# iacopo97/Multimodal-SAM-Adapter

Hardware: AMD Instinct MI355X
Metric: images/sec encoder fwd @1024x1024 RGB+LiDAR ViT-L (higher is better)
Workload: dtype split-operand MFMA: fp16 hi + e5m2 cross terms (h8c / h8 planes, ViT / interaction / up-conv GEMMs) fp16 hi/lo pairs x3 (TwinConvNeXt: f3 planes) and bf16 hi/lo x3 (neck, head); attention blocks with the rel-pos terms fused: every contraction on one fp16 MFMA (q, k, v, P rounded to fp16) in the bloc

## Files before the change

### include/mmsa.h

```cpp
#ifndef MMSA_H
#define MMSA_H
#include <stddef.h>
#include <stdint.h>
#ifdef __cplusplus
extern "C" {
#endif

#ifdef MMSA_BUILDING_LIBRARY
typedef hipStream_t mmsa_stream_t;
#else
typedef void* mmsa_stream_t;
#endif

#include "mmsa_version.h"
int mmsa_version(void);
const char* mmsa_last_error(void);

int mmsa_debug_poison_lds(unsigned pattern, mmsa_stream_t stream);
int mmsa_event_create(void** ev);
int mmsa_event_record(void* ev, mmsa_stream_t stream);
int mmsa_event_elapsed_ms(void* start, void* stop, float* ms);
int mmsa_event_destroy(void* ev);

enum { MMSA_ACT_NONE = 0, MMSA_ACT_GELU = 1, MMSA_ACT_RELU = 2, MMSA_ACT_RELU6 = 3, MMSA_ACT_HSWISH = 4, MMSA_ACT_SIGMOID = 5 };

enum { MMSA_DT_F32 = 0, MMSA_DT_F16 = 1, MMSA_DT_F64 = 2 };

enum { MMSA_FMT_B3 = 0, MMSA_FMT_H8 = 1, MMSA_FMT_H8C = 2, MMSA_FMT_F3 = 3, MMSA_FMT_W8 = 4  };

int mmsa_ms_deform_attn_forward(const void* value, const int64_t* spatial_shapes, const int64_t* level_start_index,
                                const void* sampling_loc, const void* attn_weight, void* out, int batch,
                                int spatial_size, int num_heads, int channels, int num_levels, int num_query,
                                int num_point, int im2col_step, int dtype, mmsa_stream_t stream);

int mmsa_ms_deform_attn_backward(const void* value, const int64_t* spatial_shapes, const int64_t* level_start_index,
                                 const void* sampling_loc, const void* attn_weight, const void* grad_output,
                                 void* grad_value, void* grad_sampling_loc, void* grad_attn_weight, int batch,
                                 int spatial_size, int num_heads, int channels, int num_levels, int num_query,
                                 int num_point, int im2col_step, int dtype, mmsa_stream_t stream);

int mmsa_msda_fused(const float* value, const int64_t* spatial_shapes, const int64_t* level_start_index,
                    const float* raw, long ldraw, const float* ref_points, float* out, long ldo,
                    uint16_t* out_planes, long ldop , int out_fmt , int batch,
                    int spatial_size, int num_heads, int channels, int num_levels, int num_query, int num_point,
                    float* clamp_max , mmsa_stream_t stream);

int mmsa_msda_fused_planes(const uint16_t* value_planes, long ldvp, int lo_bytes, const int64_t* spatial_shapes, const int64_t* level_start_index,
                           const float* raw, long ldraw, const float* ref_points, float* out, long ldo,
                           uint16_t* out_planes, long ldop, int out_fmt, int batch,
                           int spatial_size, int num_heads, int channels, int num_levels, int num_query, int num_point,
                           float* clamp_max, mmsa_stream_t stream);

int mmsa_rowstats_finalize(const float* rowstats, int rows, int strips, int D, float eps, float* mean_rstd, mmsa_stream_t stream);

int mmsa_zero_bytes(void* p, size_t bytes, mmsa_stream_t stream);
int mmsa_gemm_split3(const float* A, const uint16_t* Ap, long lda, long strideA,
                     const uint16_t* Wp, long strideW,
                     const float* bias, long strideBias, const float* colscale, const float* resid, long ldr,
                     long strideR, int resid_mod, float beta, float* C, long ldc, long strideC,
                     uint16_t* Cp, long ldcp, long strideCp, int M, int N, int K,
                     int batch, int act, float alpha, int out_mode, int ps_H, int ps_W, int ps_C, int fmt, int cp_fmt,
                     int max_grid, float* rowstats_out, const float* rownorm_mean_rstd, const float* rownorm_colsum, int flavour,
                     float* clamp_max , mmsa_stream_t stream);

int mmsa_convnext_mlp_fused(const uint16_t* Ap, long lda, long strideA, const uint16_t* W1p, long strideW1, const uint16_t* W2p,
                            long strideW2, const float* b1, const float* b2, const float* gamma, float* x, long ldx, long strideX,
                            int M, int C, int batch, int max_grid, int fmt,
                            float* clamp_max , mmsa_stream_t stream);

int mmsa_split_planes(const float* src, long ld, int rows, int cols, int cols_pad, uint16_t* planes, int kind,
                      float* clamp_max , mmsa_stream_t stream);

int mmsa_attention(const float* qkv, long ldq, const float* qkv_bias, const float* rp, float* out, long ldo, int B,
                   int H, int W, int heads, int head_dim, int window_size, float scale, mmsa_stream_t stream);
int mmsa_attention_planes(const uint16_t* qkv_planes, long ldq, const uint16_t* bias_planes, const float* rp,
                          uint16_t* out_planes, long ldo, int B, int H, int W, int heads, int head_dim,
                          int window_size, float scale, int out_fmt ,
                          int v_fmt ,
                          float* max_abs_logit , mmsa_stream_t stream);

int mmsa_relpos_bias(const float* qkv, long ldq, const float* Rh, const float* Rw, float* rp, int B, int H, int W,
                     int heads, int head_dim, int window_size, mmsa_stream_t stream);
int mmsa_relpos_bias_planes(const uint16_t* qkv_planes, long ldq, const float* Rh, const float* Rw,
                            float* rp, int B, int H, int W, int heads, int head_dim, int window_size, mmsa_stream_t stream);

int mmsa_layernorm_rows(const float* x, long ldx, const float* w, const float* b, float eps, float* y, long ldy,
                        float* y2, long ldy2, uint16_t* y_planes, long ldp ,
                        int rows, int C, int map_mode, int map_H, int map_W, int group_rows, long w_gstride, long y_gcol,
                        int y_wrap, int plane_fmt , float* clamp_max ,
                        mmsa_stream_t stream);

int mmsa_colstats(const float* x, long ldx, long strideB, const float* wrow, int B, int HW, int C, double* out,
                  int out_is_zero , mmsa_stream_t stream);

int mmsa_ffrm_finalize(const double* stats, int B, int HW, int C, float mean_w, float mean_b, const float* Wc,
                       const float* gn_w, const float* gn_b, float* mean_o, float* rstd_o, float* mult_o,
                       float* scratch , mmsa_stream_t stream);
int mmsa_lnhw_apply(const float* x, long ldx, const float* mean, const float* rstd, const float* mult, const float* w,
                    const float* bias, float* y, long ldy, int B, int HW, int C, mmsa_stream_t stream);

int mmsa_dwconv_nhwc(const float* x, long ldx, long xstrideB, const float* w, const float* bias, float* y, long ldy,
                     long ystrideB, uint16_t* y_planes, long ldp, long pstrideB , int planes_fmt ,
                     int B, int H, int W, int C, int k, int act,
                     int imgs_per_group ,
                     float* rowstats ,
                     float* clamp_max , mmsa_stream_t stream);
int mmsa_gconv_nhwc(const float* x, long ldx, const float* w, const float* bias, float* y, long ldy, int B, int H,
                    int W, int G, int cin_g, int cout_g, int k, int act, mmsa_stream_t stream);
int mmsa_gfe_qkv_conv(const float* x, long ldx, const float* w, float* y, long ldy, int B, int H, int W, int G, int cin_g, int cout_g,
                      int* covered, mmsa_stream_t stream);
int mmsa_dwpair_gate(const float* x, long ldx, const float* w, float* y, long ldy, uint16_t* y_planes, long ldp, int B, int H,
                     int W, int C, mmsa_stream_t stream);
int mmsa_im2col_nchw(const float* x, int B, int Ctot, int c0, int Cin, int H, int W, int p, float* out, int Kpad,
                     mmsa_stream_t stream);

long mmsa_gram_tn_scratch_bytes(int B, int P, int c);
int mmsa_gram_tn(const float* X, long ldx, const float* Y, long ldy, long strideB, double* G , int B, int P, int c,
                 int nblk, void* scratch, long scratch_bytes, mmsa_stream_t stream);
int mmsa_chanattn_build(const double* G, const double* sq, long sq_strideB, const double* sk, long sk_strideB,
                        const float* temp, const float* Wp, uint16_t* planes , int B, int c, int cpad,
                        int heads, mmsa_stream_t stream);
int mmsa_gffm_build(const double* E, uint16_t* x_planes, uint16_t* y_planes , int B, int c,
                    int cpad, mmsa_stream_t stream);
int mmsa_gelu_gate(const float* x, long ldx, float* y, long ldy, long rows, int C, mmsa_stream_t stream);
int mmsa_pool_hw(const float* z, long ldz, float* out, long ldo, int B, int H, int W, int C, mmsa_stream_t stream);
int mmsa_ca_apply(const float* z, long ldz, const float* att, long lda, float* out, long ldo,
                  uint16_t* out_planes, long ldp , int B, int H, int W, int C, mmsa_stream_t stream);

int mmsa_tail_fuse(const float* cmap, long ldc, long cstrideB, const float* xtok, long ldx, const float* bn_scale,
                   const float* bn_shift, float* out, uint16_t* out_planes , long ldp,
                   int B, int Hc, int Wc, int Hx, int Wx, int C, mmsa_stream_t stream);

int mmsa_global_attention_planes(const uint16_t* qkv_planes, long ldq, const uint16_t* bias_planes, const uint16_t* relpos_planes,
                                 uint16_t* out_planes, long ldo, int B, int H, int W, int heads, int head_dim, float scale,
                                 int out_fmt , int v_fmt ,
                                 float* max_abs_logit , mmsa_stream_t stream);

int mmsa_window_attention_planes(const uint16_t* qkv_planes, long ldq, const uint16_t* bias_planes,
                                 const uint16_t* relpos_planes, const uint16_t* selector, uint16_t* out_planes, long ldo, int B, int H, int W,
                                 int heads, int head_dim, int window_size, float scale, int out_fmt ,
                                 int v_fmt , float* max_abs_logit , mmsa_stream_t stream);

int mmsa_nchw_to_planes(const float* src, long strideB, uint16_t* planes, long ldp, int B, int C, long HW,
                        mmsa_stream_t stream);
int mmsa_head_fuse(const float* z0, const float* z1, int H1, int W1, const float* z2, int H2, int W2, const float* z3,
                   int H3, int W3, long ld, const float* bn_scale, const float* bn_shift, uint16_t* planes, long ldp,
                   float* out32, long ldo, int B, int H, int W, int C, int act, mmsa_stream_t stream);
int mmsa_tokens_to_nchw(const float* src, long ld, float* dst, int B, long HW, int C, mmsa_stream_t stream);

int mmsa_bilinear_accum_nchw(const float* src, long src_strideB, int B, int C, int hs, int ws, float* dst, int Hd, int Wd, int y0, int x0,
                             int hc, int wc, float* count, int accumulate, mmsa_stream_t stream);
int mmsa_div_count_nchw(float* x, const float* count, int B, int C, long HW, mmsa_stream_t stream);
int mmsa_argmax_nchw(const float* x, unsigned char* out, int B, int C, long HW, mmsa_stream_t stream);
int mmsa_crop_batch_nchw(const float* src, int B, int C, int H, int W, const int* windows, int n, float* dst, int hc, int wc,
                         mmsa_stream_t stream);
int mmsa_slide_argmax(const float* logits, int n, int C, int hs, int ws, const int* windows, unsigned char* out, int B, int H, int W,
                      int hc, int wc, int* uncovered, mmsa_stream_t stream);
int mmsa_slide_argmax_resized(const float* logits, int n, int C, int hs, int ws, const int* windows, unsigned char* out, int B, int H, int W,
                              int hc, int wc, int Hd, int Wd, int Hcut, int Wcut, int* uncovered, mmsa_stream_t stream);

int mmsa_softmax_flip_accum_nchw(const float* logits, float* acc, int B, int C, int H, int W, int flip, int accumulate, int finish_div, mmsa_stream_t stream);
int mmsa_aug_argmax(const float* const* logits, const int* views, int A, int C, const int* windows, const int* windows_host, int total,
                    unsigned char* out, int B, int Ho, int Wo, int* uncovered, mmsa_stream_t stream);

int mmsa_argmax_max_nchw(const float* x, unsigned char* out, float* maxval, int B, int C, long HW, mmsa_stream_t stream);
int mmsa_slide_argmax_conf(const float* logits, int n, int C, int hs, int ws, const int* windows, unsigned char* out, float* conf, int B, int H, int W,
                           int hc, int wc, int* uncovered, mmsa_stream_t stream);
int mmsa_slide_argmax_resized_conf(const float* logits, int n, int C, int hs, int ws, const int* windows, unsigned char* out, float* conf, int B, int H,
                                   int W, int hc, int wc, int Hd, int Wd, int Hcut, int Wcut, int* uncovered, mmsa_stream_t stream);
int mmsa_aug_argmax_conf(const float* const* logits, const int* views, int A, int C, const int* windows, const int* windows_host, int total,
                         unsigned char* out, float* conf, int B, int Ho, int Wo, int* uncovered, mmsa_stream_t stream);

enum { MMSA_PRE_U8 = 0, MMSA_PRE_F32 = 1 };
int mmsa_preprocess_nhwc(const void* src0, int dtype0, const void* src1, int dtype1, int B, int Hs, int Ws, const float* mean,
                         const float* sinv, const int* div255, const int* swap, const float* pad_val, float* dst, int H, int W,
                         mmsa_stream_t stream);
int mmsa_preprocess_crops(const void* src0, int dtype0, const void* src1, int dtype1, int B, int Hs, int Ws, const float* mean,
                          const float* sinv, const int* div255, const int* swap, const float* pad_val, int H, int W, const int* windows,
                          int n, float* dst, int hc, int wc, mmsa_stream_t stream);
int mmsa_preprocess_resize_nhwc(const void* src0, int dtype0, const void* src1, int dtype1, int B, int Hs, int Ws, const float* mean,
                                const float* sinv, const int* div255, const int* swap, const float* pad_val, float* dst, int H, int W,
                                int Hr, int Wr, const int* xofs, const void* xcoef, const int* yofs, const void* ycoef, int fixed_point,
                                mmsa_stream_t stream);
int mmsa_preprocess_resize_crops(const void* src0, int dtype0, const void* src1, int dtype1, int B, int Hs, int Ws, const float* mean,
                                 const float* sinv, const int* div255, const int* swap, const float* pad_val, int H, int W, const int* windows,
                                 int n, float* dst, int hc, int wc, int Hr, int Wr, const int* xofs, const void* xcoef, const int* yofs,
                                 const void* ycoef, int fixed_point, mmsa_stream_t stream);

int mmsa_eval_confusion_u8(const unsigned char* pred, const unsigned char* label, int B, int H, int W, int Hl, int Wl, const unsigned char* lut,
                           int C, const int* ymap, const int* xmap, const int* slots, int n_slots, int64_t* counts, mmsa_stream_t stream);
int mmsa_slide_argmax_eval(const float* logits, int n, int C, int hs, int ws, const int* windows, unsigned char* out, int B, int H, int W,
                           int hc, int wc, int* uncovered, const unsigned char* label, int Hl, int Wl, const unsigned char* lut, const int* ymap,
                           const int* xmap, const int* slots, int n_slots, int64_t* counts, mmsa_stream_t stream);

int mmsa_eval_calibration(const unsigned char* pred, const float* conf, const unsigned char* label, int B, int H, int W, int Hl, int Wl,
                          const unsigned char* lut, int C, const int* ymap, const int* xmap, const int* slots, int n_slots, int bins, int64_t* cal,
                          mmsa_stream_t stream);

int mmsa_eval_selective(const unsigned char* pred, const float* conf, const unsigned char* label, int B, int H, int W, int Hl, int Wl,
                        const unsigned char* lut, int C, const int* ymap, const int* xmap, const int* slots, int n_slots, int bins, int64_t* counts,
                        mmsa_stream_t stream);
int mmsa_abstain_u8(const unsigned char* pred, const float* conf, long n, int bins, int min_bin, unsigned char* out, mmsa_stream_t stream);

int mmsa_slide_argmax_conf_t(const float* logits, int n, int C, int hs, int ws, const int* windows, unsigned char* out, float* conf, int B, int H, int W,
                             int hc, int wc, int* uncovered, float inv_temperature, mmsa_stream_t stream);
int mmsa_slide_argmax_resized_conf_t(const float* logits, int n, int C, int hs, int ws, const int* windows, unsigned char* out, float* conf, int B, int H,
                                     int W, int hc, int wc, int Hd, int Wd, int Hcut, int Wcut, int* uncovered, float inv_temperature, mmsa_stream_t stream);
int mmsa_softmax_flip_accum_nchw_t(const float* logits, float* acc, int B, int C, int H, int W, int flip, int accumulate, int finish_div,
                                   float inv_temperature, mmsa_stream_t stream);
int mmsa_temperature_sweep_nchw(const float* logits, const unsigned char* label, int B, int C, int H, int W, int Hl, int Wl, const unsigned char* lut,
                                const int* ymap, const int* xmap, const int* slots, int n_slots, const float* inv_temperatures, int J, int bins,
                                int64_t* sweep, mmsa_stream_t stream);

int mmsa_argmax_score_nchw(const float* prob, unsigned char* out, float* score, int B, int C, int H, int W, int kind, float inv_log_c, mmsa_stream_t stream);
int mmsa_slide_argmax_score(const float* logits, int n, int C, int hs, int ws, const int* windows, unsigned char* out, float* score, int B, int H, int W,
                            int hc, int wc, int* uncovered, int kind, float inv_temperature, float inv_log_c, mmsa_stream_t stream);
int mmsa_slide_argmax_resized_score(const float* logits, int n, int C, int hs, int ws, const int* windows, unsigned char* out, float* score, int B, int H,
                                    int W, int hc, int wc, int Hd, int Wd, int Hcut, int Wcut, int* uncovered, int kind, float inv_temperature,
                                    float inv_log_c, mmsa_stream_t stream);

int mmsa_slide_argmax_topk(const float* logits, int n, int C, int hs, int ws, const int* windows, unsigned char* classes, float* probs, int B, int H, int W,
                           int hc, int wc, int* uncovered, int K, float inv_temperature, mmsa_stream_t stream);
int mmsa_argmax_topk_nchw(const float* prob, const unsigned char* first, unsigned char* classes, float* probs, int B, int C, int H, int W, int K,
                          mmsa_stream_t stream);
int mmsa_eval_topk_u8(const unsigned char* classes, int K, const unsigned char* label, int B, int H, int W, int Hl, int Wl, const unsigned char* lut, int C,
                      const int* ymap, const int* xmap, const int* slots, int n_slots, int64_t* counts, mmsa_stream_t stream);

int mmsa_eval_boundary_u8(const unsigned char* pred, const unsigned char* label, int B, int H, int W, int Hl, int Wl, const unsigned char* lut, int C,
                          const int* ymap, const int* xmap, const int* slots, int n_slots, int radius, int border, int64_t* counts, mmsa_stream_t stream);

int mmsa_boundary_distance_u8(const unsigned char* src, int B, int Hs, int Ws, const unsigned char* lut, const int* ymap, const int* xmap, int H, int W,
                              int cap, int border, unsigned short* scratch, unsigned short* d2, mmsa_stream_t stream);
int mmsa_eval_boundary_d2(const unsigned char* pred, const unsigned char* label, int B, int H, int W, int Hl, int Wl, const unsigned char* lut, int C,
                          const int* ymap, const int* xmap, const int* slots, int n_slots, const unsigned short* d2_pred, const unsigned short* d2_label,
                          int t, int64_t* counts, mmsa_stream_t stream);
int mmsa_eval_boundary_displacement(const unsigned char* pred, const unsigned char* label, int B, int H, int W, int Hl, int Wl, const unsigned char* lut,
                                    int C, const int* ymap, const int* xmap, const int* slots, int n_slots, const unsigned short* d2_pred,
                                    const unsigned short* d2_label, int cap, int64_t* hist, mmsa_stream_t stream);

int mmsa_components_u8(const unsigned char* src, int B, int Hs, int Ws, const unsigned char* lut, const int* ymap, const int* xmap, int H, int W,
                       int connectivity, int* root, mmsa_stream_t stream);
int mmsa_component_area(const int* root, int B, int H, int W, int* area, mmsa_stream_t stream);
int mmsa_suppress_small_u8(const unsigned char* pred, const int* root, const int* area, int B, int H, int W, int min_area, int fill, unsigned char* out,
                           mmsa_stream_t stream);
int mmsa_eval_segments(const unsigned char* pred, const unsigned char* label, int B, int H, int W, int Hl, int Wl, const unsigned char* lut, int C,
                       const int* ymap, const int* xmap, const int* slots, int n_slots, const int* root_pred, const int* root_label, int bins, int* scratch,
                       int64_t* counts, mmsa_stream_t stream);

int mmsa_segment_pairs(const unsigned char* pred, const unsigned char* label, int Hl, int Wl, const unsigned char* lut, int C, const int* ymap,
                       const int* xmap, const int* root_pred, const int* root_label, int B, int H, int W, int64_t* keys, int* counts, long capacity,
                       int* overflow, mmsa_stream_t stream);
int mmsa_eval_panoptic(const unsigned char* pred, const unsigned char* label, int B, int H, int W, int Hl, int Wl, const unsigned char* lut, int C,
                       const int* ymap, const int* xmap, const int* slots, int n_slots, const int* root_pred, const int* root_label, const int* planes,
                       const int64_t* keys, const int* counts, long capacity, int* match, int64_t* pq_counts, mmsa_stream_t stream);

int mmsa_render_u8(const unsigned char* pred, long pred_image_stride, long pred_row_stride, int B, int h, int w, const unsigned* palette, int npal,
                   int palette_reverse, const unsigned char* src, int Hs, int Ws, int src_reverse, double opacity, double one_minus_opacity,
                   unsigned char* out, mmsa_stream_t stream);
int mmsa_render_denorm_f32(const unsigned char* pred, long pred_image_stride, long pred_row_stride, int B, int h, int w, const unsigned* palette, int npal,
                           int palette_reverse, const float* src, int Cs, int Hs, int Ws, const float* mean, const float* std, int to_rgb, int mul255,
                           double opacity, double one_minus_opacity, unsigned char* out, mmsa_stream_t stream);

int mmsa_render_labels_u8(const unsigned char* pred, long pred_image_stride, long pred_row_stride, const unsigned char* label, int B, int h, int w, int Hl, int Wl,
                          const unsigned char* lut, int C, const int* ymap, const int* xmap, int mode, int wrong_by_label, const unsigned* table, int ntab,
                          const void* src, int src_form, int Cs, int Hs, int Ws, int src_reverse, const float* mean, const float* std, int to_rgb, int mul255,
                          double opacity, double one_minus_opacity, double mark_opacity, double one_minus_mark_opacity, unsigned char* out,
                          mmsa_stream_t stream);
int mmsa_render_values_f32(const float* values, const unsigned char* pred, long pred_image_stride, long pred_row_stride, int B, int h, int w, int bins,
                           int min_bin, const unsigned* table, int ntab, const void* src, int src_form, int Cs, int Hs, int Ws, int src_reverse,
                           const float* mean, const float* std, int to_rgb, int mul255, double opacity, double one_minus_opacity, double mark_opacity,
                           double one_minus_mark_opacity, unsigned char* out, mmsa_stream_t stream);
int mmsa_render_band_u8(const unsigned char* pred, long pred_image_stride, long pred_row_stride, const unsigned char* label, int B, int H, int W, int Hl, int Wl,
                        const unsigned char* lut, int C, const int* ymap, const int* xmap, int radius, int border, int where, int mark_by_label,
                        int inside_by_label, const unsigned* table, int ntab, const void* src, int src_form, int Cs, int Hs, int Ws, int src_reverse,
                        const float* mean, const float* std, int to_rgb, int mul255, double opacity, double one_minus_opacity, double mark_opacity,
                        double one_minus_mark_opacity, unsigned char* out, mmsa_stream_t stream);

#ifdef __cplusplus
}
#endif
#endif
```

### multimodal-sam-adapter_amd/csrc/common.h

```cpp
#pragma once
#include <hip/hip_runtime.h>
#include <stdint.h>
#include <stdio.h>
#include <stdarg.h>

#define MMSA_OK 0
#define MMSA_ERR_ARG (-1)
#define MMSA_ERR_LAUNCH (-2)

#define MMSA_BUILDING_LIBRARY 1
#include "../../include/mmsa.h"
void mmsa_set_error(const char* fmt, ...);

#ifdef MMSA_DEBUG_KNOBS
#include <stdlib.h>
static inline int mmsa_knob_env(const char* name, int dflt) { const char* v = getenv(name); return v ? atoi(v) : dflt; }
#define MMSA_KNOB(name_, dflt_) mmsa_knob_env(name_, dflt_)
#else
#define MMSA_KNOB(name_, dflt_) (dflt_)
#endif

#define MMSA_CHECK_ARG(cond, ...)            \
  do {                                       \
    if (!(cond)) {                           \
      mmsa_set_error(__VA_ARGS__);           \
      return MMSA_ERR_ARG;                   \
    }                                        \
  } while (0)

#define MMSA_CHECK_LAUNCH(name)                                              \
  do {                                                                       \
    hipError_t e__ = hipGetLastError();                                      \
    if (e__ != hipSuccess) {                                                 \
      mmsa_set_error("%s: launch failed: %s", name, hipGetErrorString(e__)); \
      return MMSA_ERR_LAUNCH;                                                \
    }                                                                        \
  } while (0)

#define MMSA_CHECK_INV_TEMPERATURE(name, it) \
  MMSA_CHECK_ARG((it) > 0.f && (it) <= 3.402823466e38f, "%s: inv_temperature = %g; a finite value > 0 is expected (float32(1 / T))", name, (double)(it))

#ifndef MMSA_XCD_ORDER
#define MMSA_XCD_ORDER 1
#endif
__device__ __forceinline__ unsigned mmsa_xcd_order(unsigned lin, unsigned total) {
#if MMSA_XCD_ORDER
  const unsigned per = total >> 3;
  return lin < (per << 3) ? (lin & 7u) * per + (lin >> 3) : lin;
#else
  (void)total;
  return lin;
#endif
}
__device__ __forceinline__ unsigned mmsa_block_lin() { return blockIdx.x + gridDim.x * (blockIdx.y + gridDim.y * blockIdx.z); }
__device__ __forceinline__ unsigned mmsa_block_count() { return gridDim.x * gridDim.y * gridDim.z; }

typedef __attribute__((ext_vector_type(8))) short bf16x8;
typedef __attribute__((ext_vector_type(4))) short bf16x4;
typedef __attribute__((ext_vector_type(4))) float f32x4;

__device__ __forceinline__ unsigned short f32_to_bf16_rn(float x) {
  unsigned u = __float_as_uint(x);
  u += 0x7FFFu + ((u >> 16) & 1u);
  return (unsigned short)(u >> 16);
}
__device__ __forceinline__ float bf16_to_f32(unsigned short h) { return __uint_as_float(((unsigned)h) << 16); }

typedef __attribute__((ext_vector_type(2))) __bf16 mmsa_bf16x2;
typedef __attribute__((ext_vector_type(2))) float mmsa_f32x2;

__device__ __forceinline__ void split2(float a, float b, unsigned& hi, unsigned& lo) {
  const mmsa_f32x2 v = {a, b};
  const mmsa_bf16x2 h = __builtin_convertvector(v, mmsa_bf16x2);
  const mmsa_f32x2 r = v - __builtin_convertvector(h, mmsa_f32x2);
  const mmsa_bf16x2 l = __builtin_convertvector(r, mmsa_bf16x2);
  hi = __builtin_bit_cast(unsigned, h);
  lo = __builtin_bit_cast(unsigned, l);
}

__device__ __forceinline__ void split_bf16(float x, unsigned short& hi, unsigned short& lo) {
  unsigned h, l;
  split2(x, 0.f, h, l);
  hi = (unsigned short)(h & 0xFFFFu);
  lo = (unsigned short)(l & 0xFFFFu);
}

__device__ __forceinline__ void split4(const float4 v, uint2& hi, uint2& lo) {
  split2(v.x, v.y, hi.x, lo.x);
  split2(v.z, v.w, hi.y, lo.y);
}

__device__ __forceinline__ float wave_sum(float v) {
#pragma unroll
  for (int o = 32; o > 0; o >>= 1) v += __shfl_xor(v, o, 64);
  return v;
}
__device__ __forceinline__ float half_wave_sum(float v) {
#pragma unroll
  for (int o = 16; o > 0; o >>= 1) v += __shfl_xor(v, o, 64);
  return v;
}
__device__ __forceinline__ float wave_max(float v) {
#pragma unroll
  for (int o = 32; o > 0; o >>= 1) v = fmaxf(v, __shfl_xor(v, o, 64));
  return v;
}

__host__ __device__ __forceinline__ int ilv(int k) { return ((k >> 5) << 6) | (k & 31); }

#define MMSA_CP_BASE(f_) ((f_) & 0xff)
#define MMSA_CP_SPLIT(f_) (((f_) >> 8) * 32)
#define MMSA_CP_AT(f_, col_) ((MMSA_CP_SPLIT(f_) > 0 && (col_) >= MMSA_CP_SPLIT(f_)) ? MMSA_FMT_H8 : MMSA_CP_BASE(f_))
#define MMSA_H8_MAX 57344.0f
#define MMSA_H8_LO_SCALE 2048.0f
#define MMSA_H8_MFMA_SCALE 0x74747474
#define MMSA_H8C_LO_COMP 1.09375f
typedef __attribute__((ext_vector_type(2))) _Float16 mmsa_h2;
typedef __attribute__((ext_vector_type(8))) _Float16 f16x8;
__device__ __forceinline__ void split2_f16(float a, float b, unsigned& hi, unsigned& lo) {
  const mmsa_f32x2 v = {a, b};
  const mmsa_h2 h = __builtin_convertvector(v, mmsa_h2);
  const mmsa_f32x2 r = v - __builtin_convertvector(h, mmsa_f32x2);
  hi = __builtin_bit_cast(unsigned, h);
  lo = __builtin_bit_cast(unsigned, __builtin_convertvector(r, mmsa_h2));
}
__device__ __forceinline__ unsigned pack_f16(float a, float b) {
  const mmsa_f32x2 v = {a, b};
  return __builtin_bit_cast(unsigned, __builtin_convertvector(v, mmsa_h2));
}

#define MMSA_F3_MAX 65504.0f
__device__ __forceinline__ void f3_split2(float a, float b, unsigned& hi, unsigned& lo) {
  a = __builtin_amdgcn_fmed3f(a, -MMSA_F3_MAX, MMSA_F3_MAX);
  b = __builtin_amdgcn_fmed3f(b, -MMSA_F3_MAX, MMSA_F3_MAX);
  split2_f16(a, b, hi, lo);
}
__device__ __forceinline__ void f3_split4(const float4 v, uint2& hi, uint2& lo) {
  f3_split2(v.x, v.y, hi.x, lo.x);
  f3_split2(v.z, v.w, hi.y, lo.y);
}
__device__ __forceinline__ void split4_fmt(const float4 v, uint2& hi, uint2& lo, int fmt) {
  if (fmt == MMSA_FMT_F3) f3_split4(v, hi, lo);
  else split4(v, hi, lo);
}

template <bool UPPER, bool COMP = false>
__device__ __forceinline__ void h8_split2(float a, float b, unsigned& hi, unsigned& lo8, unsigned& qh8) {
  a = __builtin_amdgcn_fmed3f(a, -MMSA_H8_MAX, MMSA_H8_MAX);
  b = __builtin_amdgcn_fmed3f(b, -MMSA_H8_MAX, MMSA_H8_MAX);
  const mmsa_f32x2 v = {a, b};
  const mmsa_h2 h = __builtin_convertvector(v, mmsa_h2);
  const mmsa_f32x2 hf = __builtin_convertvector(h, mmsa_f32x2);
  constexpr float ls_ = COMP ? MMSA_H8_LO_SCALE * MMSA_H8C_LO_COMP : MMSA_H8_LO_SCALE;
  const mmsa_f32x2 l = (v - hf) * ls_;
  hi = __builtin_bit_cast(unsigned, h);
  lo8 = (unsigned)__builtin_amdgcn_cvt_pk_bf8_f32(l.x, l.y, (int)lo8, UPPER);
  qh8 = (unsigned)__builtin_amdgcn_cvt_pk_bf8_f32(hf.x, hf.y, (int)qh8, UPPER);
}
template <bool COMP = false>
__device__ __forceinline__ void h8_split4(const float4 v, uint2& hi, unsigned& lo8, unsigned& qh8) {
  lo8 = 0u; qh8 = 0u;
  h8_split2<false, COMP>(v.x, v.y, hi.x, lo8, qh8);
  h8_split2<true, COMP>(v.z, v.w, hi.y, lo8, qh8);
}
__host__ __device__ __forceinline__ int h8_lo_off(int c) { return ((c >> 5) << 7) + 64 + (((c & 31) >> 3) << 4) + (c & 7); }

__device__ __forceinline__ void store_planes4(unsigned short* row, int c, const float4 v, int fmt) {
  if (fmt == MMSA_FMT_H8) {
    uint2 hi; unsigned lo8, qh8;
    h8_split4(v, hi, lo8, qh8);
    *reinterpret_cast<uint2*>(row + ilv(c)) = hi;
    unsigned char* rb = reinterpret_cast<unsigned char*>(row) + h8_lo_off(c);
    *reinterpret_cast<unsigned*>(rb) = lo8;
    *reinterpret_cast<unsigned*>(rb + 8) = qh8;
  } else {
    uint2 hh, ll;
    split4_fmt(v, hh, ll, fmt);
    *reinterpret_cast<uint2*>(row + ilv(c)) = hh;
    *reinterpret_cast<uint2*>(row + ilv(c) + 32) = ll;
  }
}

template <int XOR>
__device__ __forceinline__ void store_planes8_pair(unsigned short* row, int c8, const float4 v, int fmt, bool odd, bool do_store) {
  uint2 mine_hi, mine_x;
  if (fmt == MMSA_FMT_H8) h8_split4(v, mine_hi, mine_x.x, mine_x.y);
  else split4_fmt(v, mine_hi, mine_x, fmt);
  const uint2 snd = odd ? mine_hi : mine_x;
  uint2 rcv;
  rcv.x = __shfl_xor(snd.x, XOR, 64);
  rcv.y = __shfl_xor(snd.y, XOR, 64);
  uint4 pk;
  if (!odd) pk = make_uint4(mine_hi.x, mine_hi.y, rcv.x, rcv.y);
  else if (fmt == MMSA_FMT_H8) pk = make_uint4(rcv.x, mine_x.x, rcv.y, mine_x.y);
  else pk = make_uint4(rcv.x, rcv.y, mine_x.x, mine_x.y);
  const int off = odd ? (fmt == MMSA_FMT_H8 ? h8_lo_off(c8) >> 1 : ilv(c8) + 32) : ilv(c8);
  if (do_store) *reinterpret_cast<uint4*>(row + off) = pk;
}

__device__ __forceinline__ void store_planes1(unsigned short* row, int c, float x, int fmt) {
  if (fmt == MMSA_FMT_H8) {
    unsigned hi, lo8 = 0u, qh8 = 0u;
    h8_split2<false>(x, 0.f, hi, lo8, qh8);
    row[ilv(c)] = (unsigned short)(hi & 0xFFFFu);
    unsigned char* rb = reinterpret_cast<unsigned char*>(row) + h8_lo_off(c & ~3) + (c & 3);
    rb[0] = (unsigned char)(lo8 & 0xFFu);
    rb[8] = (unsigned char)(qh8 & 0xFFu);
  } else {
    unsigned short hh, ll;
    if (fmt == MMSA_FMT_F3) {
      unsigned h2, l2;
      f3_split2(x, 0.f, h2, l2);
      hh = (unsigned short)(h2 & 0xFFFFu);
      ll = (unsigned short)(l2 & 0xFFFFu);
    } else {
      split_bf16(x, hh, ll);
    }
    row[ilv(c)] = hh;
    row[ilv(c) + 32] = ll;
  }
}

struct H8cRow {
  unsigned short* hi;
  unsigned char* lo;
};
__device__ __forceinline__ H8cRow h8c_row(unsigned short* base, long ld_pair, long row, int kpad) {
  unsigned short* pb = base + (row >> 1) * ld_pair;
  H8cRow r;
  r.hi = pb + (row & 1) * kpad;
  r.lo = reinterpret_cast<unsigned char*>(pb + 2 * kpad) + (row & 1) * 64;
  return r;
}
__host__ __device__ __forceinline__ int h8c_lo_off(int k) { return ((k >> 6) << 7) + (((k & 31) >> 3) << 4) + (((k >> 5) & 1) << 3) + (k & 7); }
__device__ __forceinline__ void h8c_store4(const H8cRow r, int c, const float4 v) {
  uint2 hi; unsigned lo8, qh8;
  h8_split4<true>(v, hi, lo8, qh8);
  *reinterpret_cast<uint2*>(r.hi + c) = hi;
  *reinterpret_cast<unsigned*>(r.lo + h8c_lo_off(c)) = lo8;
}
template <int XOR>
__device__ __forceinline__ void h8c_store8_pair(const H8cRow r, int c8, const float4 v, bool odd, bool do_store) {
  uint2 hi; unsigned lo8, qh8;
  h8_split4<true>(v, hi, lo8, qh8);
  const uint2 snd = odd ? hi : make_uint2(lo8, 0u);
  uint2 rcv;
  rcv.x = __shfl_xor(snd.x, XOR, 64);
  rcv.y = __shfl_xor(snd.y, XOR, 64);
  if (!do_store) return;
  if (!odd) *reinterpret_cast<uint4*>(r.hi + c8) = make_uint4(hi.x, hi.y, rcv.x, rcv.y);
  else *reinterpret_cast<uint2*>(r.lo + h8c_lo_off(c8)) = make_uint2(rcv.x, lo8);
}
__device__ __forceinline__ void h8c_store1(const H8cRow r, int c, float x) {
  unsigned hi, lo8 = 0u, qh8 = 0u;
  h8_split2<false, true>(x, 0.f, hi, lo8, qh8);
  r.hi[c] = (unsigned short)(hi & 0xFFFFu);
  r.lo[h8c_lo_off(c)] = (unsigned char)(lo8 & 0xFFu);
}
template <int XOR>
__device__ __forceinline__ void store_planes8_pair_any(unsigned short* base, long ld, long row, int kpad, int c8, const float4 v, int fmt, bool odd, bool do_store) {
  if (fmt == MMSA_FMT_H8C) h8c_store8_pair<XOR>(h8c_row(base, ld, row, kpad), c8, v, odd, do_store);
  else store_planes8_pair<XOR>(base + row * ld, c8, v, fmt, odd, do_store);
}
__device__ __forceinline__ void store_planes4_any(unsigned short* base, long ld, long row, int kpad, int c, const float4 v, int fmt) {
  if (fmt == MMSA_FMT_H8C) h8c_store4(h8c_row(base, ld, row, kpad), c, v);
  else store_planes4(base + row * ld, c, v, fmt);
}
#define MMSA_PAD64(x_) (((x_) + 63) & ~63)

#define MMSA_W8_EMIN (-15)
#define MMSA_W8_EMAX 7

__device__ __forceinline__ float mmsa_clamp_limit(int fmt) {
  return (fmt == MMSA_FMT_H8 || fmt == MMSA_FMT_H8C) ? MMSA_H8_MAX : fmt == MMSA_FMT_F3 ? MMSA_F3_MAX : 3.0e38f;
}
#ifndef MMSA_CW_LEG
#define MMSA_CW_LEG 1
#endif
#ifndef MMSA_CW_REGS
#define MMSA_CW_REGS 1
#endif
#ifndef MMSA_CLAMP_WATCH
#define MMSA_CLAMP_WATCH 1
#endif
__device__ __forceinline__ void clamp_see(float& m, const float4 v) {
  if (MMSA_CLAMP_WATCH) m = fmaxf(fmaxf(m, fmaxf(fabsf(v.x), fabsf(v.y))), fmaxf(fabsf(v.z), fabsf(v.w)));
}
__device__ __forceinline__ void clamp_see1(float& m, float x) { if (MMSA_CLAMP_WATCH) m = fmaxf(m, fabsf(x)); }
__device__ __forceinline__ void clamp_report(float* word, float m, float limit) {
  if (MMSA_CLAMP_WATCH && word != nullptr && m > limit) atomicMax(reinterpret_cast<int*>(word), __float_as_int(m));
}

enum { ACT_NONE = 0, ACT_GELU = 1, ACT_RELU = 2, ACT_RELU6 = 3, ACT_HSWISH = 4, ACT_SIGMOID = 5 };

#ifndef MMSA_GELU_DEG
#define MMSA_GELU_DEG 7
#endif
#if MMSA_GELU_DEG == 6
#define MMSA_GELU_COEFFS {-1.151147127e+00f, -4.589156806e-01f, -5.323817953e-02f, 7.977456786e-03f, -7.398718735e-04f, 2.992386726e-05f}
#elif MMSA_GELU_DEG == 7
#define MMSA_GELU_COEFFS {-1.151126981e+00f, -4.590439200e-01f, -5.294858292e-02f, 7.670805324e-03f, -5.757985055e-04f, -1.279479329e-05f, 4.278379038e-06f}
#else
#define MMSA_GELU_COEFFS {-1.151111007e+00f, -4.591621459e-01f, -5.262760073e-02f, 7.245406508e-03f, -2.720646735e-04f, -1.314778056e-04f, 2.805791701e-05f, -1.902148711e-06f}
#endif
__device__ __forceinline__ float gelu1(float x) {
  constexpr float c[MMSA_GELU_DEG] = MMSA_GELU_COEFFS;
  const float a = fminf(fabsf(x), 6.0f);
  float p = fmaf(c[MMSA_GELU_DEG - 1], a, c[MMSA_GELU_DEG - 2]);
#pragma unroll
  for (int k = MMSA_GELU_DEG - 3; k >= 0; --k) p = fmaf(p, a, c[k]);
  p *= a;
  const float r = 1.0f - __builtin_amdgcn_exp2f(p);
  const float h = x * 0.5f;
  return fmaf(fabsf(h), r, h);
}
typedef __attribute__((ext_vector_type(2))) float mmsa_f2;
__device__ __forceinline__ mmsa_f2 gelu2(mmsa_f2 x) {
  mmsa_f2 a;
  a.x = fminf(fabsf(x.x), 6.0f);
  a.y = fminf(fabsf(x.y), 6.0f);
  constexpr float c[MMSA_GELU_DEG] = MMSA_GELU_COEFFS;
  mmsa_f2 p = a * c[MMSA_GELU_DEG - 1] + c[MMSA_GELU_DEG - 2];
#pragma unroll
  for (int k = MMSA_GELU_DEG - 3; k >= 0; --k) p = p * a + c[k];
  p = p * a;
  mmsa_f2 e;
  e.x = __builtin_amdgcn_exp2f(p.x);
  e.y = __builtin_amdgcn_exp2f(p.y);
  const mmsa_f2 r = 1.0f - e;
  const mmsa_f2 h = x * 0.5f;
  mmsa_f2 o;
  o.x = fmaf(fabsf(h.x), r.x, h.x);
  o.y = fmaf(fabsf(h.y), r.y, h.y);
  return o;
}
__device__ __forceinline__ float4 gelu4(float4 v) {
  const mmsa_f2 a = gelu2((mmsa_f2){v.x, v.y}), b = gelu2((mmsa_f2){v.z, v.w});
  return make_float4(a.x, a.y, b.x, b.y);
}

__device__ __forceinline__ float apply_act(float x, int act) {
  switch (act) {
    case ACT_GELU: return gelu1(x);
    case ACT_RELU: return fmaxf(x, 0.0f);
    case ACT_RELU6: return fminf(fmaxf(x, 0.0f), 6.0f);
    case ACT_HSWISH: return x * (fminf(fmaxf(x + 3.0f, 0.0f), 6.0f) / 6.0f);
    case ACT_SIGMOID: return 1.0f / (1.0f + expf(-x));
    default: return x;
  }
}

static inline int cdiv(long a, long b) { return (int)((a + b - 1) / b); }

#define MMSA_MAX_DEVICES 16
struct MmsaPerDevice { int cus[MMSA_MAX_DEVICES]; };
template <class F>
static inline int mmsa_per_device(MmsaPerDevice& st, F&& setup) {
  int dev = 0;
  if (hipGetDevice(&dev) != hipSuccess || dev < 0) dev = 0;
  if (dev < MMSA_MAX_DEVICES && st.cus[dev] > 0) return st.cus[dev];
  setup();
  int n = 0;
  if (hipDeviceGetAttribute(&n, hipDeviceAttributeMultiprocessorCount, dev) != hipSuccess || n <= 0) n = 256;
  if (dev < MMSA_MAX_DEVICES) st.cus[dev] = n;
  return n;
}
```

### multimodal-sam-adapter_amd/csrc/head.hip

```cpp
#include "common.h"

template <bool VEC>
__global__ __launch_bounds__(256) void nchw_to_planes_kernel(const float* __restrict__ src, long strideB, int C, long HW,
                                                             uint16_t* __restrict__ planes, long ldp) {
  __shared__ float tile[32][257];
  const int b = blockIdx.z;
  const long pix0 = (long)blockIdx.x * 256;
  const int c0 = blockIdx.y * 32;
  const int lane = threadIdx.x & 63, wv = threadIdx.x >> 6;
  const float* sb = src + (long)b * strideB;
  if (VEC) {
    float4 v[8];
#pragma unroll
    for (int j = 0; j < 8; ++j) {
      const int c = c0 + wv * 8 + j;
      const long pix = pix0 + 4 * lane;
      v[j] = (c < C && pix < HW) ? *reinterpret_cast<const float4*>(sb + (long)c * HW + pix) : make_float4(0.f, 0.f, 0.f, 0.f);
    }
#pragma unroll
    for (int j = 0; j < 8; ++j) {
      float* t = &tile[wv * 8 + j][4 * lane];
      t[0] = v[j].x; t[1] = v[j].y; t[2] = v[j].z; t[3] = v[j].w;
    }
  } else {
#pragma unroll
    for (int j = 0; j < 8; ++j) {
      const int cl = wv * 8 + j;
      const int c = c0 + cl;
#pragma unroll
      for (int k = 0; k < 4; ++k) {
        const long pix = pix0 + lane + 64 * k;
        tile[cl][lane + 64 * k] = (c < C && pix < HW) ? sb[(long)c * HW + pix] : 0.f;
      }
    }
  }
  __syncthreads();
  const int q = threadIdx.x & 3;
  const int pl = threadIdx.x >> 2;
#pragma unroll
  for (int k = 0; k < 4; ++k) {
    const int p = pl + 64 * k;
    const long pix = pix0 + p;
    if (pix >= HW) continue;
    float v[8];
#pragma unroll
    for (int j = 0; j < 8; ++j) v[j] = tile[8 * q + j][p];
    uint4 hi, lo;
    split2(v[0], v[1], hi.x, lo.x);
    split2(v[2], v[3], hi.y, lo.y);
    split2(v[4], v[5], hi.z, lo.z);
    split2(v[6], v[7], hi.w, lo.w);
    uint16_t* row = planes + ((long)b * HW + pix) * ldp + (long)blockIdx.y * 64 + 8 * q;
    *reinterpret_cast<uint4*>(row) = hi;
    *reinterpret_cast<uint4*>(row + 32) = lo;
  }
}

extern "C" int mmsa_nchw_to_planes(const float* src, long strideB, uint16_t* planes, long ldp, int B, int C, long HW,
                                   hipStream_t stream) {
  MMSA_CHECK_ARG(src && planes, "nchw_to_planes: null pointer");
  MMSA_CHECK_ARG(B > 0 && C > 0 && HW > 0, "nchw_to_planes: bad shape");
  const int cpad = (C + 31) / 32 * 32;
  MMSA_CHECK_ARG(ldp >= 2L * cpad && ldp % 64 == 0, "nchw_to_planes: planes row stride %ld < 2*%d or not a multiple of 64", ldp, cpad);
  MMSA_CHECK_ARG((reinterpret_cast<uintptr_t>(planes) & 127) == 0, "nchw_to_planes: planes must be 128-byte aligned");
  MMSA_CHECK_ARG(strideB >= (long)C * HW, "nchw_to_planes: image stride %ld < C*HW", strideB);
  dim3 grid(cdiv(HW, 256), cpad / 32, B);
  if ((HW & 3) == 0 && (strideB & 3) == 0 && (reinterpret_cast<uintptr_t>(src) & 15) == 0)
    hipLaunchKernelGGL(nchw_to_planes_kernel<true>, grid, dim3(256), 0, stream, src, strideB, C, HW, planes, ldp);
  else
    hipLaunchKernelGGL(nchw_to_planes_kernel<false>, grid, dim3(256), 0, stream, src, strideB, C, HW, planes, ldp);
  MMSA_CHECK_LAUNCH("nchw_to_planes");
  return MMSA_OK;
}

struct HeadLevels {
  const float* z[3];
  int H[3], W[3];
  float rh[3], rw[3];
};

__global__ __launch_bounds__(256) void head_fuse_kernel(const float* __restrict__ z0, long ld, HeadLevels lv, int nlv,
                                                        const float* __restrict__ bn_scale, const float* __restrict__ bn_shift,
                                                        uint16_t* __restrict__ planes, long ldp, float* __restrict__ out32, long ldo,
                                                        int H, int W, int C, long npix_total, int act) {
  const long pixg = (long)blockIdx.x * 4 + (threadIdx.x >> 6);
  if (pixg >= npix_total) return;
  const int lane = threadIdx.x & 63;
  const unsigned hw = (unsigned)H * (unsigned)W;
  const unsigned pg = (unsigned)pixg;
  const int b = (int)(pg / hw);
  const int rem = (int)(pg - (unsigned)b * hw);
  const int h = rem / W, w = rem - h * W;
  long o00[3], o01[3], o10[3], o11[3];
  float lh[3], lw[3];
#pragma unroll
  for (int i = 0; i < 3; ++i) {
    if (i < nlv) {
      float sh = ((float)h + 0.5f) * lv.rh[i] - 0.5f;
      float sw = ((float)w + 0.5f) * lv.rw[i] - 0.5f;
      sh = sh < 0.f ? 0.f : sh;
      sw = sw < 0.f ? 0.f : sw;
      const int h0 = min((int)sh, lv.H[i] - 1), w0 = min((int)sw, lv.W[i] - 1);
      const int h1 = h0 + (h0 < lv.H[i] - 1 ? 1 : 0), w1 = w0 + (w0 < lv.W[i] - 1 ? 1 : 0);
      lh[i] = sh - (float)h0;
      lw[i] = sw - (float)w0;
      const long base = (long)b * lv.H[i] * lv.W[i];
      o00[i] = (base + (long)h0 * lv.W[i] + w0) * ld;
      o01[i] = (base + (long)h0 * lv.W[i] + w1) * ld;
      o10[i] = (base + (long)h1 * lv.W[i] + w0) * ld;
      o11[i] = (base + (long)h1 * lv.W[i] + w1) * ld;
    } else {
      o00[i] = o01[i] = o10[i] = o11[i] = 0; lh[i] = lw[i] = 0.f;
    }
  }
  for (int c = lane * 8; c < C; c += 512) {
    float v[8];
    float4 t[3][2][4];
    const float4 a = *reinterpret_cast<const float4*>(z0 + pixg * ld + c);
    const float4 d = *reinterpret_cast<const float4*>(z0 + pixg * ld + c + 4);
#pragma unroll
    for (int i = 0; i < 3; ++i) {
      const int il = i < nlv ? i : 0;
      const float* zi = (nlv > 0 ? lv.z[il] : z0 + pixg * ld) + c;
#pragma unroll
      for (int hh = 0; hh < 2; ++hh) {
        t[i][hh][0] = *reinterpret_cast<const float4*>(zi + o00[il] + 4 * hh);
        t[i][hh][1] = *reinterpret_cast<const float4*>(zi + o01[il] + 4 * hh);
        t[i][hh][2] = *reinterpret_cast<const float4*>(zi + o10[il] + 4 * hh);
        t[i][hh][3] = *reinterpret_cast<const float4*>(zi + o11[il] + 4 * hh);
      }
    }
    const float4 s0 = *reinterpret_cast<const float4*>(bn_scale + c), s1 = *reinterpret_cast<const float4*>(bn_scale + c + 4);
    const float4 f0 = *reinterpret_cast<const float4*>(bn_shift + c), f1 = *reinterpret_cast<const float4*>(bn_shift + c + 4);
    __builtin_amdgcn_sched_barrier(0);
    v[0] = a.x; v[1] = a.y; v[2] = a.z; v[3] = a.w; v[4] = d.x; v[5] = d.y; v[6] = d.z; v[7] = d.w;
#pragma unroll
    for (int i = 0; i < 3; ++i) {
      if (i < nlv) {
        const float w00 = (1.f - lh[i]) * (1.f - lw[i]), w01 = (1.f - lh[i]) * lw[i], w10 = lh[i] * (1.f - lw[i]), w11 = lh[i] * lw[i];
#pragma unroll
        for (int hh = 0; hh < 2; ++hh) {
          const float4 t00 = t[i][hh][0], t01 = t[i][hh][1], t10 = t[i][hh][2], t11 = t[i][hh][3];
          v[4 * hh + 0] += w00 * t00.x + w01 * t01.x + w10 * t10.x + w11 * t11.x;
          v[4 * hh + 1] += w00 * t00.y + w01 * t01.y + w10 * t10.y + w11 * t11.y;
          v[4 * hh + 2] += w00 * t00.z + w01 * t01.z + w10 * t10.z + w11 * t11.z;
          v[4 * hh + 3] += w00 * t00.w + w01 * t01.w + w10 * t10.w + w11 * t11.w;
        }
      }
    }
    const float bs[8] = {s0.x, s0.y, s0.z, s0.w, s1.x, s1.y, s1.z, s1.w}, bf[8] = {f0.x, f0.y, f0.z, f0.w, f1.x, f1.y, f1.z, f1.w};
#pragma unroll
    for (int j = 0; j < 8; ++j) v[j] = apply_act(v[j] * bs[j] + bf[j], act);
    if (out32) {
      *reinterpret_cast<float4*>(out32 + pixg * ldo + c) = make_float4(v[0], v[1], v[2], v[3]);
      *reinterpret_cast<float4*>(out32 + pixg * ldo + c + 4) = make_float4(v[4], v[5], v[6], v[7]);
    }
    if (planes) {
      uint4 hi, lo;
      split2(v[0], v[1], hi.x, lo.x);
      split2(v[2], v[3], hi.y, lo.y);
      split2(v[4], v[5], hi.z, lo.z);
      split2(v[6], v[7], hi.w, lo.w);
      uint16_t* row = planes + pixg * ldp + ilv(c);
      *reinterpret_cast<uint4*>(row) = hi;
      *reinterpret_cast<uint4*>(row + 32) = lo;
    }
  }
}

extern "C" int mmsa_head_fuse(const float* z0, const float* z1, int H1, int W1, const float* z2, int H2, int W2, const float* z3,
                              int H3, int W3, long ld, const float* bn_scale, const float* bn_shift, uint16_t* planes, long ldp,
                              float* out32, long ldo, int B, int H, int W, int C, int act, hipStream_t stream) {
  MMSA_CHECK_ARG(z0 && bn_scale && bn_shift && (planes || out32), "head_fuse: null pointer");
  MMSA_CHECK_ARG(((((uintptr_t)bn_scale) | ((uintptr_t)bn_shift) | ((uintptr_t)z0)) & 15) == 0, "head_fuse: z0 / bn_scale / bn_shift must be 16-byte aligned");
  MMSA_CHECK_ARG(B > 0 && H > 0 && W > 0 && C > 0 && C % 8 == 0, "head_fuse: bad shape (C=%d must be a multiple of 8)", C);
  MMSA_CHECK_ARG(ld >= C && ld % 4 == 0, "head_fuse: row stride %ld", ld);
  MMSA_CHECK_ARG(!planes || (ldp >= 2L * ((C + 31) / 32 * 32) && ldp % 64 == 0 && (reinterpret_cast<uintptr_t>(planes) & 127) == 0),
                 "head_fuse: planes stride/alignment");
  MMSA_CHECK_ARG(!out32 || (ldo >= C && ldo % 4 == 0), "head_fuse: fp32 out stride %ld", ldo);
  HeadLevels lv;
  int n = 0;
  const float* zs[3] = {z1, z2, z3};
  const int hs[3] = {H1, H2, H3}, wsz[3] = {W1, W2, W3};
  for (int i = 0; i < 3; ++i) {
    lv.z[i] = nullptr; lv.H[i] = lv.W[i] = 1; lv.rh[i] = lv.rw[i] = 1.f;
  }
  for (int i = 0; i < 3; ++i) {
    if (!zs[i]) continue;
    MMSA_CHECK_ARG(hs[i] > 0 && wsz[i] > 0, "head_fuse: level %d has bad size", i + 1);
    lv.z[n] = zs[i]; lv.H[n] = hs[i]; lv.W[n] = wsz[i];
    lv.rh[n] = (float)hs[i] / (float)H;
    lv.rw[n] = (float)wsz[i] / (float)W;
    ++n;
  }
  const long npix = (long)B * H * W;
  MMSA_CHECK_ARG(npix < (1L << 31), "head_fuse: too many pixels for the 32-bit index arithmetic");
  hipLaunchKernelGGL(head_fuse_kernel, dim3(cdiv(npix, 4)), dim3(256), 0, stream, z0, ld, lv, n, bn_scale, bn_shift, planes, ldp,
                     out32, ldo, H, W, C, npix, act);
  MMSA_CHECK_LAUNCH("head_fuse");
  return MMSA_OK;
}

__global__ __launch_bounds__(256) void tokens_to_nchw_kernel(const float* __restrict__ src, long ld, float* __restrict__ dst, long HW, int C) {
  __shared__ float tile[32][33];
  const int b = blockIdx.z;
  const long pix0 = (long)blockIdx.x * 32;
  const int c0 = blockIdx.y * 32;
  const int tx = threadIdx.x & 31, ty = threadIdx.x >> 5;
#pragma unroll
  for (int k = 0; k < 4; ++k) {
    const int pl = ty + 8 * k;
    const long pix = pix0 + pl;
    const int c = c0 + tx;
    tile[pl][tx] = (pix < HW && c < C) ? src[((long)b * HW + pix) * ld + c] : 0.f;
  }
  __syncthreads();
#pragma unroll
  for (int k = 0; k < 4; ++k) {
    const int c = c0 + ty + 8 * k;
    const long pix = pix0 + tx;
    if (c < C && pix < HW) dst[((long)b * C + c) * HW + pix] = tile[tx][ty + 8 * k];
  }
}

extern "C" int mmsa_tokens_to_nchw(const float* src, long ld, float* dst, int B, long HW, int C, hipStream_t stream) {
  MMSA_CHECK_ARG(src && dst, "tokens_to_nchw: null pointer");
  MMSA_CHECK_ARG(B > 0 && HW > 0 && C > 0 && ld >= C, "tokens_to_nchw: bad shape");
  dim3 grid(cdiv(HW, 32), cdiv(C, 32), B);
  hipLaunchKernelGGL(tokens_to_nchw_kernel, grid, dim3(256), 0, stream, src, ld, dst, HW, C);
  MMSA_CHECK_LAUNCH("tokens_to_nchw");
  return MMSA_OK;
}
```

### multimodal-sam-adapter_amd/csrc/neck.hip

```cpp
#include "common.h"
#include <stdlib.h>

#define GR_ROWS 256
#define GR_BLK 96
#define GR_T 6
__device__ __forceinline__ bool gram_block_needed(int bi, int bj, int c, int nblk) {
  if (nblk <= 1) return true;
  const int ch = c / nblk;
  const int hi0 = (GR_BLK * bi) / ch, hi1 = min(c - 1, GR_BLK * bi + GR_BLK - 1) / ch;
  const int hj0 = (GR_BLK * bj) / ch, hj1 = min(c - 1, GR_BLK * bj + GR_BLK - 1) / ch;
  return !(hi1 < hj0 || hj1 < hi0);
}
__global__ __launch_bounds__(256) void gram_part_kernel(const float* __restrict__ X, long ldx, const float* __restrict__ Y, long ldy,
                                                        long strideB, float4* __restrict__ part, int P, int c, int nblk, int nslice) {
  const int nb = (c + GR_BLK - 1) / GR_BLK;
  const unsigned wg_ = mmsa_xcd_order(mmsa_block_lin(), mmsa_block_count());
  const int bx_ = (int)(wg_ % gridDim.x);
  const int bi = bx_ / nb, bj = bx_ % nb;
  if (!gram_block_needed(bi, bj, c, nblk)) return;
  const int lane = threadIdx.x & 63, wave = threadIdx.x >> 6;
  const int l15 = lane & 15, kk = lane >> 4;
  const int b = (int)(wg_ / (gridDim.x * gridDim.y));
  const int slice = (int)((wg_ / gridDim.x) % gridDim.y);
  const int u0 = 3 * (wave >> 1), v0 = 3 * (wave & 1);
// ... 11 lines not shown
#pragma unroll
  for (int u = 0; u < 3; ++u)
#pragma unroll
    for (int v = 0; v < 3; ++v) acc[u][v] = (f32x4){0.f, 0.f, 0.f, 0.f};
  const int pbeg = slice * GR_ROWS;
  const int pend = min(P, pbeg + GR_ROWS);
#define GR_LOADS(av_, bv_, pb_)                                                                   \
  _Pragma("unroll") for (int t = 0; t < 8; ++t) {                                                 \
    const int p = (pb_) + 4 * t + kk;                                                             \
    const long pr = p < pend ? p : pbeg;             \
    const float* xr = Xb + pr * ldx;                                                              \
    const float* yr = Yb + pr * ldy;                                                              \
    _Pragma("unroll") for (int u = 0; u < 3; ++u) { av_[t][u] = xr[ci[u]]; bv_[t][u] = yr[cj[u]]; } \
  }
#define GR_MFMAS(av_, bv_, pb_)                                                                   \
  _Pragma("unroll") for (int t = 0; t < 8; ++t) {                                                 \
    const float mp = ((pb_) + 4 * t + kk) < pend ? 1.f : 0.f;                                     \
      \
    _Pragma("unroll") for (int u = 0; u < 3; ++u) { av_[t][u] *= mp * mi[u]; bv_[t][u] *= mp * mj[u]; } \
    _Pragma("unroll") for (int u = 0; u < 3; ++u)                                                 \
      _Pragma("unroll") for (int v = 0; v < 3; ++v) acc[u][v] = __builtin_amdgcn_mfma_f32_16x16x4f32(av_[t][u], bv_[t][v], acc[u][v], 0, 0, 0); \
  }
  float a0[8][3], b0[8][3], a1[8][3], b1[8][3];
  GR_LOADS(a0, b0, pbeg)
#pragma unroll 1
  for (int pb = pbeg; pb < pend; pb += 64) {
    __builtin_amdgcn_sched_barrier(0);
    GR_LOADS(a1, b1, pb + 32)
    __builtin_amdgcn_sched_barrier(0);
    GR_MFMAS(a0, b0, pb)
    __builtin_amdgcn_sched_barrier(0);
    GR_LOADS(a0, b0, pb + 64)
    __builtin_amdgcn_sched_barrier(0);
    GR_MFMAS(a1, b1, pb + 32)
  }
#undef GR_LOADS
#undef GR_MFMAS
  float4* dst = part + ((((long)b * nb * nb + bx_) * nslice + slice) * (GR_T * GR_T)) * 64 + lane;
#pragma unroll
  for (int u = 0; u < 3; ++u)
#pragma unroll
    for (int v = 0; v < 3; ++v) dst[((u0 + u) * GR_T + v0 + v) * 64] = make_float4(acc[u][v][0], acc[u][v][1], acc[u][v][2], acc[u][v][3]);
}
__global__ __launch_bounds__(1024) void gram_sum_kernel(const float4* __restrict__ part, double* __restrict__ G, int c, int nblk, int nslice) {
  __shared__ double red[16][64][4];
  const int nb = (c + GR_BLK - 1) / GR_BLK;
  const int bi = blockIdx.y / nb, bj = blockIdx.y % nb;
  if (!gram_block_needed(bi, bj, c, nblk)) return;
  const int lane = threadIdx.x & 63, q = threadIdx.x >> 6;
  const int tile = blockIdx.x, b = blockIdx.z;
  const float4* src = part + (((long)b * nb * nb + blockIdx.y) * nslice * (GR_T * GR_T) + tile) * 64 + lane;
  double s0 = 0, s1 = 0, s2 = 0, s3 = 0;
#pragma unroll 4
  for (int sl = q; sl < nslice; sl += 16) {
    const float4 v = src[(long)sl * (GR_T * GR_T) * 64];
    s0 += (double)v.x; s1 += (double)v.y; s2 += (double)v.z; s3 += (double)v.w;
  }
  red[q][lane][0] = s0; red[q][lane][1] = s1; red[q][lane][2] = s2; red[q][lane][3] = s3;
  __syncthreads();
  if (threadIdx.x < 256) {
    const int ln = threadIdx.x >> 2, r = threadIdx.x & 3;
    double t = 0;
#pragma unroll
    for (int k = 0; k < 16; ++k) t += red[k][ln][r];
    const int u = tile / GR_T, v = tile % GR_T;
    const int i = GR_BLK * bi + 16 * u + 4 * (ln >> 4) + r;
    const int j = GR_BLK * bj + 16 * v + (ln & 15);
    if (i < c && j < c) G[((long)b * c + i) * c + j] = t;
  }
}

extern "C" long mmsa_gram_tn_scratch_bytes(int B, int P, int c) {
  if (B <= 0 || P <= 0 || c <= 0) return 0;
  const long nb = cdiv(c, GR_BLK);
  return (long)B * nb * nb * cdiv(P, GR_ROWS) * (GR_T * GR_T) * 64 * (long)sizeof(float4);
}

extern "C" int mmsa_gram_tn(const float* X, long ldx, const float* Y, long ldy, long strideB, double* G,
                            int B, int P, int c, int nblk, void* scratch, long scratch_bytes, hipStream_t stream) {
  MMSA_CHECK_ARG(X && Y && G && scratch && B > 0 && P > 0 && c > 0 && nblk > 0 && c % nblk == 0, "gram_tn: bad args");
  MMSA_CHECK_ARG(scratch_bytes >= mmsa_gram_tn_scratch_bytes(B, P, c) && (((uintptr_t)scratch) & 15) == 0,
                 "gram_tn: scratch of %ld bytes, %ld needed (mmsa_gram_tn_scratch_bytes), 16-byte aligned", scratch_bytes, mmsa_gram_tn_scratch_bytes(B, P, c));
  const int nb = cdiv(c, GR_BLK), nslice = cdiv(P, GR_ROWS);
  hipLaunchKernelGGL(gram_part_kernel, dim3(nb * nb, nslice, B), dim3(256), 0, stream, X, ldx, Y, ldy, strideB,
                     reinterpret_cast<float4*>(scratch), P, c, nblk, nslice);
  MMSA_CHECK_LAUNCH("gram_tn");
  hipLaunchKernelGGL(gram_sum_kernel, dim3(GR_T * GR_T, nb * nb, B), dim3(1024), 0, stream, reinterpret_cast<const float4*>(scratch), G, c, nblk, nslice);
  MMSA_CHECK_LAUNCH("gram_tn (slice sum)");
  return MMSA_OK;
}

__global__ __launch_bounds__(256) void chanattn_build_kernel(const double* __restrict__ G, const double* __restrict__ sq,
                                                             long sq_strideB, const double* __restrict__ sk, long sk_strideB,
                                                             const float* __restrict__ temp, const float* __restrict__ Wp,
                                                             unsigned short* __restrict__ planes,
                                                             int c, int cpad, int heads) {
  extern __shared__ float attn[];
  const int h = blockIdx.x, b = blockIdx.y;
  const int ch = c / heads;
  const int st = ch + 1;
  const double* Gb = G + (long)b * c * c;
  const float t = temp[h];
  float* nq = attn + ch * st;
  float* nk = nq + ch;
  for (int i = threadIdx.x; i < ch; i += 256) {
    nq[i] = fmaxf((float)sqrt(sq[(long)b * sq_strideB + h * ch + i]), 1e-12f);
    nk[i] = fmaxf((float)sqrt(sk[(long)b * sk_strideB + h * ch + i]), 1e-12f);
  }
  __syncthreads();
  for (int idx0 = threadIdx.x; idx0 < ch * ch; idx0 += 256 * 4) {
    double gv[4];
    int ii[4], jj[4];
#pragma unroll
    for (int u = 0; u < 4; ++u) {
      const int idx = min(idx0 + 256 * u, ch * ch - 1);
      ii[u] = idx / ch; jj[u] = idx - ii[u] * ch;
      gv[u] = Gb[(long)(h * ch + ii[u]) * c + h * ch + jj[u]];
    }
#pragma unroll
    for (int u = 0; u < 4; ++u)
      if (idx0 + 256 * u < ch * ch) attn[ii[u] * st + jj[u]] = (float)gv[u] / (nq[ii[u]] * nk[jj[u]]) * t;
  }
  __syncthreads();
  for (int i = threadIdx.x; i < ch; i += 256) {
    float mx = -INFINITY;
#pragma unroll 8
    for (int j = 0; j < ch; ++j) mx = fmaxf(mx, attn[i * st + j]);
    float s = 0.f;
#pragma unroll 4
    for (int j = 0; j < ch; ++j) {
      const float e = expf(attn[i * st + j] - mx);
      attn[i * st + j] = e;
      s += e;
    }
    const float inv = 1.0f / s;
#pragma unroll 8
    for (int j = 0; j < ch; ++j) attn[i * st + j] *= inv;
  }
  __syncthreads();
  const int o_per = (c + gridDim.z - 1) / gridDim.z;
  const int o_beg = blockIdx.z * o_per, o_end = min(c, o_beg + o_per);
  float* wl = nk + ch;
  {
    const int nw = (o_end - o_beg) * ch;
    for (int idx0 = threadIdx.x; idx0 < nw; idx0 += 256 * 4) {
      float wv[4];
#pragma unroll
      for (int u = 0; u < 4; ++u) {
        const int idx = min(idx0 + 256 * u, nw - 1);
        const int o = idx / ch, i = idx - o * ch;
        wv[u] = Wp[(long)(o_beg + o) * c + h * ch + i];
      }
#pragma unroll
      for (int u = 0; u < 4; ++u)
        if (idx0 + 256 * u < nw) wl[idx0 + 256 * u] = wv[u];
    }
  }
  __syncthreads();
  for (int idx = o_beg * ch + threadIdx.x; idx < o_end * ch; idx += 256) {
    const int o = idx / ch, j = idx - o * ch;
    const float* wrow = wl + (o - o_beg) * ch;
    float acc = 0.f;
#pragma unroll 8
    for (int i = 0; i < ch; ++i) acc += wrow[i] * attn[i * st + j];
    unsigned short hh, ll;
    split_bf16(acc, hh, ll);
    unsigned short* q_ = planes + ((long)b * c + o) * 2 * cpad + ilv(h * ch + j);
    q_[0] = hh;
    q_[32] = ll;
  }
}

extern "C" int mmsa_chanattn_build(const double* G, const double* sq, long sq_strideB, const double* sk, long sk_strideB,
                                   const float* temp, const float* Wp, unsigned short* planes,
                                   int B, int c, int cpad, int heads, hipStream_t stream) {
  MMSA_CHECK_ARG(G && sq && sk && temp && Wp && planes, "chanattn_build: null pointer");
  MMSA_CHECK_ARG(c % heads == 0 && cpad >= c, "chanattn_build: bad channel split");
  const int ch = c / heads;
  const int nz = c >= 192 ? 16 : 4;
  const size_t smem = ((size_t)ch * (ch + 1) + 2 * (size_t)ch + (size_t)cdiv(c, nz) * ch) * sizeof(float);
  MMSA_CHECK_ARG(smem <= 64 * 1024, "chanattn_build: head block too large");
  hipLaunchKernelGGL(chanattn_build_kernel, dim3(heads, B, nz), dim3(256), smem, stream, G, sq, sq_strideB, sk, sk_strideB, temp, Wp, planes, c, cpad, heads);
  MMSA_CHECK_LAUNCH("chanattn_build");
  return MMSA_OK;
}

__global__ __launch_bounds__(256) void gffm_build_kernel(const double* __restrict__ E, unsigned short* __restrict__ xp,
                                                         unsigned short* __restrict__ yp, int c, int cpad) {
  __shared__ float red[4];
  const int i = blockIdx.x, b = blockIdx.y, tr = blockIdx.z;
  const double* Eb = E + (long)b * c * c;
  const int lane = threadIdx.x & 63, wave = threadIdx.x >> 6;
  float mx = -INFINITY;
  for (int j = threadIdx.x; j < c; j += 256) mx = fmaxf(mx, (float)(tr ? Eb[(long)j * c + i] : Eb[(long)i * c + j]));
  mx = wave_max(mx);
  if (lane == 0) red[wave] = mx;
  __syncthreads();
  mx = fmaxf(fmaxf(red[0], red[1]), fmaxf(red[2], red[3]));
  __syncthreads();
  float s = 0.f;
  for (int j = threadIdx.x; j < c; j += 256) s += expf((float)((tr ? Eb[(long)j * c + i] : Eb[(long)i * c + j]) - (double)mx));
  s = wave_sum(s);
  if (lane == 0) red[wave] = s;
  __syncthreads();
  const float inv = 1.0f / (red[0] + red[1] + red[2] + red[3]);
  unsigned short* pl = tr ? yp : xp;
  for (int j = threadIdx.x; j < c; j += 256) {
    const float p = expf((float)((tr ? Eb[(long)j * c + i] : Eb[(long)i * c + j]) - (double)mx)) * inv;
    unsigned short hh, ll;
    split_bf16(p, hh, ll);
    unsigned short* q_ = pl + ((long)b * c + i) * 2 * cpad + ilv(j);
    q_[0] = hh;
    q_[32] = ll;
  }
}

extern "C" int mmsa_gffm_build(const double* E, unsigned short* xp, unsigned short* yp, int B, int c, int cpad,
                               hipStream_t stream) {
  MMSA_CHECK_ARG(E && xp && yp && cpad >= c, "gffm_build: bad args");
  hipLaunchKernelGGL(gffm_build_kernel, dim3(c, B, 2), dim3(256), 0, stream, E, xp, yp, c, cpad);
  MMSA_CHECK_LAUNCH("gffm_build");
  return MMSA_OK;
}

__global__ __launch_bounds__(256) void gelu_gate_kernel(const float* __restrict__ x, long ldx, float* __restrict__ y, long ldy,
                                                        int C, long total4) {
  const unsigned c4n = C >> 2;
  for (unsigned i = blockIdx.x * blockDim.x + threadIdx.x; i < (unsigned)total4; i += gridDim.x * blockDim.x) {
    const unsigned rowu = i / c4n;
    const int c = (int)(i - rowu * c4n) * 4;
    const long row = rowu;
    const float4 a = *reinterpret_cast<const float4*>(x + row * ldx + c);
    const float4 g = *reinterpret_cast<const float4*>(x + row * ldx + C + c);
    float4 o;
    o.x = apply_act(a.x, ACT_GELU) * g.x;
    o.y = apply_act(a.y, ACT_GELU) * g.y;
    o.z = apply_act(a.z, ACT_GELU) * g.z;
    o.w = apply_act(a.w, ACT_GELU) * g.w;
    *reinterpret_cast<float4*>(y + row * ldy + c) = o;
  }
}

extern "C" int mmsa_gelu_gate(const float* x, long ldx, float* y, long ldy, long rows, int C, hipStream_t stream) {
  MMSA_CHECK_ARG(x && y && rows > 0 && C > 0 && (C & 3) == 0 && (ldx & 3) == 0 && (ldy & 3) == 0, "gelu_gate: bad args");
  const long total4 = rows * (C >> 2);
  MMSA_CHECK_ARG(total4 < (1L << 31), "gelu_gate: too many elements for the 32-bit index arithmetic");
  int blocks = cdiv(total4, 256);
  if (blocks > 8192) blocks = 8192;
  hipLaunchKernelGGL(gelu_gate_kernel, dim3(blocks), dim3(256), 0, stream, x, ldx, y, ldy, C, total4);
  MMSA_CHECK_LAUNCH("gelu_gate");
  return MMSA_OK;
}

template <bool VEC>
__global__ __launch_bounds__(256) void pool_hw_kernel(const float* __restrict__ z, long ldz, float* __restrict__ out, long ldo,
                                                      int H, int W, int C) {
  const int r = blockIdx.x, b = blockIdx.y;
  const float* zb = z + (long)b * H * W * ldz;
  const bool row = r < H;
  const int n = row ? W : H;
  const long step = row ? ldz : (long)W * ldz;
  const float* base = zb + (row ? (long)r * W * ldz : (long)(r - H) * ldz);
  constexpr int V = VEC ? 4 : 1;
  for (int c = threadIdx.x * V; c < C; c += 256 * V) {
    float s[4] = {0.f, 0.f, 0.f, 0.f};
    int i = 0;
    for (; i + 8 <= n; i += 8) {
      float v[8][4];
#pragma unroll
      for (int k = 0; k < 8; ++k) {
        if constexpr (VEC) {
          const float4 t = *reinterpret_cast<const float4*>(base + (long)(i + k) * step + c);
          v[k][0] = t.x; v[k][1] = t.y; v[k][2] = t.z; v[k][3] = t.w;
        } else {
          v[k][0] = base[(long)(i + k) * step + c];
        }
      }
#pragma unroll
      for (int k = 0; k < 8; ++k)
#pragma unroll
        for (int q = 0; q < V; ++q) s[q] += v[k][q];
    }
    for (; i < n; ++i)
#pragma unroll
      for (int q = 0; q < V; ++q) s[q] += base[(long)i * step + c + q];
    float* o = out + ((long)b * (H + W) + r) * ldo + c;
#pragma unroll
    for (int q = 0; q < V; ++q) o[q] = s[q] / (float)n;
  }
}

extern "C" int mmsa_pool_hw(const float* z, long ldz, float* out, long ldo, int B, int H, int W, int C, hipStream_t stream) {
  MMSA_CHECK_ARG(z && out && B > 0 && H > 0 && W > 0 && C > 0, "pool_hw: bad args");
  if ((C & 3) == 0 && (ldz & 3) == 0 && (ldo & 3) == 0 && ((((uintptr_t)z) | ((uintptr_t)out)) & 15) == 0)
    hipLaunchKernelGGL(pool_hw_kernel<true>, dim3(H + W, B), dim3(256), 0, stream, z, ldz, out, ldo, H, W, C);
  else
    hipLaunchKernelGGL(pool_hw_kernel<false>, dim3(H + W, B), dim3(256), 0, stream, z, ldz, out, ldo, H, W, C);
  MMSA_CHECK_LAUNCH("pool_hw");
  return MMSA_OK;
}

__global__ __launch_bounds__(256) void ca_apply_kernel(const float* __restrict__ z, long ldz, const float* __restrict__ att, long lda,
                                                       float* __restrict__ out, long ldo, unsigned short* __restrict__ outp, long ldp,
                                                       int H, int W, int C, long total4) {
  const unsigned c4n = C >> 2;
  for (unsigned i = blockIdx.x * blockDim.x + threadIdx.x; i < (unsigned)total4; i += gridDim.x * blockDim.x) {
    const unsigned rowu = i / c4n;
    const int c = (int)(i - rowu * c4n) * 4;
    const long row = rowu;
    const unsigned t = rowu / (unsigned)W;
    const int w = (int)(rowu - t * (unsigned)W);
    const int b = (int)(t / (unsigned)H);
    const int h = (int)(t - (unsigned)b * (unsigned)H);
    const float4 v = *reinterpret_cast<const float4*>(z + row * ldz + c);
    const float4 ah = *reinterpret_cast<const float4*>(att + ((long)b * (H + W) + h) * lda + c);
    const float4 aw = *reinterpret_cast<const float4*>(att + ((long)b * (H + W) + H + w) * lda + c);
    float4 o;
    o.x = v.x + v.x * aw.x * ah.x;
    o.y = v.y + v.y * aw.y * ah.y;
    o.z = v.z + v.z * aw.z * ah.z;
    o.w = v.w + v.w * aw.w * ah.w;
    if (out) *reinterpret_cast<float4*>(out + row * ldo + c) = o;
    if (outp) {
      uint2 h2, l2;
      split4(o, h2, l2);
      unsigned short* q_ = outp + row * ldp + ilv(c);
      *reinterpret_cast<uint2*>(q_) = h2;
      *reinterpret_cast<uint2*>(q_ + 32) = l2;
    }
  }
}

extern "C" int mmsa_ca_apply(const float* z, long ldz, const float* att, long lda, float* out, long ldo,
                             unsigned short* out_planes, long ldp, int B, int H, int W, int C, hipStream_t stream) {
  MMSA_CHECK_ARG(z && att && (out || out_planes) && (C & 3) == 0 && (ldz & 3) == 0 && (lda & 3) == 0 && (ldo & 3) == 0, "ca_apply: bad args");
  MMSA_CHECK_ARG(!out_planes || ((((uintptr_t)out_planes) & 127) == 0 && (ldp & 63) == 0 && ldp >= 2L * ((C + 31) / 32 * 32)), "ca_apply: bad output planes");
  const long total4 = (long)B * H * W * (C >> 2);
  MMSA_CHECK_ARG(total4 < (1L << 31), "ca_apply: too many elements for the 32-bit index arithmetic");
  int blocks = cdiv(total4, 256);
  if (blocks > 8192) blocks = 8192;
  hipLaunchKernelGGL(ca_apply_kernel, dim3(blocks), dim3(256), 0, stream, z, ldz, att, lda, out, ldo, out_planes, ldp, H, W, C, total4);
  MMSA_CHECK_LAUNCH("ca_apply");
  return MMSA_OK;
}
```

### multimodal-sam-adapter_amd/csrc/tail.hip

```cpp
#include "common.h"

__global__ __launch_bounds__(256) void tail_fuse_kernel(const float* __restrict__ cmap, long ldc, long cstrideB, const float* __restrict__ xtok, long ldx,
                                                        const float* __restrict__ bn_scale, const float* __restrict__ bn_shift,
                                                        float* __restrict__ out, unsigned short* __restrict__ outp, long ldp,
                                                        int Hc, int Wc, int Hx, int Wx, int C, float rh, float rw) {
  __shared__ float tile[32][33];
  const int b = blockIdx.z;
  const int pix0 = blockIdx.x * 32;
  const int c0 = blockIdx.y * 32;
  const int tx = threadIdx.x & 31, ty = threadIdx.x >> 5;
  const int npix = Hc * Wc;
#pragma unroll
  for (int k = 0; k < 4; ++k) {
    const int pl = ty + 8 * k;
    const int pix = pix0 + pl;
    const int c = c0 + tx;
    float v = 0.f;
    if (pix < npix && c < C) {
      const int h = pix / Wc, w = pix - h * Wc;
      v = cmap[(long)b * cstrideB + (long)pix * ldc + c];
      float sh = ((float)h + 0.5f) * rh - 0.5f;
      float sw = ((float)w + 0.5f) * rw - 0.5f;
      sh = sh < 0.f ? 0.f : sh;
      sw = sw < 0.f ? 0.f : sw;
      const int h0 = (int)sh, w0 = (int)sw;
      const int h1 = h0 + (h0 < Hx - 1 ? 1 : 0), w1 = w0 + (w0 < Wx - 1 ? 1 : 0);
      const float lh = sh - (float)h0, lw = sw - (float)w0;
      if (xtok) {
        const float* xb = xtok + (long)b * Hx * Wx * ldx + c;
        const float v00 = xb[((long)h0 * Wx + w0) * ldx], v01 = xb[((long)h0 * Wx + w1) * ldx];
        const float v10 = xb[((long)h1 * Wx + w0) * ldx], v11 = xb[((long)h1 * Wx + w1) * ldx];
        const float r = (1.f - lh) * ((1.f - lw) * v00 + lw * v01) + lh * ((1.f - lw) * v10 + lw * v11);
        v = v + r;
      }
      v = v * bn_scale[c] + bn_shift[c];
      if (outp) {
        unsigned short hh, ll;
        split_bf16(v, hh, ll);
        unsigned short* q_ = outp + ((long)b * npix + pix) * ldp + ilv(c);
        q_[0] = hh;
        q_[32] = ll;
      }
    }
    tile[pl][tx] = v;
  }
  __syncthreads();
#pragma unroll
  for (int k = 0; k < 4; ++k) {
    const int cl = ty + 8 * k;
    const int c = c0 + cl;
    const int pix = pix0 + tx;
    if (c < C && pix < npix) out[((long)b * C + c) * npix + pix] = tile[tx][cl];
  }
}

__global__ __launch_bounds__(256) void tail_fuse64_kernel(const float* __restrict__ cmap, long ldc, long cstrideB, const float* __restrict__ xtok, long ldx,
                                                          const float* __restrict__ bn_scale, const float* __restrict__ bn_shift,
                                                          float* __restrict__ out, unsigned short* __restrict__ outp, long ldp,
                                                          int Hc, int Wc, int Hx, int Wx, int C, float rh, float rw) {
  __shared__ float tile[64][65];
  const int b = blockIdx.z;
  const int pix0 = blockIdx.x * 64, c0 = blockIdx.y * 64;
  const int t = threadIdx.x;
  const int cg = t & 15, pr = t >> 4;
  const int npix = Hc * Wc;
  const int c = c0 + 4 * cg;
  const bool c_ok = c < C;
  float4 sc = make_float4(0.f, 0.f, 0.f, 0.f), sf = sc;
  if (c_ok) { sc = *reinterpret_cast<const float4*>(bn_scale + c); sf = *reinterpret_cast<const float4*>(bn_shift + c); }
  const float* xb = xtok + (long)b * Hx * Wx * ldx + c;
#pragma unroll
  for (int k = 0; k < 4; ++k) {
    const int pl = pr + 16 * k;
    const int pix = pix0 + pl;
    float4 v = make_float4(0.f, 0.f, 0.f, 0.f);
    const bool ok = pix < npix && c_ok;
    if (ok) {
      const int h = pix / Wc, w = pix - h * Wc;
      v = *reinterpret_cast<const float4*>(cmap + (long)b * cstrideB + (long)pix * ldc + c);
      float sh = ((float)h + 0.5f) * rh - 0.5f;
      float sw = ((float)w + 0.5f) * rw - 0.5f;
      sh = sh < 0.f ? 0.f : sh;
      sw = sw < 0.f ? 0.f : sw;
      const int h0 = (int)sh, w0 = (int)sw;
      const int h1 = h0 + (h0 < Hx - 1 ? 1 : 0), w1 = w0 + (w0 < Wx - 1 ? 1 : 0);
      const float lh = sh - (float)h0, lw = sw - (float)w0;
      if (xtok) {
        const float4 v00 = *reinterpret_cast<const float4*>(xb + ((long)h0 * Wx + w0) * ldx), v01 = *reinterpret_cast<const float4*>(xb + ((long)h0 * Wx + w1) * ldx);
        const float4 v10 = *reinterpret_cast<const float4*>(xb + ((long)h1 * Wx + w0) * ldx), v11 = *reinterpret_cast<const float4*>(xb + ((long)h1 * Wx + w1) * ldx);
#define TF_ONE(f_) { const float r_ = (1.f - lh) * ((1.f - lw) * v00.f_ + lw * v01.f_) + lh * ((1.f - lw) * v10.f_ + lw * v11.f_); v.f_ = (v.f_ + r_) * sc.f_ + sf.f_; }
        TF_ONE(x) TF_ONE(y) TF_ONE(z) TF_ONE(w)
#undef TF_ONE
      } else {
        v.x = v.x * sc.x + sf.x; v.y = v.y * sc.y + sf.y; v.z = v.z * sc.z + sf.z; v.w = v.w * sc.w + sf.w;
      }
    }
    if (outp) {
      unsigned short* row = outp + ((long)b * npix + min(pix, npix - 1)) * ldp;
      store_planes8_pair<1>(row, c & ~7, v, MMSA_FMT_B3, (cg & 1) != 0, ok);
    }
    tile[pl][4 * cg + 0] = v.x; tile[pl][4 * cg + 1] = v.y; tile[pl][4 * cg + 2] = v.z; tile[pl][4 * cg + 3] = v.w;
  }
  __syncthreads();
  const int pg = t & 15, cr = t >> 4;
  const bool vec = (npix & 3) == 0;
#pragma unroll
  for (int k = 0; k < 4; ++k) {
    const int cl = cr + 16 * k;
    const int cc = c0 + cl;
    const int pix = pix0 + 4 * pg;
    if (cc >= C || pix >= npix) continue;
    const float4 o = make_float4(tile[4 * pg][cl], tile[4 * pg + 1][cl], tile[4 * pg + 2][cl], tile[4 * pg + 3][cl]);
    float* dst = out + ((long)b * C + cc) * npix + pix;
    if (vec) *reinterpret_cast<float4*>(dst) = o;
    else {
      dst[0] = o.x;
      if (pix + 1 < npix) dst[1] = o.y;
      if (pix + 2 < npix) dst[2] = o.z;
      if (pix + 3 < npix) dst[3] = o.w;
    }
  }
}

extern "C" int mmsa_tail_fuse(const float* cmap, long ldc, long cstrideB, const float* xtok, long ldx, const float* bn_scale,
                              const float* bn_shift, float* out, unsigned short* out_planes, long ldp, int B, int Hc, int Wc,
                              int Hx, int Wx, int C, hipStream_t stream) {
  MMSA_CHECK_ARG(cmap && bn_scale && bn_shift && out, "tail_fuse: null pointer");
  MMSA_CHECK_ARG(B > 0 && Hc > 0 && Wc > 0 && Hx > 0 && Wx > 0 && C > 0, "tail_fuse: bad shape");
  MMSA_CHECK_ARG(!out_planes || ((C & 31) == 0 && ldp >= 2L * C), "tail_fuse: planes output needs C % 32 == 0 and ldp >= 2C");
  const float rh = (float)Hx / (float)Hc, rw = (float)Wx / (float)Wc;
  const bool old_tiles = MMSA_KNOB("MMSA_TAIL32", 0) != 0;
  const bool wide = !old_tiles && (C & 3) == 0 && (ldc & 3) == 0 && (!xtok || (ldx & 3) == 0) && (cstrideB & 3) == 0 &&
                    ((((uintptr_t)cmap) | ((uintptr_t)xtok) | ((uintptr_t)bn_scale) | ((uintptr_t)bn_shift) | ((uintptr_t)out)) & 15) == 0 &&
                    (!out_planes || ((C & 7) == 0 && (ldp & 7) == 0 && (((uintptr_t)out_planes) & 15) == 0));
  if (wide) {
    dim3 grid64(cdiv((long)Hc * Wc, 64), cdiv(C, 64), B);
    hipLaunchKernelGGL(tail_fuse64_kernel, grid64, dim3(256), 0, stream, cmap, ldc, cstrideB, xtok, ldx, bn_scale, bn_shift, out, out_planes, ldp, Hc, Wc, Hx, Wx, C, rh, rw);
    MMSA_CHECK_LAUNCH("tail_fuse");
    return MMSA_OK;
  }
  dim3 grid(cdiv((long)Hc * Wc, 32), cdiv(C, 32), B);
  hipLaunchKernelGGL(tail_fuse_kernel, grid, dim3(256), 0, stream, cmap, ldc, cstrideB, xtok, ldx, bn_scale, bn_shift, out, out_planes, ldp, Hc, Wc, Hx, Wx, C, rh, rw);
  MMSA_CHECK_LAUNCH("tail_fuse");
  return MMSA_OK;
}
```

### multimodal-sam-adapter_amd/mmsa/backbone.py

```python
import contextlib
import functools
import math
import os

import torch
import torch.nn as nn

from . import ops, pack
from .pack import PackPlan, _linear_resize_rows, fold_gfe_qkv
from .params import CONVNEXT_ARCH, build_tree

_VIT_DEFAULTS = dict(img_size=1024, patch_size=16, in_chans=3, embed_dim=1024, depth=24, mlp_ratio=4.0,
                     qkv_bias=True, use_abs_pos=True, use_rel_pos=True, rel_pos_zero_init=True, window_size=14,
                     global_attn_indexes=[5, 11, 17, 23], pretrained_size=1024, fix=False)


class OperandRangeError(RuntimeError):
    """A forward converted a value beyond the range of an fp16-based operand format (the clamp watch word, include/mmsa.h) and nothing is left to
    re-route: `range_fallback` is off, or the value is a q / k / v (or a qkv bias / rel-pos table entry) beyond +-65504 inside the attention kernels,
    which read fp16-based planes in every mode.  The outputs of that forward are invalid."""


class Workspace:

    def __init__(self, device):
        self.device = device
        self.bufs = {}
        self.zeroed = set()

    def get(self, name, rows, cols, dtype=torch.float32, zero=False):
        n = rows * cols
        b = self.bufs.get(name)
        if b is None or b.numel() < n or b.dtype != dtype:
            b = torch.zeros(n, dtype=dtype, device=self.device) if zero else torch.empty(n, dtype=dtype, device=self.device)
            self.bufs[name] = b
        if zero:
            self.zeroed.add(name)
        return b[:n].view(rows, cols)

    def poison(self):
        for name, b in self.bufs.items():
            if name in self.zeroed:
                continue
            if b.dtype in (torch.float32, torch.float64):
                b.fill_(float("nan"))
            elif b.dtype == torch.int16:
                b.fill_(0x7fc0)

    def planes(self, name, rows, cols, zero=False, fmt=ops.FMT_B3):
        tr, tc, cp = ops.planes_shape(rows, cols, fmt)
        return ops.Planes(self.get(name + ".pl", tr, tc, torch.int16, zero or cp != cols), rows, cols, cp, fmt)

    def nbytes(self):
        return sum(b.numel() * b.element_size() for b in self.bufs.values())


class _Tagged:

    def __init__(self, ws, tag):
        self.ws, self.tag = ws, tag

    def get(self, name, *a, **k):
        return self.ws.get(self.tag + name, *a, **k)

    def planes(self, name, *a, **k):
        return self.ws.planes(self.tag + name, *a, **k)

    @property
    def device(self):
        return self.ws.device

    def poison(self):
        return self.ws.poison()

    def nbytes(self):
        return self.ws.nbytes()


class SAMAdapterbimodalMixModNewInTwinConvNEW(nn.Module):
    def __init__(self, pretrain_size=1024, num_heads=12, conv_inplane=64, n_points=4,
                 modalities_name=['rgb', 'depth', 'lidar', 'event'], modalities_ch=[3, 3, 3, 1],
                 deform_num_heads=6, init_values=0., gamma_init_values=0., interaction_indexes=None, with_cffn=True,
                 cffn_ratio=0.25, deform_ratio=1.0, add_vit_feature=True, pretrained=None,
                 use_extra_extractor=True, with_cp=True, drop_path_rate=0.4, drop_rate=0., drop_multimodal_path=0.2,
                 arch='base', checkpoint='check', *args, **kwargs):
        super().__init__()
        vit = dict(_VIT_DEFAULTS)
        for k in list(kwargs):
            if k in vit:
                vit[k] = kwargs.pop(k)
        if 'rgb' not in modalities_name or len(modalities_name) != 2:
            raise NotImplementedError("mmsa: the MI355X path implements the bimodal (rgb + one auxiliary modality) encoder; "
                                      f"got modalities_name={modalities_name}")
        if list(modalities_ch) != [3, 3]:
            raise NotImplementedError("mmsa: TwinConvNeXt takes two 3-channel streams (TC:296-316)")
        if not vit["use_abs_pos"]:
            raise NotImplementedError("mmsa: use_abs_pos=False is not a working configuration of the reference either (its forward interpolates "
                                      "self.pos_embed unconditionally, BK:276, which is None then: IE:113-114)")
        if interaction_indexes is None:
            raise ValueError("interaction_indexes is required")
        D = vit["embed_dim"]
        self.cfg = dict(embed_dim=D, depth=vit["depth"], num_heads=num_heads, mlp_ratio=vit["mlp_ratio"],
                        patch_size=vit["patch_size"], pretrained_size=vit["pretrained_size"], img_size=vit["img_size"],
                        window_size=vit["window_size"], global_attn_indexes=list(vit["global_attn_indexes"]),
                        conv_inplane=conv_inplane, n_points=n_points, deform_num_heads=deform_num_heads,
                        init_values=init_values, interaction_indexes=[list(i) for i in interaction_indexes],
                        cffn_ratio=cffn_ratio, deform_ratio=deform_ratio, arch=arch,
                        use_extra_extractor=bool(use_extra_extractor), with_cffn=bool(with_cffn), add_vit_feature=bool(add_vit_feature),
                        use_rel_pos=bool(vit["use_rel_pos"]), qkv_bias=bool(vit["qkv_bias"]))
        a = CONVNEXT_ARCH[arch] if isinstance(arch, str) else arch
        self.depths, self.channels = list(a["depths"]), list(a["channels"])
        if [2 * c for c in self.channels] != [conv_inplane * m for m in (4, 8, 16, 32)]:
            raise ValueError("conv_inplane*{4,8,16,32} must equal twice the ConvNeXt stage widths (AM:894-907)")
        for c in self.channels:
            if c % 32 != 0:
                raise ValueError("ConvNeXt stage widths must be multiples of 32 (groups=32 convs, GroupNorm(32))")
        hd = D // num_heads
        if D % num_heads or ops.pad32(hd) not in (32, 64, 96):
            raise NotImplementedError(f"mmsa: attention head_dim {hd} not supported by the HIP kernels (up to 96; widths that are "
                                      "not multiples of 32 run zero-padded per head, e.g. ViT-H's 80 as 96)")
        self.img_size = vit["img_size"]
        self.embed_dim = D
        self.interaction_indexes = self.cfg["interaction_indexes"]
        self.modalities_name, self.modalities_ch = modalities_name, modalities_ch
        self.in_ch_im = 3
        build_tree(self, self.cfg)
        self._packed = None
        self._ws = None
        self._taps = None
        self.register_load_state_dict_post_hook(lambda m, _: m.invalidate())
        self.init_weights(pretrained)
        if isinstance(checkpoint, str) and checkpoint not in ("", "check"):
            local = checkpoint if os.path.isfile(checkpoint) else os.environ.get("MMSA_CONVNEXT_CKPT", "")
            if os.path.isfile(local):
                self.load_convnext_checkpoint(local)
            else:
                import warnings
                warnings.warn(f"mmsa: ConvNeXt checkpoint '{checkpoint}' is not a local file and MMSA_CONVNEXT_CKPT names no mirror: "
                              "TwinConvNeXt keeps its random initialisation (the reference downloads and loads it, TC:382-443)")
        self.eval()

    def init_weights(self, pretrained=None):
        if isinstance(pretrained, str):
            from .checkpoint import load_pretrained
            self._pretrained_report = load_pretrained(self, pretrained)

    def load_convnext_checkpoint(self, path):
        ck = torch.load(path, map_location="cpu")
        sd = ck.get("state_dict", ck.get("model", ck)) if isinstance(ck, dict) else ck
        sd = {(k[9:] if k.startswith("backbone.") else k): v for k, v in sd.items()}
        if list(sd.keys())[0].startswith("module."):
            sd = {k[7:]: v for k, v in sd.items()}
        own = self.state_dict()
        loaded, new = [], {}
        for k, v in sd.items():
            dot = k.find(".")
            for sfx in ("_x", "_y"):
                nk = (k[:dot] + sfx + k[dot:]) if dot != -1 else k + sfx
                full = "spm.twin_conv." + nk
                if full in own:
                    new[full] = v
                    loaded.append(full)
        self.load_state_dict(new, strict=False)
        return loaded

    def invalidate(self):
        self._packed = None
        self._wide_range = False
        self._carry_modes = None
        self._inter_pairs = set()

    def train(self, mode=True):
        if mode:
            raise NotImplementedError("mmsa: the MI355X backbone implements the inference forward path only")
        return super().train(False)

    H8_DEFAULT = ("vit", "inter", "up", "attnv")
    attention_precision = "auto"

    range_fallback = True

    inter_follow_blocks = True

    fp8_weights = False

    fuse_gfe_qkv = True

    def _inter_pair_set(self):
        return set(getattr(self, "_inter_pairs", ()) or ())

    def _interaction_of_block(self, bi):
        for i, idx in enumerate(self.interaction_indexes):
            if idx[0] <= bi <= idx[-1]:
                return i
        return None

    def _wide(self):
        return bool(getattr(self, "_wide_range", False))

    def _h8_sites(self):
        return PackPlan.of(self).h8_sites

    @contextlib.contextmanager
    def chain(self, index):
        base = self._ws
        if base is None:
            raise RuntimeError("mmsa: run one forward() before opening a chain (workspace not created yet)")
        self._ws = _Tagged(base, f"chain{index}_")
        try:
            yield self
        finally:
            self._ws = base

    @torch.no_grad()
    def effective_state_dict(self):
        sd = self.state_dict()
        out = type(sd)((k, v.detach().clone()) for k, v in sd.items())
        plan = PackPlan.of(self)
        if not plan.fp8_weights:
            return out
        fold = plan.fold_ln
        dev = torch.device("cuda", torch.cuda.current_device()) if torch.cuda.is_available() else torch.device("cpu")
        for i in range(self.cfg["depth"]):
            b = f"blocks.{i}."
            for key, ln in (("attn.qkv.weight", "norm1.weight"), ("attn.proj.weight", None), ("mlp.lin1.weight", "norm2.weight"), ("mlp.lin2.weight", None)):
                w = sd[b + key].detach().to(dev, torch.float32)
                lnw = sd[b + ln].detach().to(dev, torch.float32) if (fold and ln) else None
                out[b + key] = pack.fp8_effective(w, lnw)[1].to(sd[b + key].device, sd[b + key].dtype)
        return out

    def _fold_ln_wanted(self):
        return PackPlan.of(self).fold_ln

    def _pack(self, dev):
        return pack.pack(self, dev)

    _hd_true = property(lambda self: self.cfg["embed_dim"] // self.cfg["num_heads"])
    _hd_pad = property(lambda self: ops.pad32(self._hd_true))

    @torch.no_grad()
    def _geometry(self, H, W, dev):
        pk = self._packed
        key = (H, W)
        if key in pk["geom"]:
            return pk["geom"][key]
        cfg = self.cfg
        p = cfg["patch_size"]
        Hp, Wp = H // p, W // p
        g = {}
        g["pos"] = _bicubic_resize(pk["pos_src"][0], Hp, Wp).reshape(Hp * Wp, -1).contiguous()
        ss1 = torch.tensor([(H // 8, W // 8), (H // 16, W // 16), (H // 32, W // 32)], dtype=torch.int64)
        ss2 = torch.tensor([(H // 16, W // 16)], dtype=torch.int64)
        g["ss1"], g["ss2"] = ss1.to(dev), ss2.to(dev)
        g["lsi1"] = torch.cat((ss1.new_zeros(1), ss1.prod(1).cumsum(0)[:-1])).to(dev)
        g["lsi2"] = ss2.new_zeros(1).to(dev)
        g["ref1"] = _ref_points([(H // 16, W // 16)]).to(dev)
        g["ref2"] = _ref_points([(H // 8, W // 8), (H // 16, W // 16), (H // 32, W // 32)]).to(dev)
        g["rel"] = []
        ws = cfg["window_size"]
        hd_ = self._hd_pad
        g["relg"] = []
        for blk in pk["blocks"]:
            relg = None
            if blk["ws"]:
                g["rel"].append((_rel_table(ws, blk["rph"]), _rel_table(ws, blk["rpw"])) if blk.get("relp") is None else None)
            elif hd_ == 64 and Wp == 64 and Hp <= 64 and Hp % 4 == 0:
                th = blk["rph"] if blk["rph"].shape[0] == 2 * Hp - 1 else _linear_resize_rows(blk["rph"], 2 * Hp - 1)
                tw = blk["rpw"] if blk["rpw"].shape[0] == 2 * Wp - 1 else _linear_resize_rows(blk["rpw"], 2 * Wp - 1)
                relg = (ops.global_relpos_planes(th, tw, fmt=ops.FMT_F3),
                        ops.global_relpos_planes(th, tw, fmt=ops.FMT_H8) if blk["qkv_bp16"] is not None else None)
                g["rel"].append(None)
            else:
                g["rel"].append((_rel_table(Hp, blk["rph"]), _rel_table(Wp, blk["rpw"])))
            g["relg"].append(relg)
        pk["geom"][key] = g
        return g

    @torch.no_grad()
    def _prepare(self, x):
        if not x.is_cuda:
            raise RuntimeError("mmsa: input must be a GPU tensor; the MI355X backbone has no CPU path")
        if x.dim() != 4 or x.shape[1] != 6:
            raise RuntimeError(f"mmsa: expected [B, 6, H, W] (rgb + auxiliary modality), got {tuple(x.shape)}")
        B, _, H, W = x.shape
        if H != self.img_size or W != self.img_size:
            raise RuntimeError(f"mmsa: H=W=img_size={self.img_size} is required (GFFM LayerNorm length, AM:240-241); got {H}x{W}")
        if H % 32 != 0:
            raise RuntimeError("mmsa: img_size must be a multiple of 32")
        dev = x.device
        x = x.contiguous().float()
        if self._packed is None or self._packed.get("dev") != dev or pack.packed_settings(self._packed) != PackPlan.of(self).settings():
            self._packed = self._pack(dev)
            self._packed["dev"] = dev
        if self._ws is None or self._ws.device != dev:
            self._ws = Workspace(dev)
        return x, B, H, W

    def _cbufs(self, B, H, W, tag=""):
        D = self.cfg["embed_dim"]
        Nc = (H // 8) * (W // 8) + (H // 16) * (W // 16) + (H // 32) * (W // 32)
        return self._ws.get("c1" + tag, B * (H // 4) * (W // 4), D), self._ws.get("c" + tag, B * Nc, D), Nc

    def forward(self, x):
        if not x.is_cuda:
            raise RuntimeError("mmsa: input must be a GPU tensor; the MI355X backbone has no CPU path")
        with torch.cuda.device(x.device):
            guard = self.attention_guard == "sync" and not torch.cuda.is_current_stream_capturing()
            depth = self.cfg["depth"]
            for _ in range(depth + 2):
                x, B, H, W = self._prepare(x)
                with ops.clamp_watch(self._packed["attn_guard"][depth:]):
                    c1, cbuf, Nc = self._cbufs(B, H, W)
                    c1_ready = self._spm(x, B, H, W, c1, cbuf, Nc)
                    outs = self._vit(x, B, H, W, c1, cbuf, c1_ready)
                if not guard or not self.check_attention_guard():
                    break
            return outs, None

    @torch.no_grad()
    def forward_taps(self, x):
        self._taps = {}
        try:
            outs, _ = self.forward(x)
            torch.cuda.synchronize(x.device)
            taps = self._taps
        finally:
            self._taps = None
        B, _, H, W = x.shape
        D = self.cfg["embed_dim"]
        res = {}
        for k, v in taps.items():
            if k.startswith(("twin", "fuse")):
                i = int(k[-1])
                h, w = H // (4 << i), W // (4 << i)
                res[k] = v.reshape(B, h, w, -1).permute(0, 3, 1, 2).contiguous()
            else:
                res[k] = v.reshape(B, -1, D)
        for i, f in enumerate(outs):
            res[f"f{i + 1}"] = f
        return outs, res

    def forward_pipelined(self, x_next):
        cur = getattr(self, "_pl_cur", None)
        dev_ = x_next.device if x_next is not None else (cur["x"].device if cur is not None else None)
        if dev_ is None:
            return None
        with torch.cuda.device(dev_):
            return self._forward_pipelined(x_next, cur)

    def _forward_pipelined(self, x_next, cur):
        main = torch.cuda.current_stream()
        nxt = None
        if x_next is not None:
            x_next, B, H, W = self._prepare(x_next)
            q = 1 - cur["set"] if cur is not None else 0
            c1, cbuf, Nc = self._cbufs(B, H, W, f"_p{q}")
            if getattr(self, "_pipe_stream", None) is None or self._pipe_stream.device != x_next.device:
                self._pipe_stream = torch.cuda.Stream(device=x_next.device)
            sa = self._pipe_stream
            ops.zero_(self._ws.get("pl_tick", 1, 1))
            sa.wait_stream(main)
            with torch.cuda.stream(sa):
                joins = self._spm(x_next, B, H, W, c1, cbuf, Nc, join=False)
            nxt = dict(x=x_next, set=q, dims=(B, H, W), c1=c1, c=cbuf)
        outs = None
        if cur is not None:
            B, H, W = cur["dims"]
            outs = self._vit(cur["x"], B, H, W, cur["c1"], cur["c"], None)
        if nxt is not None:
            for e in joins:
                main.wait_event(e)
            main.wait_stream(self._pipe_stream)
        self._pl_cur = nxt
        return (outs, None) if outs is not None else None

    def _vit(self, x, B, H, W, c1, cbuf, c1_ready):
        pk, ws, cfg = self._packed, self._ws, self.cfg
        dev = x.device
        geo = self._geometry(H, W, dev)
        D = cfg["embed_dim"]
        p = cfg["patch_size"]
        Hp, Wp = H // p, W // p
        T = Hp * Wp
        n2, n3, n4 = (H // 8) * (W // 8), T, (H // 32) * (W // 32)
        Nc = n2 + n3 + n4

        a = ws.get("pe_a", B * T, pk["pe_w"].kpad)
        ops.im2col_nchw(x, 0, 3, p, a)
        xs = [ws.get(f"x{i}", B * T, D) for i in range(len(self.interaction_indexes) + 1)]
        ops.gemm(a, pk["pe_w"], xs[0], bias=pk["pe_b"], resid=geo["pos"], resid_mod=T)
        taps = self._taps
        if taps is not None:
            taps["x_in"], taps["c_in"] = xs[0].clone(), cbuf[:B * Nc].clone()

        self._cfold = None
        n_inter = len(self.interaction_indexes)
        for i, idx in enumerate(self.interaction_indexes):
            it = pk["inter"][i]
            self._injector(it["inj"], xs[i], xs[i + 1], cbuf, geo, B, T, Nc)
            for bi in range(idx[0], idx[-1] + 1):
                self._block(pk["blocks"][bi], geo["rel"][bi], xs[i + 1], B, Hp, Wp, geo["relg"][bi],
                            next_fmt=pk["blocks"][bi + 1]["qkv"].afmt if bi < idx[-1] else None)
            for j, ex in enumerate(it["ext"]):
                self._extractor(ex, cbuf, xs[i + 1], geo, B, T, Nc, H, W, last=(i == n_inter - 1 and j == len(it["ext"]) - 1))
            if taps is not None:
                taps[f"x{i}"], taps[f"c{i}"] = xs[i + 1].clone(), cbuf[:B * Nc].clone()
        self._cfold = None

        if c1_ready is not None:
            torch.cuda.current_stream().wait_event(c1_ready)
        if taps is not None:
            taps["c1_map"] = c1.clone()
        outs = []
        c2p = ws.planes("up_a", B * n2, D, fmt=pk["up"].fmt)
        for bi in range(B):
            ops.split_planes(cbuf[bi * Nc:bi * Nc + n2], kpad=D, out=c2p.rows(bi * n2, (bi + 1) * n2))
        ops.gemm(c2p, pk["up"], c1, bias=pk["up_b"], resid=c1, batch=B, m=n2, stride_a=c2p.batch_stride(n2),
                 stride_r=(H // 4) * (W // 4) * D, stride_c=(H // 4) * (W // 4) * D, pixel_shuffle=(H // 8, W // 8, D))
        emit = bool(getattr(self, "emit_planes", False)) and D % 32 == 0
        ctag = getattr(self._ws, "tag", "")
        if not hasattr(self, "_planes_gens"):
            self._planes_gens = {}
        pgen = self._planes_gens.setdefault(ctag, [0])
        pgen[0] += 1
        outs = []
        for k, (src, cs, (hh, wwd)) in enumerate(((c1, (H // 4) * (W // 4) * D, (H // 4, W // 4)), (cbuf, Nc * D, (H // 8, W // 8)),
                                                  (cbuf[n2:], Nc * D, (Hp, Wp)), (cbuf[n2 + n3:], Nc * D, (H // 32, W // 32)))):
            f = torch.empty(B, D, hh, wwd, device=dev)
            fpl = ws.planes(f"f{k + 1}_out", B * hh * wwd, D) if emit else None
            ops.tail_fuse(src, cs, xs[k + 1] if self.cfg["add_vit_feature"] else None, *pk["bn"][k], f, B, hh, wwd, Hp, Wp, out_planes=fpl)
            if emit:
                f._mmsa_planes = fpl.stamp(pgen)
            outs.append(f)
        f1, f2, f3, f4 = outs
        return [f1, f2, f3, f4]

    def _stream_planes(self, rows, fmt):
        D = self.cfg["embed_dim"]
        return (self._ws.planes("blk_xp", rows, D, fmt=fmt), self._ws.get("blk_rs", rows, 2 * (D // 64)))

    def _block(self, bp, rel, x, B, Hp, Wp, relg=None, next_fmt=None):
        ws, cfg = self._ws, self.cfg
        D, heads = cfg["embed_dim"], cfg["num_heads"]
        hd = self._hd_pad
        scale = self._hd_true ** -0.5
        Da = heads * hd
        T = Hp * Wp
        folded_w = self._packed["fold_ln"]
        fold = folded_w and B * T >= 128
        fused = bp.get("relp") is not None or relg is not None
        f16 = bp["qkv_bp16"] is not None and self._attn_mode(bp) == "f16"
        vf = bp["qkv"].afmt
        gw = self._packed["attn_guard"][bp["index"]:bp["index"] + 1]
        if fold:
            xp, rs = self._stream_planes(B * T, vf)
            mr = ws.get("blk_mr", B * T, 2)
            ops.rowstats_finalize(rs, B * T, D, 1e-6, mr)
            n = None
        else:
            n = ws.planes("blk_n", B * T, D, fmt=vf)
            if folded_w:
                ops.layernorm(x, self._packed["ln_one"], self._packed["ln_zero"], 1e-6, out_planes=n)
            else:
                ops.layernorm(x, bp["n1w"], bp["n1b"], 1e-6, out_planes=n)
        all16 = fused and f16
        qkv = ws.planes("blk_qkv", B * T, 3 * Da, fmt=ops.FMT_H8 if all16 else ops.FMT_F3)
        if all16:
            bias_p = bp["qkv_bp16"]
        elif f16 and not fused:
            bias_p = bp["qkv_bp"]
            qkv.split = bias_p.split
        else:
            bias_p = bp["qkv_bp_b3"]
        if fold:
            ops.gemm(xp, bp["qkv"], bias=bp["qkv_bf"], out_planes=qkv, row_norm=(mr, bp["qkv_cs"]))
        else:
            ops.gemm(n, bp["qkv"], bias=bp["qkv_bf"] if folded_w else bp["qkv_b"], out_planes=qkv)
        wsz = bp["ws"]
        ao = ws.planes("blk_ao", B * T, Da, fmt=bp["proj"].afmt)
        if bp.get("relp") is not None:
            ops.window_attention(qkv, bias_p, bp["relp16"] if all16 else bp["relp"], ao, B, Hp, Wp, heads, hd, wsz, scale, max_logit=gw)
        elif relg is not None:
            ops.global_attention(qkv, bias_p, relg[1] if all16 else relg[0], ao, B, Hp, Wp, heads, hd, scale, max_logit=gw)
        else:
            kk = 2 * wsz if wsz else Hp + Wp
            rp = ws.get("blk_rp", B * heads * T, kk)
            ops.relpos_bias(qkv, rel[0], rel[1], rp, B, Hp, Wp, heads, hd, wsz)
            ops.attention(qkv, bias_p, rp, ao, B, Hp, Wp, heads, hd, wsz, scale, max_logit=gw)
        vf = bp["lin1"].afmt
        h = ws.planes("blk_h", B * T, bp["lin1"].n, fmt=vf)
        if fold:
            xp, rs = self._stream_planes(B * T, vf)
            ops.gemm(ao, bp["proj"], x, bias=bp["proj_b"], resid=x, out_planes=xp, rowstats_out=rs)
            ops.rowstats_finalize(rs, B * T, D, 1e-6, mr)
            ops.gemm(xp, bp["lin1"], bias=bp["lin1_bf"], act="gelu", out_planes=h, row_norm=(mr, bp["lin1_cs"]))
            if next_fmt is not None:
                xp, rs = self._stream_planes(B * T, next_fmt)
                ops.gemm(h, bp["lin2"], x, bias=bp["lin2_b"], resid=x, out_planes=xp, rowstats_out=rs)
            else:
                ops.gemm(h, bp["lin2"], x, bias=bp["lin2_b"], resid=x)
            return
        ops.gemm(ao, bp["proj"], x, bias=bp["proj_b"], resid=x)
        n = ws.planes("blk_n", B * T, D, fmt=vf)
        if folded_w:
            ops.layernorm(x, self._packed["ln_one"], self._packed["ln_zero"], 1e-6, out_planes=n)
        else:
            ops.layernorm(x, bp["n2w"], bp["n2b"], 1e-6, out_planes=n)
        ops.gemm(n, bp["lin1"], bias=bp["lin1_bf"] if folded_w else bp["lin1_b"], act="gelu", out_planes=h)
        ops.gemm(h, bp["lin2"], x, bias=bp["lin2_b"], resid=x)

    ATTN_F16_MAX_LOGIT = 8.0

    attention_guard = "sync"

    def _attn_policy(self):
        return getattr(self, "attention_precision", "auto")

    def _attn_mode(self, bp):
        pol = self._attn_policy()
        if pol in ("f16", "b3"):
            return pol
        return bp.get("amode") or "f16"

    def attention_guard_words(self):
        return self._packed["attn_guard"] if self._packed is not None else None

    @torch.no_grad()
    def check_attention_guard(self, reroute=True, vals=None):
        pk = self._packed
        if pk is None:
            return []
        if vals is None:
            vals = pk["attn_guard"].tolist()
        depth = self.cfg["depth"]
        clamped = max(float(vals[depth]) if len(vals) > depth else 0.0, float(pk.get("weights_clamped", 0.0)))
        if clamped > 0.0:
            if self.range_fallback and not self._wide():
                if reroute:
                    self._carry_modes = [(bp.get("amode"), bp.get("max_logit", 0.0)) for bp in pk["blocks"]]
                    self._wide_range = True
                    self._packed = None
                return list(range(depth))
            if len(vals) > depth and vals[depth] > 0.0:
                pk["attn_guard"][depth:].zero_()
            raise OperandRangeError(f"mmsa: a value of magnitude {clamped:.6g} or more (the GEMM's register epilogue reports the format's limit, not the value) was clamped on its way "
                                    "into fp16-based operand planes (h8 / h8c hold |x| <= 57344, f3 |x| <= 65504): the outputs since the last check are not the reference's.  "
                                    + ("The model is in its wide-range state already: what clamped is an operand of the attention kernels (q / k / v, a qkv bias or a rel-pos table "
                                       "entry beyond +-65504)." if self._wide() else "`range_fallback = True` (the default) re-routes instead of refusing."))
        auto = self._attn_policy() == "auto"
        moved = []
        dev, plan = pk["attn_guard"].device, PackPlan.of(self)
        sd_dev = functools.lru_cache(None)(lambda: pack.float_state_dict(self, dev))
        for bp, v in zip(pk["blocks"], vals):
            bp["max_logit"] = max(float(v), bp.get("max_logit", 0.0))
            if not auto or bp["qkv_bp16"] is None:
                continue
            if bp.get("amode") != "b3" and bp["max_logit"] > self.ATTN_F16_MAX_LOGIT:
                moved.append(bp["index"])
                if reroute:
                    bp["amode"] = "b3"
                    pack.repack_block_on_pairs(pk, bp, sd_dev, plan, dev)
            elif bp.get("amode") is None:
                bp["amode"] = "f16"
        if moved and reroute and auto and self.inter_follow_blocks and "inter" in self._h8_sites():
            want = self._inter_pair_set() | {i for i in (self._interaction_of_block(b) for b in moved) if i is not None}
            if want != self._inter_pair_set():
                self._inter_pairs = want
                self._carry_modes = [(bp.get("amode"), bp.get("max_logit", 0.0)) for bp in pk["blocks"]]
                self._packed = None
        return moved

    def attention_modes(self):
        return [(self._attn_mode(bp), bp.get("max_logit", 0.0)) for bp in self._packed["blocks"]] if self._packed else []

    def calibrate_attention(self, x):
        keep = self.attention_guard
        before = [bp.get("amode") for bp in self._packed["blocks"]] if self._packed else None
        self.attention_guard = "sync"
        try:
            self(x)
        finally:
            self.attention_guard = keep
        after = [bp.get("amode") for bp in self._packed["blocks"]]
        return [i for i, m in enumerate(after) if m == "b3" and (before is None or before[i] != "b3")]

    def _msda(self, ap, qn, fn, resid, out, ss, lsi, ref, B, Lq, S, L, colscale=None, stream_out=None, q_rn=None, f_rn=None):
        ws, cfg = self._ws, self.cfg
        M, Pn = cfg["deform_num_heads"], cfg["n_points"]
        dv = ap["val"].n
        vmode = getattr(self, "msda_value", "f32")
        if vmode in ("f16", "f16lo") and not self._wide() and (dv // M) % 8 == 0 and dv % 32 == 0:
            val = ws.planes("msda_valp", B * S, dv, fmt=ops.FMT_H8)
            ops.gemm(fn, ap["val"], bias=ap["val_b"], row_norm=f_rn, out_planes=val)
        else:
            val = ws.get("msda_val", B * S, dv)
            ops.gemm(fn, ap["val"], val, bias=ap["val_b"], row_norm=f_rn)
        raw = ws.get("msda_raw", B * Lq, ap["oa"].n)
        ops.gemm(qn, ap["oa"], raw, bias=ap["oa_b"], row_norm=q_rn)
        samp = ws.planes("msda_s", B * Lq, dv, fmt=ap["out"].fmt)
        ops.msda_fused(val, ss, lsi, raw, ref, None, B, S, M, dv // M, L, Lq, Pn, out_planes=samp, lo_bytes=vmode == "f16lo")
        if stream_out is not None:
            ops.gemm(samp, ap["out"], out, bias=ap["out_b"], resid=resid, colscale=colscale, out_planes=stream_out[0], rowstats_out=stream_out[1])
        else:
            ops.gemm(samp, ap["out"], out, bias=ap["out_b"], resid=resid, colscale=colscale)

    def _c_fold_on(self, rows):
        return bool(self._packed.get("fold_adapter_ln")) and rows % 256 == 0

    def _c_buffers(self, rows, fmt):
        D = self.cfg["embed_dim"]
        return self._ws.planes("inj_fn", rows, D, fmt=fmt), self._ws.get("c_rs", rows, 2 * (D // 64)), self._ws.get("c_mr", rows, 2)

    def _c_produced(self, rows, fmt):
        cp, crs, cmr = self._c_buffers(rows, fmt)
        ops.rowstats_finalize(crs, rows, self.cfg["embed_dim"], 1e-6, cmr)
        self._cfold = dict(planes=cp, mr=cmr)

    def _injector(self, ip, x_in, x_out, c, geo, B, T, Nc):
        ws, D = self._ws, self.cfg["embed_dim"]
        qn = ws.planes("inj_qn", B * T, D, fmt=ip["attn"]["oa"].fmt)
        ops.layernorm(x_in, ip["qnw"], ip["qnb"], 1e-6, out_planes=qn)
        st = self._cfold
        f_rn = None
        if st is not None and "val_cs" in ip["attn"]:
            fn, f_rn = st["planes"], (st["mr"], ip["attn"]["val_cs"])
        else:
            fn = ws.planes("inj_fn", B * Nc, D, fmt=ip["attn"]["val"].fmt)
            if ip["fold_c"]:
                pk = self._packed
                ops.layernorm(c, pk["ln_one"], pk["ln_zero"], 1e-6, out_planes=fn)
            else:
                ops.layernorm(c, ip["fnw"], ip["fnb"], 1e-6, out_planes=fn)
        self._msda(ip["attn"], qn, fn, x_in, x_out, geo["ss1"], geo["lsi1"], geo["ref1"], B, T, Nc, 3, colscale=ip["gamma"],
                   stream_out=(self._stream_planes(B * T, self._packed["blocks"][ip["first_block"]]["qkv"].afmt)
                               if self._packed["fold_ln"] and B * T >= 128 else None), f_rn=f_rn)

    def _extractor(self, ep, c, x, geo, B, T, Nc, H, W, last=False):
        ws, D = self._ws, self.cfg["embed_dim"]
        pk = self._packed
        rows = B * Nc
        fold = self._c_fold_on(rows) and ep["fold_c"]
        cfmt = ep["attn"]["oa"].fmt
        st = self._cfold
        q_rn = None
        if fold and st is not None and "oa_cs" in ep["attn"]:
            qn, q_rn = st["planes"], (st["mr"], ep["attn"]["oa_cs"])
        else:
            qn = ws.planes("inj_fn", rows, D, fmt=cfmt)
            if not (ep["fold_c"] and ep["first"]):
                if ep["fold_c"]:
                    ops.layernorm(c, pk["ln_one"], pk["ln_zero"], 1e-6, out_planes=qn)
                else:
                    ops.layernorm(c, ep["qnw"], ep["qnb"], 1e-6, out_planes=qn)
        fn = ws.planes("inj_qn", B * T, D, fmt=ep["attn"]["val"].fmt)
        ops.layernorm(x, ep["fnw"], ep["fnb"], 1e-6, out_planes=fn)
        produce = fold and (ep["cffn"] or not last)
        if produce:
            cp, crs, _ = self._c_buffers(rows, cfmt)
            self._cfold = None
            self._msda(ep["attn"], qn, fn, c, c, geo["ss2"], geo["lsi2"], geo["ref2"], B, Nc, T, 1, stream_out=(cp, crs), q_rn=q_rn)
            self._c_produced(rows, cfmt)
        else:
            self._cfold = None
            self._msda(ep["attn"], qn, fn, c, c, geo["ss2"], geo["lsi2"], geo["ref2"], B, Nc, T, 1, q_rn=q_rn)
        if not ep["cffn"]:
            return
        hid = ep["fc1"].n
        hp = ep["fc2"].kpad
        h1 = ws.get("ffn_h1", rows, hid)
        h2f = ws.planes(f"ffn_h2_{hp}", rows, hp, zero=True, fmt=ep["fc2"].fmt)
        st = self._cfold
        if st is not None and "fc1_cs" in ep:
            ops.gemm(st["planes"], ep["fc1"], h1, bias=ep["fc1_b"], row_norm=(st["mr"], ep["fc1_cs"]))
        else:
            qn = ws.planes("inj_fn", rows, D, fmt=ep["fc1"].fmt)
            if ep["fold_c"]:
                ops.layernorm(c, pk["ln_one"], pk["ln_zero"], 1e-6, out_planes=qn)
            else:
                ops.layernorm(c, ep["ffw"], ep["ffb"], 1e-6, out_planes=qn)
            ops.gemm(qn, ep["fc1"], h1, bias=ep["fc1_b"])
        off = 0
        for (hh, wwd) in ((H // 8, W // 8), (H // 16, W // 16), (H // 32, W // 32)):
            ops.dwconv(h1[off:], ep["dw"], ep["dw_b"], None, B, hh, wwd, 3, act="gelu",
                       xstride_b=Nc * hid, out_planes=h2f.rows(off), pstride_b=Nc * 2 * hp)
            off += hh * wwd
        self._cfold = None
        if fold and not last:
            cp, crs, _ = self._c_buffers(rows, cfmt)
            ops.gemm(h2f, ep["fc2"], c, bias=ep["fc2_b"], resid=c, out_planes=cp, rowstats_out=crs)
            self._c_produced(rows, cfmt)
        else:
            ops.gemm(h2f, ep["fc2"], c, bias=ep["fc2_b"], resid=c)

    def _spm(self, x, B, H, W, c1_out, cbuf, Nc, join=True):
        pk, ws = self._packed, self._ws
        D = self.cfg["embed_dim"]
        chans = self.channels
        sizes = [(H // 4, W // 4), (H // 8, W // 8), (H // 16, W // 16), (H // 32, W // 32)]
        tcat = [ws.get(f"tcat{i}", B * sizes[i][0] * sizes[i][1], 2 * chans[i]) for i in range(4)]
        tcat_p = [ws.planes(f"tcat{i}", B * sizes[i][0] * sizes[i][1], 2 * chans[i]) if chans[i] % 32 == 0 else None for i in range(4)]
        main = torch.cuda.current_stream()
        multi = getattr(self, "multistream", True)
        if multi:
            if not hasattr(self, "_sides"):
                self._sides = {}
            skey = (getattr(self._ws, "tag", ""), x.device)
            if skey not in self._sides:
                self._sides[skey] = [torch.cuda.Stream(device=x.device) for _ in range(4)]
            s_neck = self._sides[skey]
        else:
            s_neck = [main] * 4
        ev_x = []
        self._twin_batched(x, B, sizes, tcat, ev_x, tcat_p)
        if self._taps is not None:
            for i in range(4):
                self._taps[f"twin{i}"] = tcat[i].clone()
        offs = [0, 0, sizes[1][0] * sizes[1][1], sizes[1][0] * sizes[1][1] + sizes[2][0] * sizes[2][1]]
        joins = []
        for i in range(4):
            sn = s_neck[i]
            sn.wait_event(ev_x[i])
            with torch.cuda.stream(sn):
                if i == 0:
                    self._neck_level(0, pk["neck"][0], tcat[0], B, sizes[0][0], sizes[0][1], chans[0], c1_out, 0, tcat_p[0])
                else:
                    self._neck_level(i, pk["neck"][i], tcat[i], B, sizes[i][0], sizes[i][1], chans[i], cbuf[offs[i]:], Nc * D, tcat_p[i])
                e = torch.cuda.Event()
                e.record(sn)
                joins.append(e)
        if not join:
            return joins
        for e in joins[1:]:
            main.wait_event(e)
        return joins[0]

    def _twin_batched(self, x, B, sizes, tcat, stage_events, tcat_p=None):
        pk, ws = self._packed, self._ws
        chans = self.channels
        st = pk["twin2"]
        t = "cnb_"
        h0, w0 = sizes[0]
        P0 = B * h0 * w0
        kp = st["stem"].kpad
        a = ws.get(t + "stem_a", 2 * P0, kp)
        for si in range(2):
            ops.im2col_nchw(x, 3 * si, 3, 4, a[si * P0:(si + 1) * P0])
        t0 = ws.get(t + "tmp", 2 * P0, chans[0])
        ops.gemm(a, st["stem"], t0, bias=st["stem_b"], batch=2, m=P0, stride_a=P0 * kp, stride_w=st["stem"].n * 2 * kp,
                 stride_bias=chans[0], stride_c=P0 * chans[0])
        cur = ws.get(t + "cur0", 2 * P0, chans[0])
        ops.layernorm(t0, st["stem_nw"], st["stem_nb"], 1e-6, cur, group_rows=P0, w_gstride=chans[0])
        for i in range(4):
            hh, wwd = sizes[i]
            P = B * hh * wwd
            c = chans[i]
            if i >= 1:
                ds = st["ds"][i - 1]
                cp = chans[i - 1]
                Pp = B * sizes[i - 1][0] * sizes[i - 1][1]
                pa = ws.planes(t + "patch", 2 * P, 4 * cp, fmt=ds["w"].fmt)
                ops.layernorm(cur, ds["nw"], ds["nb"], 1e-6, out_planes=pa, patchify=(sizes[i - 1][0], sizes[i - 1][1]),
                              group_rows=Pp, w_gstride=cp)
                cur = ws.get(t + f"cur{i}", 2 * P, c)
                ops.gemm(pa, ds["w"], cur, bias=ds["b"], batch=2, m=P, stride_a=P * 2 * pa.kpad, stride_w=ds["w"].n * 2 * ds["w"].kpad,
                         stride_bias=c, stride_c=P * c)
            d = ws.get(t + "tmp", 2 * P, c)
            wf = st["stages"][i][0]["pw1"].fmt
            n = ws.planes(t + "n", 2 * P, c, fmt=wf)
            hbuf = ws.planes(t + "h", 2 * P, 4 * c, fmt=st["stages"][i][0]["pw2"].fmt)
            fuse_mlp = ops.convnext_mlp_fused_supported(c) and bool(getattr(self, "fuse_convnext_mlp", True))
            fold = "pw1f" in st["stages"][i][0] and not fuse_mlp and hh % 8 == 0 and wwd % 8 == 0 and P >= 128
            if fold:
                rs = ws.get(t + "rs", 2 * P, 2 * (c // 64))
                mr = ws.get(t + "mr", 2 * P, 2)
            for blk in st["stages"][i]:
                if fold:
                    ops.dwconv(cur, blk["dw"], blk["dw_b"], None, 2 * B, hh, wwd, 7, imgs_per_group=B, out_planes=n, rowstats_out=rs)
                    ops.rowstats_finalize(rs, 2 * P, c, 1e-6, mr)
                    ops.gemm(n, blk["pw1f"], bias=blk["pw1_bf"], act="gelu", out_planes=hbuf, row_norm=(mr, blk["pw1_cs"]), batch=2, m=P,
                             stride_a=P * 2 * n.kpad, stride_w=blk["pw1f"].n * 2 * blk["pw1f"].kpad, stride_bias=4 * c, stride_cp=P * 2 * hbuf.kpad)
                    ops.gemm(hbuf, blk["pw2"], cur, bias=blk["pw2_b"], colscale=blk["gamma"], resid=cur, batch=2, m=P,
                             stride_a=P * 2 * hbuf.kpad, stride_w=blk["pw2"].n * 2 * blk["pw2"].kpad, stride_bias=c,
                             stride_r=P * c, stride_c=P * c)
                    continue
                ops.dwconv(cur, blk["dw"], blk["dw_b"], d, 2 * B, hh, wwd, 7, imgs_per_group=B)
                ops.layernorm(d, blk["nw"], blk["nb"], 1e-6, out_planes=n, group_rows=P, w_gstride=c)
                if fuse_mlp:
                    ops.convnext_mlp_fused(n, blk["pw1"], blk["pw2"], blk["pw1_b"], blk["pw2_b"], blk["gamma"], cur, P, batch=2,
                                           stride_a=P * 2 * n.kpad, stride_w1=blk["pw1"].n * 2 * blk["pw1"].kpad,
                                           stride_w2=blk["pw2"].n * 2 * blk["pw2"].kpad, stride_x=P * c)
                    continue
                ops.gemm(n, blk["pw1"], bias=blk["pw1_b"], act="gelu", out_planes=hbuf, batch=2, m=P, stride_a=P * 2 * n.kpad,
                         stride_w=blk["pw1"].n * 2 * blk["pw1"].kpad, stride_bias=4 * c, stride_cp=hbuf.batch_stride(P))
                ops.gemm(hbuf, blk["pw2"], cur, bias=blk["pw2_b"], colscale=blk["gamma"], resid=cur, batch=2, m=P,
                         stride_a=hbuf.batch_stride(P), stride_w=blk["pw2"].batch_stride(blk["pw2"].n), stride_bias=c,
                         stride_r=P * c, stride_c=P * c)
            nw, nb = st["out_norm"][i]
            ops.layernorm(cur, nw, nb, 1e-6, tcat[i], group_rows=P, w_gstride=c, y_gcol=c, y_wrap=True,
                          out_planes=tcat_p[i] if tcat_p is not None else None)
            ev = torch.cuda.Event()
            ev.record(torch.cuda.current_stream())
            stage_events.append(ev)

    def _neck_level(self, level, lv, t, B, h, w, c, out, out_stride_b, tp=None):
        ws = _Tagged(self._ws, f"nk{level}_")
        C = 2 * c
        HW = h * w
        P = B * HW
        gcat = ws.get("nk_g", P, C)
        lcat = ws.get("nk_l", P, C)
        pl_ok = tp is not None and c % 32 == 0
        gcat_p = ws.planes("nk_gp", P, C) if pl_ok else None
        lcat_p = ws.planes("nk_lp", P, C) if pl_ok else None
        n_st, n_g, n_st2 = B * 3 * 3 * c, B * c * c, B * 3 * C
        acc_blk = ws.get("nk_acc", 1, 2 * (n_st + n_g) + n_g + n_st2, dtype=torch.float64)
        ops.zero_(acc_blk[0, :2 * n_st + n_st2])
        gram_scr = ws.get("nk_gscr", 1, (ops.gram_tn_scratch_bytes(B, HW, c) + 3) // 4)
        acc_off = [0, 2 * n_st + n_st2]

        def acc_buf(rows, cols, gram=False):
            o = acc_off[int(gram)]
            acc_off[int(gram)] = o + rows * cols
            return acc_blk[0, o:o + rows * cols].view(rows, cols)
        for m in range(2):
            X = t[:, m * c:(m + 1) * c]
            gp = lv["gfe"][m]
            y = ws.get("nk_y", P, c)
            s = ws.get("nk_s", P, c)
            ops.layernorm(X, gp["nw"], gp["nb"], 1e-5, y, out2=s)
            q2 = ws.get("nk_q2", P, 3 * c)
            if not ("q12" in gp and getattr(self, "fuse_gfe_qkv", True) and ops.gfe_qkv(y, gp["q12"], q2, B, h, w, 32, c // 32, 3 * c // 32)):
                q1 = ws.get("nk_q1", P, 3 * c)
                ops.gconv(y, gp["q1"], None, q1, B, h, w, 32, c // 32, 3 * c // 32, 1)
                ops.gconv(q1, gp["q2"], None, q2, B, h, w, 32, 3 * c // 32, 3 * c // 32, 3)
            st = acc_buf(B * 3, 3 * c)
            ops.colstats(q2, HW * 3 * c, B, HW, st, out_is_zero=True)
            g = acc_buf(B * c, c, gram=True)
            ops.gram_tn(q2[:, :c], q2[:, c:2 * c], HW * 3 * c, g, B, HW, nblk=8, scratch=gram_scr)
            cp = ops.pad32(c)
            pl = ops.Planes(ws.get(f"nk_pp{c}", B * c, 2 * cp, dtype=torch.int16, zero=True), c, c, cp)
            base = st.data_ptr()
            ops.chanattn_build(g, base + 8 * (3 * c), 9 * c, base + 8 * (3 * c + c), 9 * c, gp["temp"], gp["proj"], pl, B, c, 8)
            ops.gemm(q2[:, 2 * c:], pl, gcat[:, m * c:(m + 1) * c], alpha=gp["scale2"], resid=s, batch=B, m=HW,
                     stride_a=HW * 3 * c, stride_w=c * 2 * cp, stride_r=HW * c, stride_c=HW * C,
                     out_planes=gcat_p.cols(m * c, (m + 1) * c) if pl_ok else None, stride_cp=HW * 2 * C)
            lp = lv["loc"][m]
            h1 = ws.get("nk_q1", P, 2 * c)
            h2 = ws.get("nk_q2", P, 2 * c)
            if pl_ok:
                ops.gemm(tp.cols(m * c, (m + 1) * c), lp["w1"], h1, act="relu6")
                h2p = ws.planes("nk_h2p", P, 2 * c)
                ops.dwconv(h1, lp["dw"], None, None, B, h, w, 3, act="relu6", out_planes=h2p)
                ops.gemm(h2p, lp["w3"], alpha=lp["scale"], resid=X, out_planes=lcat_p.cols(m * c, (m + 1) * c))
            else:
                ops.gemm(X, lp["w1"], h1, act="relu6")
                ops.dwconv(h1, lp["dw"], None, h2, B, h, w, 3, act="relu6")
                ops.gemm(h2, lp["w3"], lcat[:, m * c:(m + 1) * c], alpha=lp["scale"], resid=X)
        e = acc_buf(B * c, c, gram=True)
        ops.gram_tn(gcat[:, :c], gcat[:, c:], HW * C, e, B, HW, nblk=1, scratch=gram_scr)
        cp = ops.pad32(c)
        px = ops.Planes(ws.get(f"nk_pp{c}", B * c, 2 * cp, dtype=torch.int16, zero=True), c, c, cp)
        py = ops.Planes(ws.get(f"nk_pp2{c}", B * c, 2 * cp, dtype=torch.int16, zero=True), c, c, cp)
        ops.gffm_build(e, px, py, B, c)
        fbuf = ws.get("nk_f", P, C)
        ops.gemm(gcat_p.cols(c, C) if pl_ok else gcat[:, c:], px, fbuf[:, :c], alpha=lv["gx"], resid=gcat[:, :c], batch=B, m=HW,
                 stride_a=HW * C * (2 if pl_ok else 1), stride_w=c * 2 * cp, stride_r=HW * C, stride_c=HW * C)
        ops.gemm(gcat_p.cols(0, c) if pl_ok else gcat[:, :c], py, fbuf[:, c:], alpha=lv["gy"], resid=gcat[:, c:], batch=B, m=HW,
                 stride_a=HW * C * (2 if pl_ok else 1), stride_w=c * 2 * cp, stride_r=HW * C, stride_c=HW * C)
        st = acc_buf(B * 3, C)
        ops.colstats(fbuf, HW * C, B, HW, st, wrow=lv["lnw"], out_is_zero=True)
        mean = ws.get("nk_mean", B, C)
        rstd = ws.get("nk_rstd", B, C)
        mult = ws.get("nk_mult", B, C)
        ops.ffrm_finalize(st, B, HW, C, lv["lnw_mean"], lv["lnb_mean"], lv["ffrm_w"], lv["gn_w"], lv["gn_b"], mean, rstd, mult,
                          ws.get("nk_ffrm", 2 * B, C))
        fn = ws.get("nk_g", P, C)
        ops.lnhw_apply(fbuf, mean, rstd, mult, lv["lnw"], lv["lnb"], fn, B, HW)
        hm = ws.get("nk_hm", P, 2 * C)
        ops.gemm(lcat_p if pl_ok else lcat, lv["mlp_in"], hm)
        hg = ws.planes("nk_hg", P, C)
        ops.dwpair_gate(hm, lv["mlp_dw"], None, B, h, w, C, out_planes=hg)
        z = ws.get("nk_f", P, C)
        ops.gemm(hg, lv["mlp_out"], z, alpha=lv["s2"], resid=fn, beta=lv["s1"])
        pooled = ws.get("nk_pool", B * (h + w), C)
        ops.pool_hw(z, pooled, B, h, w)
        y1 = ws.get(f"nk_y1_{lv['mip_pad']}", B * (h + w), lv["mip_pad"], zero=True)
        ops.gemm(pooled, lv["ca1"], y1, bias=lv["ca1_b"], act="hswish")
        att = ws.get("nk_att", B * (h + w), C)
        ops.gemm(y1, lv["cah"], att, bias=lv["cah_b"], act="sigmoid", batch=B, m=h,
                 stride_a=(h + w) * lv["mip_pad"], stride_c=(h + w) * C)
        ops.gemm(y1[h:], lv["caw"], att[h:], bias=lv["caw_b"], act="sigmoid", batch=B, m=w,
                 stride_a=(h + w) * lv["mip_pad"], stride_c=(h + w) * C)
        if pl_ok:
            zo = ws.planes("nk_zop", P, C)
            ops.ca_apply(z, att, None, B, h, w, out_planes=zo)
            sa = HW * 2 * C
        else:
            zo = ws.get("nk_g", P, C)
            ops.ca_apply(z, att, zo, B, h, w)
            sa = HW * C
        if self._taps is not None:
            self._taps[f"fuse{level}"] = ops.planes_to_float(zo, cols=C) if pl_ok else zo[:, :C].clone()
        if out_stride_b == 0:
            ops.gemm(zo, lv["fc"], out, bias=lv["fc_b"])
        else:
            ops.gemm(zo, lv["fc"], out, bias=lv["fc_b"], batch=B, m=HW, stride_a=sa, stride_c=out_stride_b)


class SAMAdapterbimodalMixModNewInTwinConvNEWwithcp(SAMAdapterbimodalMixModNewInTwinConvNEW):
    """Second registered name (backbones/__init__.py:3-9): identical inference math, extra training-only kwargs."""


def _ref_points(shapes):
    refs = []
    for (h, w) in shapes:
        ys = torch.linspace(0.5, h - 0.5, h, dtype=torch.float32) / h
        xs = torch.linspace(0.5, w - 0.5, w, dtype=torch.float32) / w
        gy, gx = torch.meshgrid(ys, xs, indexing="ij")
        refs.append(torch.stack((gx.reshape(-1), gy.reshape(-1)), -1))
    return torch.cat(refs, 0).contiguous()


def rel_pos_index(q_size, k_size):
    q = torch.arange(q_size)[:, None] * max(k_size / q_size, 1.0)
    k = torch.arange(k_size)[None, :] * max(q_size / k_size, 1.0)
    return ((q - k) + (k_size - 1) * max(q_size / k_size, 1.0)).long()


def _rel_table(size, rel_pos):
    L = 2 * size - 1
    tab = rel_pos if rel_pos.shape[0] == L else _linear_resize_rows(rel_pos, L)
    return tab[rel_pos_index(size, size).to(tab.device)].contiguous()


def _cubic_w(t, A=-0.75):
    def c1(x):
        return ((A + 2) * x - (A + 3)) * x * x + 1

    def c2(x):
        return ((A * x - 5 * A) * x + 8 * A) * x - 4 * A
    return torch.stack([c2(t + 1), c1(t), c1(1 - t), c2(2 - t)], -1)


def _bicubic_matrix(n_in, n_out, device):
    scale = n_in / n_out
    x = (torch.arange(n_out, dtype=torch.float32, device=device) + 0.5) * scale - 0.5
    ix = x.floor()
    w = _cubic_w(x - ix)
    m = torch.zeros(n_out, n_in, dtype=torch.float32, device=device)
    for k in range(4):
        idx = (ix.long() - 1 + k).clamp(0, n_in - 1)
        m.scatter_add_(1, idx[:, None], w[:, k:k + 1])
    return m


def _bicubic_resize(src_hwc, H, W):
    h, w, _ = src_hwc.shape
    if (h, w) == (H, W):
        return src_hwc.contiguous()
    my = _bicubic_matrix(h, H, src_hwc.device)
    mx = _bicubic_matrix(w, W, src_hwc.device)
    return torch.einsum("Hh,hwc,Ww->HWc", my, src_hwc, mx).contiguous()
```

### multimodal-sam-adapter_amd/mmsa/lib.py

```python
import ctypes
import os
from ctypes import c_char_p, c_double, c_float, c_int, c_long, c_void_p, POINTER

_HERE = os.path.dirname(os.path.abspath(__file__))
LIB_PATH = os.environ.get("MMSA_LIB") or os.path.join(_HERE, "libmmsa_hip.so")

if not os.path.exists(LIB_PATH):
    raise RuntimeError(
        f"{LIB_PATH} not found: the MI355X HIP library is required (no CPU/PyTorch fallback exists). "
        "Build it with: python multimodal-sam-adapter_amd/build.py")

import torch

_lib = ctypes.CDLL(LIB_PATH)

P = c_void_p
I = c_int
L = c_long
F = c_float

_PAINT_TAIL = [P, I, P, I, I, I, I, I, P, P, I, I, c_double, c_double, c_double, c_double, P, P]
SIGNATURES = {
    "mmsa_version": [],
    "mmsa_last_error": [],
    "mmsa_debug_poison_lds": [ctypes.c_uint, P],
    "mmsa_event_create": [POINTER(c_void_p)],
    "mmsa_event_record": [P, P],
    "mmsa_event_elapsed_ms": [P, P, POINTER(c_float)],
    "mmsa_event_destroy": [P],
    "mmsa_ms_deform_attn_forward": [P, P, P, P, P, P, I, I, I, I, I, I, I, I, I, P],
    "mmsa_ms_deform_attn_backward": [P, P, P, P, P, P, P, P, P, I, I, I, I, I, I, I, I, I, P],
    "mmsa_msda_fused": [P, P, P, P, L, P, P, L, P, L, I, I, I, I, I, I, I, I, P, P],
    "mmsa_msda_fused_planes": [P, L, I, P, P, P, L, P, P, L, P, L, I, I, I, I, I, I, I, I, P, P],
    "mmsa_gemm_split3": [P, P, L, L, P, L, P, L, P, P, L, L, I, F, P, L, L, P, L, L, I, I, I, I, I, F, I, I, I, I, I, I, I, P, P, P, I, P, P],
    "mmsa_convnext_mlp_fused": [P, L, L, P, L, P, L, P, P, P, P, L, L, I, I, I, I, I, P, P],
    "mmsa_rowstats_finalize": [P, I, I, I, F, P, P],
    "mmsa_zero_bytes": [P, ctypes.c_size_t, P],
    "mmsa_split_planes": [P, L, I, I, I, P, I, P, P],
    "mmsa_attention": [P, L, P, P, P, L, I, I, I, I, I, I, F, P],
    "mmsa_attention_planes": [P, L, P, P, P, L, I, I, I, I, I, I, F, I, I, P, P],
    "mmsa_relpos_bias": [P, L, P, P, P, I, I, I, I, I, I, P],
    "mmsa_relpos_bias_planes": [P, L, P, P, P, I, I, I, I, I, I, P],
    "mmsa_layernorm_rows": [P, L, P, P, F, P, L, P, L, P, L, I, I, I, I, I, I, L, L, I, I, P, P],
    "mmsa_colstats": [P, L, L, P, I, I, I, P, I, P],
    "mmsa_ffrm_finalize": [P, I, I, I, F, F, P, P, P, P, P, P, P, P],
    "mmsa_lnhw_apply": [P, L, P, P, P, P, P, P, L, I, I, I, P],
    "mmsa_dwconv_nhwc": [P, L, L, P, P, P, L, L, P, L, L, I, I, I, I, I, I, I, I, P, P, P],
    "mmsa_dwpair_gate": [P, L, P, P, L, P, L, I, I, I, I, P],
    "mmsa_gconv_nhwc": [P, L, P, P, P, L, I, I, I, I, I, I, I, I, P],
    "mmsa_gfe_qkv_conv": [P, L, P, P, L, I, I, I, I, I, I, POINTER(c_int), P],
    "mmsa_im2col_nchw": [P, I, I, I, I, I, I, I, P, I, P],
    "mmsa_gram_tn": [P, L, P, L, L, P, I, I, I, I, P, L, P],
    "mmsa_gram_tn_scratch_bytes": [I, I, I],
    "mmsa_chanattn_build": [P, P, L, P, L, P, P, P, I, I, I, I, P],
    "mmsa_gffm_build": [P, P, P, I, I, I, P],
    "mmsa_gelu_gate": [P, L, P, L, L, I, P],
    "mmsa_pool_hw": [P, L, P, L, I, I, I, I, P],
    "mmsa_ca_apply": [P, L, P, L, P, L, P, L, I, I, I, I, P],
    "mmsa_tail_fuse": [P, L, L, P, L, P, P, P, P, L, I, I, I, I, I, I, P],
    "mmsa_global_attention_planes": [P, L, P, P, P, L, I, I, I, I, I, F, I, I, P, P],
    "mmsa_window_attention_planes": [P, L, P, P, P, P, L, I, I, I, I, I, I, F, I, I, P, P],
    "mmsa_nchw_to_planes": [P, L, P, L, I, I, L, P],
    "mmsa_head_fuse": [P, P, I, I, P, I, I, P, I, I, L, P, P, P, L, P, L, I, I, I, I, I, P],
    "mmsa_tokens_to_nchw": [P, L, P, I, L, I, P],
    "mmsa_bilinear_accum_nchw": [P, L, I, I, I, I, P, I, I, I, I, I, I, P, I, P],
    "mmsa_div_count_nchw": [P, P, I, I, L, P],
    "mmsa_argmax_nchw": [P, P, I, I, L, P],
    "mmsa_crop_batch_nchw": [P, I, I, I, I, P, I, P, I, I, P],
    "mmsa_slide_argmax": [P, I, I, I, I, P, P, I, I, I, I, I, P, P],
    "mmsa_slide_argmax_resized": [P, I, I, I, I, P, P, I, I, I, I, I, I, I, I, I, P, P],
    "mmsa_softmax_flip_accum_nchw": [P, P, I, I, I, I, I, I, I, P],
    "mmsa_aug_argmax": [P, P, I, I, P, P, I, P, I, I, I, P, P],
    "mmsa_argmax_max_nchw": [P, P, P, I, I, L, P],
    "mmsa_slide_argmax_conf": [P, I, I, I, I, P, P, P, I, I, I, I, I, P, P],
    "mmsa_slide_argmax_resized_conf": [P, I, I, I, I, P, P, P, I, I, I, I, I, I, I, I, I, P, P],
    "mmsa_aug_argmax_conf": [P, P, I, I, P, P, I, P, P, I, I, I, P, P],
    "mmsa_preprocess_nhwc": [P, I, P, I, I, I, I, P, P, P, P, P, P, I, I, P],
    "mmsa_preprocess_crops": [P, I, P, I, I, I, I, P, P, P, P, P, I, I, P, I, P, I, I, P],
    "mmsa_preprocess_resize_nhwc": [P, I, P, I, I, I, I, P, P, P, P, P, P, I, I, I, I, P, P, P, P, I, P],
    "mmsa_preprocess_resize_crops": [P, I, P, I, I, I, I, P, P, P, P, P, I, I, P, I, P, I, I, I, I, P, P, P, P, I, P],
    "mmsa_eval_confusion_u8": [P, P, I, I, I, I, I, P, I, P, P, P, I, P, P],
    "mmsa_eval_calibration": [P, P, P, I, I, I, I, I, P, I, P, P, P, I, I, P, P],
    "mmsa_eval_selective": [P, P, P, I, I, I, I, I, P, I, P, P, P, I, I, P, P],
    "mmsa_abstain_u8": [P, P, L, I, I, P, P],
    "mmsa_slide_argmax_conf_t": [P, I, I, I, I, P, P, P, I, I, I, I, I, P, F, P],
    "mmsa_slide_argmax_resized_conf_t": [P, I, I, I, I, P, P, P, I, I, I, I, I, I, I, I, I, P, F, P],
    "mmsa_softmax_flip_accum_nchw_t": [P, P, I, I, I, I, I, I, I, F, P],
    "mmsa_temperature_sweep_nchw": [P, P, I, I, I, I, I, I, P, P, P, P, I, P, I, I, P, P],
    "mmsa_argmax_score_nchw": [P, P, P, I, I, I, I, I, F, P],
    "mmsa_slide_argmax_score": [P, I, I, I, I, P, P, P, I, I, I, I, I, P, I, F, F, P],
    "mmsa_slide_argmax_resized_score": [P, I, I, I, I, P, P, P, I, I, I, I, I, I, I, I, I, P, I, F, F, P],
    "mmsa_slide_argmax_topk": [P, I, I, I, I, P, P, P, I, I, I, I, I, P, I, F, P],
    "mmsa_argmax_topk_nchw": [P, P, P, P, I, I, I, I, I, P],
    "mmsa_eval_topk_u8": [P, I, P, I, I, I, I, I, P, I, P, P, P, I, P, P],
    "mmsa_eval_boundary_u8": [P, P, I, I, I, I, I, P, I, P, P, P, I, I, I, P, P],
    "mmsa_boundary_distance_u8": [P, I, I, I, P, P, P, I, I, I, I, P, P, P],
    "mmsa_eval_boundary_d2": [P, P, I, I, I, I, I, P, I, P, P, P, I, P, P, I, P, P],
    "mmsa_eval_boundary_displacement": [P, P, I, I, I, I, I, P, I, P, P, P, I, P, P, I, P, P],
    "mmsa_components_u8": [P, I, I, I, P, P, P, I, I, I, P, P],
    "mmsa_component_area": [P, I, I, I, P, P],
    "mmsa_suppress_small_u8": [P, P, P, I, I, I, I, I, P, P],
    "mmsa_eval_segments": [P, P, I, I, I, I, I, P, I, P, P, P, I, P, P, I, P, P, P],
    "mmsa_segment_pairs": [P, P, I, I, P, I, P, P, P, P, I, I, I, P, P, L, P, P],
    "mmsa_eval_panoptic": [P, P, I, I, I, I, I, P, I, P, P, P, I, P, P, P, P, P, L, P, P, P],
    "mmsa_slide_argmax_eval": [P, I, I, I, I, P, P, I, I, I, I, I, P, P, I, I, P, P, P, P, I, P, P],
    "mmsa_render_u8": [P, L, L, I, I, I, P, I, I, P, I, I, I, c_double, c_double, P, P],
    "mmsa_render_denorm_f32": [P, L, L, I, I, I, P, I, I, P, I, I, I, P, P, I, I, c_double, c_double, P, P],
    "mmsa_render_labels_u8": [P, L, L, P, I, I, I, I, I, P, I, P, P, I, I] + _PAINT_TAIL,
    "mmsa_render_values_f32": [P, P, L, L, I, I, I, I, I] + _PAINT_TAIL,
    "mmsa_render_band_u8": [P, L, L, P, I, I, I, I, I, P, I, P, P, I, I, I, I, I] + _PAINT_TAIL,
}
_RESTYPES = {"mmsa_last_error": c_char_p, "mmsa_gram_tn_scratch_bytes": c_long}

for _name, _args in SIGNATURES.items():
    _fn = getattr(_lib, _name)
    _fn.argtypes = _args
    _fn.restype = _RESTYPES.get(_name, c_int)


ABI_VERSION = 114
if _lib.mmsa_version() != ABI_VERSION:
    raise RuntimeError(f"{LIB_PATH}: ABI version {_lib.mmsa_version()} but mmsa/lib.py binds version {ABI_VERSION} (include/mmsa.h MMSA_ABI_VERSION): "
                       "rebuild with python multimodal-sam-adapter_amd/build.py")


def last_error() -> str:
    return _lib.mmsa_last_error().decode()


POISON_LDS = os.environ.get("MMSA_DEBUG_POISON_LDS") == "1"


def call(name, *args):
    if POISON_LDS and not name.startswith(("mmsa_event", "mmsa_debug")) and args:
        _lib.mmsa_debug_poison_lds(0x7FC07FC0, args[-1])
    rc = getattr(_lib, name)(*args)
    if rc != 0:
        raise RuntimeError(f"{name} failed (rc={rc}): {last_error()}")


def version() -> int:
    return _lib.mmsa_version()


raw = _lib
```

### multimodal-sam-adapter_amd/mmsa/ops.py

```python
import ctypes

import os

import torch

from . import lib

ACT = {"none": 0, "gelu": 1, "relu": 2, "relu6": 3, "hswish": 4, "sigmoid": 5}

GEMM_PROFILE = None
CLAMP_WATCH = None
GEMM_MAX_GRID = 0
GEMM_FLAVOUR = 0
GEMM_SHAPES = None


def _event():
    ev = ctypes.c_void_p()
    lib.call("mmsa_event_create", ctypes.byref(ev))
    return ev


def collect_gemm_profile(prof):
    flops, ms = 0.0, 0.0
# ... 347 lines not shown
    if out_planes is not None:
        pp, _, _, ldp = out_planes.mat("y planes")
    mh, mw = patchify or (0, 0)
    lib.call("mmsa_layernorm_rows", px, ldx, _chk(w), _chk(b), eps, py, ldy, p2, ld2, pp, ldp, rows, c,
             1 if patchify else 0, mh, mw, group_rows, w_gstride, y_gcol, 1 if y_wrap else 0,
             out_planes.fmt if out_planes is not None else FMT_B3, _clamp_ptr(), _stream())
    return out if out is not None else out_planes


MSDA_DTYPES = {torch.float32: 0, torch.float16: 1, torch.float64: 2}


def _msda_args(value, spatial_shapes, level_start_index, sampling_loc, attn_weight, extra=()):
    dt = value.dtype
    if dt not in MSDA_DTYPES:
        raise RuntimeError(f"ms_deform_attn: dtype {dt} not supported (float32, float16, float64)")
    for t, n in ((value, "value"), (sampling_loc, "sampling_loc"), (attn_weight, "attn_weight")) + tuple(extra):
        if not t.is_contiguous():
            raise RuntimeError(f"{n} tensor has to be contiguous")
        if t.dtype != dt:
            raise RuntimeError(f"{n} must have the dtype of value ({dt}), got {t.dtype}")
    if not (spatial_shapes.is_contiguous() and level_start_index.is_contiguous()):
        raise RuntimeError("spatial_shapes / level_start_index tensor has to be contiguous")
    return dt


def msda_forward(value, spatial_shapes, level_start_index, sampling_loc, attn_weight, im2col_step=64):
    dt = _msda_args(value, spatial_shapes, level_start_index, sampling_loc, attn_weight)
    n, s, m, d = value.shape
    _, lq, _, l, p, _ = sampling_loc.shape
    out = torch.empty(n, lq, m * d, dtype=dt, device=value.device)
    lib.call("mmsa_ms_deform_attn_forward", _chk(value, dt), _chk(spatial_shapes, torch.int64), _chk(level_start_index, torch.int64),
             _chk(sampling_loc, dt), _chk(attn_weight, dt), out.data_ptr(), n, s, m, d, l, lq, p, im2col_step, MSDA_DTYPES[dt], _stream())
    return out


def msda_backward(value, spatial_shapes, level_start_index, sampling_loc, attn_weight, grad_output, im2col_step=64):
    dt = _msda_args(value, spatial_shapes, level_start_index, sampling_loc, attn_weight, extra=((grad_output, "grad_output"),))
    n, s, m, d = value.shape
    _, lq, _, l, p, _ = sampling_loc.shape
    if tuple(grad_output.shape) != (n, lq, m * d):
        raise RuntimeError(f"grad_output must be [{n}, {lq}, {m * d}], got {tuple(grad_output.shape)}")
    gv, gl, ga = torch.empty_like(value), torch.empty_like(sampling_loc), torch.empty_like(attn_weight)
    lib.call("mmsa_ms_deform_attn_backward", _chk(value, dt), _chk(spatial_shapes, torch.int64), _chk(level_start_index, torch.int64),
             _chk(sampling_loc, dt), _chk(attn_weight, dt), _chk(grad_output, dt), gv.data_ptr(), gl.data_ptr(), ga.data_ptr(),
             n, s, m, d, l, lq, p, im2col_step, MSDA_DTYPES[dt], _stream())
    return [gv, gl, ga]


def msda_fused(value2d, spatial_shapes, level_start_index, raw, ref_points, out, batch, spatial, heads, d, levels, lq, points,
               out_planes=None, lo_bytes=False):
    pr, _, _, ldraw = _mat(raw, "raw")
    if isinstance(value2d, Planes):
        if value2d.fmt != FMT_H8 or value2d.weight or value2d.split:
            raise RuntimeError("mmsa.msda_fused: value planes must be H8 activation planes")
        pvp, _, _, ldvp = value2d.mat("value planes")
        po, ldo = None, 0
        if out is not None:
            po, _, _, ldo = _mat(out, "out")
        pp, ldp = None, 0
        if out_planes is not None:
            pp, _, _, ldp = out_planes.mat("out planes")
        lib.call("mmsa_msda_fused_planes", pvp, ldvp, 1 if lo_bytes else 0, _chk(spatial_shapes, torch.int64), _chk(level_start_index, torch.int64), pr, ldraw,
                 _chk(ref_points), po, ldo, pp, ldp, out_planes.fmt if out_planes is not None else FMT_B3,
                 batch, spatial, heads, d, levels, lq, points, _clamp_ptr(), _stream())
        return out if out is not None else out_planes
    pv, vrows, vcols, ldv = _mat(value2d, "value")
    if vrows != batch * spatial or vcols != heads * d or (vrows > 1 and ldv != heads * d):
        raise RuntimeError(f"mmsa.msda_fused: value must be a dense [batch * spatial, heads * d] = [{batch * spatial}, {heads * d}] matrix, "
                           f"got shape {tuple(value2d.shape)} with row stride {ldv}")
    po, ldo = None, 0
    if out is not None:
        po, _, _, ldo = _mat(out, "out")
    pp, ldp = None, 0
    if out_planes is not None:
        pp, _, _, ldp = out_planes.mat("out planes")
    lib.call("mmsa_msda_fused", pv, _chk(spatial_shapes, torch.int64), _chk(level_start_index, torch.int64), pr, ldraw,
             _chk(ref_points), po, ldo, pp, ldp, out_planes.fmt if out_planes is not None else FMT_B3,
             batch, spatial, heads, d, levels, lq, points, _clamp_ptr(), _stream())
    return out if out is not None else out_planes


def relpos_bias(qkv, rh, rw, rp, b, h, w, heads, hd, ws):
    if isinstance(qkv, Planes):
        pq, _, _, ldq = qkv.mat("qkv")
        lib.call("mmsa_relpos_bias_planes", pq, ldq, _chk(rh), _chk(rw), _chk(rp), b, h, w, heads, hd, ws, _stream())
    else:
        pq, _, _, ldq = _mat(qkv, "qkv")
        lib.call("mmsa_relpos_bias", pq, ldq, _chk(rh), _chk(rw), _chk(rp), b, h, w, heads, hd, ws, _stream())
    return rp


def _v_fmt(qkv, qkv_bias, d, fused=False, rel=None):
    if qkv.fmt == FMT_H8 or qkv_bias.fmt == FMT_H8 or (rel is not None and rel.fmt == FMT_H8):
        if not (fused and qkv.fmt == FMT_H8 and qkv_bias.fmt == FMT_H8 and rel is not None and rel.fmt == FMT_H8
                and not (qkv.weight or qkv_bias.weight or rel.weight)):
            raise RuntimeError("mmsa attention: h8 planes need the fused rel-pos entry with qkv, bias AND rel-pos planes in the h8 (activation) format")
        return 2
    if qkv.split != qkv_bias.split or qkv.split not in (0, 2 * d) or (fused and qkv.split):
        raise RuntimeError(f"mmsa attention: qkv planes (split {qkv.split}) and bias planes (split {qkv_bias.split}) must both be f3 (fp16 hi/lo) "
                           f"planes, either plain or -- for the entry with a rel-pos prepass -- with the v columns from {2 * d} on as h8 planes")
    if qkv.fmt != FMT_F3 or qkv_bias.fmt != FMT_F3 or (rel is not None and rel.fmt != FMT_F3):
        raise RuntimeError("mmsa attention: the hi/lo operand form of the attention kernels reads f3 planes (fp16 hi/lo pairs: ops.FMT_F3) since round 4 -- "
                           "qkv, bias and rel-pos planes; bf16 hi/lo planes have the same layout and would be misread")
    return 1 if qkv.split else 0


def split_planes_qkv(x2d, d):
    if (2 * d) % 32 or d % 32:
        raise RuntimeError("mmsa.split_planes_qkv: embed dim must be a multiple of 32")
    qk = split_planes(x2d[:, :2 * d].contiguous(), fmt=FMT_F3)
    v = split_planes(x2d[:, 2 * d:].contiguous(), fmt=FMT_H8)
    return Planes(torch.cat([qk.p, v.p], 1).contiguous(), x2d.shape[0], 3 * d, 3 * d, FMT_F3, split=2 * d)


def _guard(g):
    if g is None:
        return None
    if g.dtype != torch.float32 or g.numel() != 1 or not g.is_cuda:
        raise RuntimeError("mmsa attention: max_logit must be a 1-element fp32 device tensor")
    return g.data_ptr()


def attention(qkv, qkv_bias, rp, out, b, h, w, heads, hd, ws, scale, max_logit=None):
    if isinstance(qkv, Planes):
        pq, _, _, ldq = qkv.mat("qkv")
        po, _, _, ldo = out.mat("out")
        lib.call("mmsa_attention_planes", pq, ldq, _chk(qkv_bias.p, torch.int16), _chk(rp),
                 po, ldo, b, h, w, heads, hd, ws, scale, out.fmt, _v_fmt(qkv, qkv_bias, heads * hd), _guard(max_logit), _stream())
    else:
        pq, _, _, ldq = _mat(qkv, "qkv")
        po, _, _, ldo = _mat(out, "out")
        lib.call("mmsa_attention", pq, ldq, _chk(qkv_bias), _chk(rp), po, ldo, b, h, w, heads, hd, ws, scale, _stream())
    return out


def window_relpos_planes(rel_pos_h, rel_pos_w, ws, fmt=FMT_B3):
    L = 2 * ws - 1
    if rel_pos_h.shape[0] != L or rel_pos_w.shape[0] != L or L > 27:
        raise RuntimeError(f"mmsa.window_relpos_planes: tables must have {L} <= 27 rows")
    m = torch.zeros(64, rel_pos_h.shape[1], dtype=torch.float32, device=rel_pos_h.device)
    m[:L] = rel_pos_h
    m[32:32 + L] = rel_pos_w
    return split_planes(m, fmt=fmt)


def global_relpos_planes(rel_pos_h, rel_pos_w, fmt=FMT_B3):
    if rel_pos_h.shape[0] > 127 or rel_pos_w.shape[0] > 127:
        raise RuntimeError("mmsa.global_relpos_planes: tables must have at most 127 rows")
    m = torch.zeros(256, rel_pos_h.shape[1], dtype=torch.float32, device=rel_pos_h.device)
    m[:rel_pos_h.shape[0]] = rel_pos_h
    m[128:128 + rel_pos_w.shape[0]] = rel_pos_w
    return split_planes(m, fmt=fmt)


def global_attention(qkv, qkv_bias, relg, out, b, h, w, heads, hd, scale, max_logit=None):
    pq, _, _, ldq = qkv.mat("qkv")
    po, _, _, ldo = out.mat("out")
    lib.call("mmsa_global_attention_planes", pq, ldq, _chk(qkv_bias.p, torch.int16), _chk(relg.p, torch.int16), po, ldo,
             b, h, w, heads, hd, scale, out.fmt, _v_fmt(qkv, qkv_bias, heads * hd, fused=True, rel=relg), _guard(max_logit), _stream())
    return out


_SELECTORS = {}


def window_selector(ws, device, f16=False):
    key = (ws, str(device), f16)
    if key not in _SELECTORS:
        sel = torch.zeros(208, 32, dtype=torch.int16)
        j = torch.arange(min(ws * ws, 208))
        one = 0x3C00
        sel[j, j // ws] = one
        sel[j, 14 + j % ws] = one
        _SELECTORS[key] = sel.to(device)
    return _SELECTORS[key]


def window_attention(qkv, qkv_bias, relp, out, b, h, w, heads, hd, ws, scale, max_logit=None):
    if not 1 <= ws <= 14:
        raise RuntimeError(f"mmsa.window_attention: window_size {ws} not supported (1..14)")
    pq, _, _, ldq = qkv.mat("qkv")
    po, _, _, ldo = out.mat("out")
    vf = _v_fmt(qkv, qkv_bias, heads * hd, fused=True, rel=relp)
    lib.call("mmsa_window_attention_planes", pq, ldq, _chk(qkv_bias.p, torch.int16), _chk(relp.p, torch.int16),
             _chk(window_selector(ws, qkv.p.device, f16=vf == 2), torch.int16), po, ldo, b, h, w, heads, hd, ws, scale, out.fmt,
             vf, _guard(max_logit), _stream())
    return out


def colstats(x, stride_b, b, hw, out, wrow=None, out_is_zero=False):
    px, _, c, ldx = _mat(x, "x")
    lib.call("mmsa_colstats", px, ldx, stride_b, _chk(wrow), b, hw, c, _chk(out, torch.float64), int(out_is_zero), _stream())
    return out


def ffrm_finalize(stats, b, hw, c, mean_w, mean_b, wc, gn_w, gn_b, mean_o, rstd_o, mult_o, scratch):
    lib.call("mmsa_ffrm_finalize", _chk(stats, torch.float64), b, hw, c, mean_w, mean_b, _chk(wc), _chk(gn_w), _chk(gn_b),
             _chk(mean_o), _chk(rstd_o), _chk(mult_o), _chk(scratch), _stream())


def lnhw_apply(x, mean, rstd, mult, w, bias, out, b, hw):
    px, _, c, ldx = _mat(x, "x")
    po, _, _, ldo = _mat(out, "y")
    lib.call("mmsa_lnhw_apply", px, ldx, _chk(mean), _chk(rstd), _chk(mult), _chk(w), _chk(bias), po, ldo, b, hw, c, _stream())
    return out


def dwconv(x, w, bias, out, b, h, wd, k, act="none", xstride_b=None, ystride_b=None, out_planes=None, pstride_b=None,
           imgs_per_group=0, rowstats_out=None):
    px, _, c, ldx = _mat(x, "x")
    po, ldo = None, 0
    if out is not None:
        po, _, _, ldo = _mat(out, "y")
    pp, ldp = None, 0
    if out_planes is not None:
        pp, _, _, ldp = out_planes.mat("y planes")
    xs = h * wd * ldx if xstride_b is None else xstride_b
    ys = h * wd * ldo if ystride_b is None else ystride_b
    ps = h * wd * ldp if pstride_b is None else pstride_b
    lib.call("mmsa_dwconv_nhwc", px, ldx, xs, _chk(w), _chk(bias), po, ldo, ys, pp, ldp, ps, out_planes.fmt if out_planes is not None else FMT_B3,
             b, h, wd, c, k, ACT[act], imgs_per_group, _chk(rowstats_out), _clamp_ptr(), _stream())
    return out if out is not None else out_planes


def gconv(x, w, bias, out, b, h, wd, groups, cin_g, cout_g, k, act="none"):
    px, _, _, ldx = _mat(x, "x")
    po, _, _, ldo = _mat(out, "y")
    lib.call("mmsa_gconv_nhwc", px, ldx, _chk(w), _chk(bias), po, ldo, b, h, wd, groups, cin_g, cout_g, k, ACT[act], _stream())


def gfe_qkv(x, w12, out, b, h, wd, groups, cin_g, cout_g):
    px, _, _, ldx = _mat(x, "x")
    po, _, _, ldo = _mat(out, "y")
    covered = ctypes.c_int(0)
    lib.call("mmsa_gfe_qkv_conv", px, ldx, _chk(w12), po, ldo, b, h, wd, groups, cin_g, cout_g, ctypes.byref(covered), _stream())
    return bool(covered.value)
    return out


def dwpair_gate(x, w_tap, out, b, h, wd, c, out_planes=None):
    px, _, _, ldx = _mat(x, "x")
    po, ldo = (None, 0)
    if out is not None:
        po, _, _, ldo = _mat(out, "y")
    pp, ldp = (None, 0)
    if out_planes is not None:
        pp, _, _, ldp = out_planes.mat("y planes")
    lib.call("mmsa_dwpair_gate", px, ldx, _chk(w_tap), po, ldo, pp, ldp, b, h, wd, c, _stream())
    return out if out is not None else out_planes


def im2col_nchw(x, c0, cin, p, out):
    b, ctot, h, w = x.shape
    if not x.is_contiguous():
        raise RuntimeError("mmsa.im2col_nchw: input image must be contiguous NCHW")
    po, _, kpad, ld = _mat(out, "out")
    if ld != kpad:
        raise RuntimeError("mmsa.im2col_nchw: output must be dense")
    lib.call("mmsa_im2col_nchw", _chk(x), b, ctot, c0, cin, h, w, p, po, kpad, _stream())
    return out


def gram_tn_scratch_bytes(b, p, c):
    return int(lib.raw.mmsa_gram_tn_scratch_bytes(b, p, c))


def gram_tn(x, y, stride_b, g, b, p, nblk=1, scratch=None):
    px, _, c, ldx = _mat(x, "X")
    py, _, _, ldy = _mat(y, "Y")
    need = gram_tn_scratch_bytes(b, p, c)
    if scratch is None:
        scratch = torch.empty((need + 3) // 4, dtype=torch.float32, device=x.device)
    if not scratch.is_cuda or not scratch.is_contiguous():
        raise RuntimeError("gram_tn: scratch must be a contiguous device tensor")
    lib.call("mmsa_gram_tn", px, ldx, py, ldy, stride_b, _chk(g, torch.float64, "G"), b, p, c, nblk, scratch.data_ptr(),
             scratch.numel() * scratch.element_size(), _stream())
    return g


def chanattn_build(g, sq, sq_stride, sk, sk_stride, temp, wp, planes, b, c, heads):
    lib.call("mmsa_chanattn_build", _chk(g, torch.float64, "G"), sq, sq_stride, sk, sk_stride, _chk(temp), _chk(wp),
             planes.p.data_ptr(), b, c, planes.kpad, heads, _stream())


def gffm_build(e, px_, py_, b, c):
    lib.call("mmsa_gffm_build", _chk(e, torch.float64, "E"), px_.p.data_ptr(), py_.p.data_ptr(), b, c, px_.kpad, _stream())


def gelu_gate(x, out, c):
    px, rows, _, ldx = _mat(x, "x")
    po, _, _, ldo = _mat(out, "y")
    lib.call("mmsa_gelu_gate", px, ldx, po, ldo, rows, c, _stream())
    return out


def pool_hw(z, out, b, h, w):
    pz, _, c, ldz = _mat(z, "z")
    po, _, _, ldo = _mat(out, "out")
    lib.call("mmsa_pool_hw", pz, ldz, po, ldo, b, h, w, c, _stream())
    return out


def ca_apply(z, att, out, b, h, w, out_planes=None):
    pz, _, c, ldz = _mat(z, "z")
    pa, _, _, lda = _mat(att, "att")
    po, ldo = (None, 0)
    if out is not None:
        po, _, _, ldo = _mat(out, "out")
    pp, ldp = (None, 0)
    if out_planes is not None:
        pp, _, _, ldp = out_planes.mat("out planes")
    lib.call("mmsa_ca_apply", pz, ldz, pa, lda, po, ldo, pp, ldp, b, h, w, c, _stream())
    return out if out is not None else out_planes


def tail_fuse(cmap, cstride_b, xtok, bn_scale, bn_shift, out, b, hc, wc, hx, wx, out_planes=None):
    pc, _, c, ldc = _mat(cmap, "cmap")
    px, ldx = None, 0
    if xtok is not None:
        px, _, _, ldx = _mat(xtok, "xtok")
    pp, ldp = (out_planes.p.data_ptr(), 2 * out_planes.kpad) if out_planes is not None else (None, 0)
    lib.call("mmsa_tail_fuse", pc, ldc, cstride_b, px, ldx, _chk(bn_scale), _chk(bn_shift), _chk(out), pp, ldp, b, hc, wc, hx, wx, c, _stream())
    return out
```

Before: 67.00.

## Store the 1/4-res map in 2x2-block-major rows and tile the head fuse

The c1 feature map and the neck ca_apply output are now stored in 2x2-block-major row order. This lets the up-conv GEMM write its output as a plain contiguous matrix instead of going through a pixel-shuffle epilogue, and lets tail_fuse read that layout directly. Separately, head_fuse gets a tiled kernel that stages the coarse-level halos in LDS, so the bilinear taps no longer gather from global memory for every pixel. The change adds layout-conversion paths for the debug taps, and any consumer that still assumes raster order would be a correctness risk.

```diff
diff --git a/include/mmsa.h b/include/mmsa.h
--- a/include/mmsa.h
+++ b/include/mmsa.h
@@ -126,10 +126,16 @@
 int mmsa_pool_hw(const float* z, long ldz, float* out, long ldo, int B, int H, int W, int C, mmsa_stream_t stream);
 int mmsa_ca_apply(const float* z, long ldz, const float* att, long lda, float* out, long ldo,
                   uint16_t* out_planes, long ldp , int B, int H, int W, int C, mmsa_stream_t stream);
+enum { MMSA_ROWS_RASTER = 0, MMSA_ROWS_BLOCK2 = 1 };
+int mmsa_ca_apply_rows(const float* z, long ldz, const float* att, long lda, float* out, long ldo,
+                       uint16_t* out_planes, long ldp, int B, int H, int W, int C, int out_rows , mmsa_stream_t stream);
 
 int mmsa_tail_fuse(const float* cmap, long ldc, long cstrideB, const float* xtok, long ldx, const float* bn_scale,
                    const float* bn_shift, float* out, uint16_t* out_planes , long ldp,
                    int B, int Hc, int Wc, int Hx, int Wx, int C, mmsa_stream_t stream);
+int mmsa_tail_fuse_rows(const float* cmap, long ldc, long cstrideB, const float* xtok, long ldx, const float* bn_scale,
+                        const float* bn_shift, float* out, uint16_t* out_planes, long ldp,
+                        int B, int Hc, int Wc, int Hx, int Wx, int C, int cmap_rows , mmsa_stream_t stream);
 
 int mmsa_global_attention_planes(const uint16_t* qkv_planes, long ldq, const uint16_t* bias_planes, const uint16_t* relpos_planes,
                                  uint16_t* out_planes, long ldo, int B, int H, int W, int heads, int head_dim, float scale,
diff --git a/multimodal-sam-adapter_amd/csrc/common.h b/multimodal-sam-adapter_amd/csrc/common.h
--- a/multimodal-sam-adapter_amd/csrc/common.h
+++ b/multimodal-sam-adapter_amd/csrc/common.h
@@ -107,6 +107,8 @@
 }
 
 __host__ __device__ __forceinline__ int ilv(int k) { return ((k >> 5) << 6) | (k & 31); }
+
+__host__ __device__ __forceinline__ int block2_row(int h, int w, int W) { return (((h >> 1) * (W >> 1) + (w >> 1)) << 2) | ((h & 1) << 1) | (w & 1); }
 
 #define MMSA_CP_BASE(f_) ((f_) & 0xff)
 #define MMSA_CP_SPLIT(f_) (((f_) >> 8) * 32)
diff --git a/multimodal-sam-adapter_amd/csrc/head.hip b/multimodal-sam-adapter_amd/csrc/head.hip
--- a/multimodal-sam-adapter_amd/csrc/head.hip
+++ b/multimodal-sam-adapter_amd/csrc/head.hip
@@ -79,6 +79,39 @@
   float rh[3], rw[3];
 };
 
+__device__ __forceinline__ void head_fuse_px8(float (&v)[8], const float4 (&t)[3][2][4], const float (&lh)[3], const float (&lw)[3], int nlv,
+                                              const float4 s0, const float4 s1, const float4 f0, const float4 f1, int act, uint4& hi, uint4& lo) {
+#pragma unroll
+  for (int i = 0; i < 3; ++i) {
+    if (i < nlv) {
+      const float w00 = (1.f - lh[i]) * (1.f - lw[i]), w01 = (1.f - lh[i]) * lw[i], w10 = lh[i] * (1.f - lw[i]), w11 = lh[i] * lw[i];
+#pragma unroll
+      for (int hh = 0; hh < 2; ++hh) {
+        const float4 t00 = t[i][hh][0], t01 = t[i][hh][1], t10 = t[i][hh][2], t11 = t[i][hh][3];
+        v[4 * hh + 0] += w00 * t00.x + w01 * t01.x + w10 * t10.x + w11 * t11.x;
+        v[4 * hh + 1] += w00 * t00.y + w01 * t01.y + w10 * t10.y + w11 * t11.y;
+        v[4 * hh + 2] += w00 * t00.z + w01 * t01.z + w10 * t10.z + w11 * t11.z;
+        v[4 * hh + 3] += w00 * t00.w + w01 * t01.w + w10 * t10.w + w11 * t11.w;
+      }
+    }
+  }
+  const float bs[8] = {s0.x, s0.y, s0.z, s0.w, s1.x, s1.y, s1.z, s1.w}, bf[8] = {f0.x, f0.y, f0.z, f0.w, f1.x, f1.y, f1.z, f1.w};
+#pragma unroll
+  for (int j = 0; j < 8; ++j) v[j] = apply_act(v[j] * bs[j] + bf[j], act);
+  split2(v[0], v[1], hi.x, lo.x);
+  split2(v[2], v[3], hi.y, lo.y);
+  split2(v[4], v[5], hi.z, lo.z);
+  split2(v[6], v[7], hi.w, lo.w);
+}
+
+__device__ __forceinline__ void head_tap(int x, float r, int n, int& x0, int& x1, float& l) {
+  float s = ((float)x + 0.5f) * r - 0.5f;
+  s = s < 0.f ? 0.f : s;
+  x0 = min((int)s, n - 1);
+  x1 = x0 + (x0 < n - 1 ? 1 : 0);
+  l = s - (float)x0;
+}
+
 __global__ __launch_bounds__(256) void head_fuse_kernel(const float* __restrict__ z0, long ld, HeadLevels lv, int nlv,
                                                         const float* __restrict__ bn_scale, const float* __restrict__ bn_shift,
                                                         uint16_t* __restrict__ planes, long ldp, float* __restrict__ out32, long ldo,
@@ -96,14 +129,9 @@
 #pragma unroll
   for (int i = 0; i < 3; ++i) {
     if (i < nlv) {
-      float sh = ((float)h + 0.5f) * lv.rh[i] - 0.5f;
-      float sw = ((float)w + 0.5f) * lv.rw[i] - 0.5f;
-      sh = sh < 0.f ? 0.f : sh;
-      sw = sw < 0.f ? 0.f : sw;
-      const int h0 = min((int)sh, lv.H[i] - 1), w0 = min((int)sw, lv.W[i] - 1);
-      const int h1 = h0 + (h0 < lv.H[i] - 1 ? 1 : 0), w1 = w0 + (w0 < lv.W[i] - 1 ? 1 : 0);
-      lh[i] = sh - (float)h0;
-      lw[i] = sw - (float)w0;
+      int h0, h1, w0, w1;
+      head_tap(h, lv.rh[i], lv.H[i], h0, h1, lh[i]);
+      head_tap(w, lv.rw[i], lv.W[i], w0, w1, lw[i]);
       const long base = (long)b * lv.H[i] * lv.W[i];
       o00[i] = (base + (long)h0 * lv.W[i] + w0) * ld;
       o01[i] = (base + (long)h0 * lv.W[i] + w1) * ld;
@@ -134,33 +162,125 @@
     const float4 f0 = *reinterpret_cast<const float4*>(bn_shift + c), f1 = *reinterpret_cast<const float4*>(bn_shift + c + 4);
     __builtin_amdgcn_sched_barrier(0);
     v[0] = a.x; v[1] = a.y; v[2] = a.z; v[3] = a.w; v[4] = d.x; v[5] = d.y; v[6] = d.z; v[7] = d.w;
-#pragma unroll
-    for (int i = 0; i < 3; ++i) {
-      if (i < nlv) {
-        const float w00 = (1.f - lh[i]) * (1.f - lw[i]), w01 = (1.f - lh[i]) * lw[i], w10 = lh[i] * (1.f - lw[i]), w11 = lh[i] * lw[i];
-#pragma unroll
-        for (int hh = 0; hh < 2; ++hh) {
-          const float4 t00 = t[i][hh][0], t01 = t[i][hh][1], t10 = t[i][hh][2], t11 = t[i][hh][3];
-          v[4 * hh + 0] += w00 * t00.x + w01 * t01.x + w10 * t10.x + w11 * t11.x;
-          v[4 * hh + 1] += w00 * t00.y + w01 * t01.y + w10 * t10.y + w11 * t11.y;
-          v[4 * hh + 2] += w00 * t00.z + w01 * t01.z + w10 * t10.z + w11 * t11.z;
-          v[4 * hh + 3] += w00 * t00.w + w01 * t01.w + w10 * t10.w + w11 * t11.w;
-        }
-      }
-    }
-    const float bs[8] = {s0.x, s0.y, s0.z, s0.w, s1.x, s1.y, s1.z, s1.w}, bf[8] = {f0.x, f0.y, f0.z, f0.w, f1.x, f1.y, f1.z, f1.w};
-#pragma unroll
-    for (int j = 0; j < 8; ++j) v[j] = apply_act(v[j] * bs[j] + bf[j], act);
+    uint4 hi, lo;
+    head_fuse_px8(v, t, lh, lw, nlv, s0, s1, f0, f1, act, hi, lo);
     if (out32) {
       *reinterpret_cast<float4*>(out32 + pixg * ldo + c) = make_float4(v[0], v[1], v[2], v[3]);
       *reinterpret_cast<float4*>(out32 + pixg * ldo + c + 4) = make_float4(v[4], v[5], v[6], v[7]);
     }
     if (planes) {
-      uint4 hi, lo;
-      split2(v[0], v[1], hi.x, lo.x);
-      split2(v[2], v[3], hi.y, lo.y);
-      split2(v[4], v[5], hi.z, lo.z);
-      split2(v[6], v[7], hi.w, lo.w);
+      uint16_t* row = planes + pixg * ldp + ilv(c);
+      *reinterpret_cast<uint4*>(row) = hi;
+      *reinterpret_cast<uint4*>(row + 32) = lo;
+    }
+  }
+}
+
+#define HEAD_TILE 16
+#define HEAD_TILE_CH 64
+#define HEAD_HALO_ITEMS 10
+struct HeadTiles {
+  int halo[3];
+  int shift[3];
+  int rcp[3];
+  int at4[3];
+  int tot4;
+};
+
+template <int ACT>
+__global__ __launch_bounds__(256) void head_fuse_tiles_kernel(const float* __restrict__ z0, long ld, HeadLevels lv, HeadTiles tl, int nlv,
+                                                              const float* __restrict__ bn_scale, const float* __restrict__ bn_shift,
+                                                              uint16_t* __restrict__ planes, long ldp, float* __restrict__ out32, long ldo,
+                                                              int H, int W, int C, int act_arg) {
+  const int act = ACT >= 0 ? ACT : act_arg;
+  __shared__ float4 halo[256 * HEAD_HALO_ITEMS];
+  const int t = threadIdx.x;
+  const int nch = C / HEAD_TILE_CH;
+  const int ch0 = (int)(blockIdx.x % nch) * HEAD_TILE_CH;
+  const int tile = blockIdx.x / nch;
+  const int tw = W / HEAD_TILE;
+  const int ty0 = (tile / tw) * HEAD_TILE, tx0 = (tile % tw) * HEAD_TILE;
+  const int b = blockIdx.y;
+  auto halo_src = [&](int j) -> const float4* {
+    const int idx = min(t + 256 * j, tl.tot4 - 1);
+    const bool l1 = idx >= tl.at4[1], l2 = idx >= tl.at4[2];
+#define HEAD_PICK(a_) (l2 ? a_[2] : l1 ? a_[1] : a_[0])
+    const int loc = idx - HEAD_PICK(tl.at4);
+    const int hs = HEAD_PICK(tl.halo), rcp = HEAD_PICK(tl.rcp), sft = HEAD_PICK(tl.shift), Hi = HEAD_PICK(lv.H), Wi = HEAD_PICK(lv.W);
+    const float* zi = HEAD_PICK(lv.z);
+#undef HEAD_PICK
+    const int p = loc >> 4, c4 = loc & 15;
+    const int hy = (p * rcp) >> 11, hx = p - hy * hs;
+    const int row = min(max((ty0 >> sft) - 1 + hy, 0), Hi - 1), col = min(max((tx0 >> sft) - 1 + hx, 0), Wi - 1);
+    return reinterpret_cast<const float4*>(zi + (((long)b * Hi + row) * Wi + col) * ld + ch0 + 4 * c4);
+  };
+  const float4 hv0 = *halo_src(0), hv1 = *halo_src(1), hv2 = *halo_src(2), hv3 = *halo_src(3), hv4 = *halo_src(4);
+  const float4 hv5 = *halo_src(5), hv6 = *halo_src(6), hv7 = *halo_src(7), hv8 = *halo_src(8), hv9 = *halo_src(9);
+  static_assert(HEAD_HALO_ITEMS == 10, "ten halo registers");
+  const int l8 = t & 7, pg = t >> 3;
+  const int c = ch0 + 8 * l8;
+  const int py = pg >> 4, px = pg & 15;
+  const int w = tx0 + px;
+  float4 a[8], d[8];
+#pragma unroll
+  for (int k = 0; k < 8; ++k) {
+    const long pixg = ((long)b * H + ty0 + 2 * k + py) * W + w;
+    a[k] = *reinterpret_cast<const float4*>(z0 + pixg * ld + c);
+    d[k] = *reinterpret_cast<const float4*>(z0 + pixg * ld + c + 4);
+  }
+  const float4 s0 = *reinterpret_cast<const float4*>(bn_scale + c), s1 = *reinterpret_cast<const float4*>(bn_scale + c + 4);
+  const float4 f0 = *reinterpret_cast<const float4*>(bn_shift + c), f1 = *reinterpret_cast<const float4*>(bn_shift + c + 4);
+  __builtin_amdgcn_sched_barrier(0);
+#define HEAD_PUT(j_) halo[min(t + 256 * j_, tl.tot4 - 1)] = hv##j_;
+  HEAD_PUT(0) HEAD_PUT(1) HEAD_PUT(2) HEAD_PUT(3) HEAD_PUT(4) HEAD_PUT(5) HEAD_PUT(6) HEAD_PUT(7) HEAD_PUT(8) HEAD_PUT(9)
+#undef HEAD_PUT
+  __syncthreads();
+  int q0[3], q1[3];
+  float lh[3], lw[3];
+#pragma unroll
+  for (int i = 0; i < 3; ++i) {
+    q0[i] = q1[i] = 0; lh[i] = lw[i] = 0.f;
+    if (i < nlv) {
+      int w0, w1;
+      head_tap(w, lv.rw[i], lv.W[i], w0, w1, lw[i]);
+      const int ox = (tx0 >> tl.shift[i]) - 1;
+      q0[i] = min(max(w0 - ox, 0), tl.halo[i] - 1);
+      q1[i] = min(max(w1 - ox, 0), tl.halo[i] - 1);
+    }
+  }
+#pragma unroll
+  for (int k = 0; k < 8; ++k) {
+    const int h = ty0 + 2 * k + py;
+    float4 tp[3][2][4];
+#pragma unroll
+    for (int i = 0; i < 3; ++i) {
+      if (i < nlv) {
+        int h0, h1;
+        head_tap(h, lv.rh[i], lv.H[i], h0, h1, lh[i]);
+        const int oy = (ty0 >> tl.shift[i]) - 1;
+        const int r0 = min(max(h0 - oy, 0), tl.halo[i] - 1) * tl.halo[i], r1 = min(max(h1 - oy, 0), tl.halo[i] - 1) * tl.halo[i];
+        const float4* im = halo + tl.at4[i] + 2 * l8;
+#pragma unroll
+        for (int hh = 0; hh < 2; ++hh) {
+          tp[i][hh][0] = im[(r0 + q0[i]) * 16 + hh];
+          tp[i][hh][1] = im[(r0 + q1[i]) * 16 + hh];
+          tp[i][hh][2] = im[(r1 + q0[i]) * 16 + hh];
+          tp[i][hh][3] = im[(r1 + q1[i]) * 16 + hh];
+        }
+      } else {
+#pragma unroll
+        for (int hh = 0; hh < 2; ++hh) tp[i][hh][0] = tp[i][hh][1] = tp[i][hh][2] = tp[i][hh][3] = make_float4(0.f, 0.f, 0.f, 0.f);
+      }
+    }
+    float v[8] = {a[k].x, a[k].y, a[k].z, a[k].w, d[k].x, d[k].y, d[k].z, d[k].w};
+    uint4 hi, lo;
+    head_fuse_px8(v, tp, lh, lw, nlv, s0, s1, f0, f1, act, hi, lo);
+    const long pixg = ((long)b * H + h) * W + w;
+    if (out32) {
+      *reinterpret_cast<float4*>(out32 + pixg * ldo + c) = make_float4(v[0], v[1], v[2], v[3]);
+      *reinterpret_cast<float4*>(out32 + pixg * ldo + c + 4) = make_float4(v[4], v[5], v[6], v[7]);
+    }
+    if (planes) {
       uint16_t* row = planes + pixg * ldp + ilv(c);
       *reinterpret_cast<uint4*>(row) = hi;
       *reinterpret_cast<uint4*>(row + 32) = lo;
@@ -195,6 +315,35 @@
   }
   const long npix = (long)B * H * W;
   MMSA_CHECK_ARG(npix < (1L << 31), "head_fuse: too many pixels for the 32-bit index arithmetic");
+  HeadTiles tl;
+  bool tiles = MMSA_KNOB("MMSA_HEAD_ROWS", 0) == 0 && H % HEAD_TILE == 0 && W % HEAD_TILE == 0 && C % HEAD_TILE_CH == 0 && B < 65536 &&
+               (long)(H / HEAD_TILE) * (W / HEAD_TILE) * (C / HEAD_TILE_CH) < (1L << 31) &&
+               ((((uintptr_t)z1) | ((uintptr_t)z2) | ((uintptr_t)z3) | ((uintptr_t)out32) | ((uintptr_t)planes)) & 15) == 0 &&
+               (!planes || ldp % 8 == 0);
+  tl.tot4 = 0;
+  for (int i = 0; i < 3; ++i) {
+    tl.halo[i] = 4; tl.rcp[i] = 512; tl.shift[i] = 3; tl.at4[i] = i == 0 ? 0 : 0x7fffffff;
+    if (i >= n || !tiles) continue;
+    int s = 0;
+    for (int k = 1; k <= 3; ++k)
+      if (((long)lv.H[i] << k) == H && ((long)lv.W[i] << k) == W) s = k;
+    if (!s) { tiles = false; continue; }
+    tl.shift[i] = s;
+    tl.halo[i] = (HEAD_TILE >> s) + 2;
+    tl.rcp[i] = (2048 + tl.halo[i] - 1) / tl.halo[i];
+    tl.at4[i] = tl.tot4;
+    tl.tot4 += tl.halo[i] * tl.halo[i] * (HEAD_TILE_CH / 4);
+  }
+  if (tiles && tl.tot4 <= 256 * HEAD_HALO_ITEMS) {
+    if (n == 0) { lv.z[0] = z0; lv.H[0] = H; lv.W[0] = W; tl.tot4 = 1; }
+    dim3 grid((unsigned)((H / HEAD_TILE) * (W / HEAD_TILE) * (C / HEAD_TILE_CH)), B);
+    if (act == ACT_RELU)
+      hipLaunchKernelGGL(head_fuse_tiles_kernel<ACT_RELU>, grid, dim3(256), 0, stream, z0, ld, lv, tl, n, bn_scale, bn_shift, planes, ldp, out32, ldo, H, W, C, act);
+    else
+      hipLaunchKernelGGL(head_fuse_tiles_kernel<-1>, grid, dim3(256), 0, stream, z0, ld, lv, tl, n, bn_scale, bn_shift, planes, ldp, out32, ldo, H, W, C, act);
+    MMSA_CHECK_LAUNCH("head_fuse");
+    return MMSA_OK;
+  }
   hipLaunchKernelGGL(head_fuse_kernel, dim3(cdiv(npix, 4)), dim3(256), 0, stream, z0, ld, lv, n, bn_scale, bn_shift, planes, ldp,
                      out32, ldo, H, W, C, npix, act);
   MMSA_CHECK_LAUNCH("head_fuse");
diff --git a/multimodal-sam-adapter_amd/csrc/neck.hip b/multimodal-sam-adapter_amd/csrc/neck.hip
--- a/multimodal-sam-adapter_amd/csrc/neck.hip
+++ b/multimodal-sam-adapter_amd/csrc/neck.hip
@@ -337,7 +337,7 @@
 
 __global__ __launch_bounds__(256) void ca_apply_kernel(const float* __restrict__ z, long ldz, const float* __restrict__ att, long lda,
                                                        float* __restrict__ out, long ldo, unsigned short* __restrict__ outp, long ldp,
-                                                       int H, int W, int C, long total4) {
+                                                       int H, int W, int C, long total4, int block2) {
   const unsigned c4n = C >> 2;
   for (unsigned i = blockIdx.x * blockDim.x + threadIdx.x; i < (unsigned)total4; i += gridDim.x * blockDim.x) {
     const unsigned rowu = i / c4n;
@@ -355,11 +355,12 @@
     o.y = v.y + v.y * aw.y * ah.y;
     o.z = v.z + v.z * aw.z * ah.z;
     o.w = v.w + v.w * aw.w * ah.w;
-    if (out) *reinterpret_cast<float4*>(out + row * ldo + c) = o;
+    const long orow = block2 ? (long)b * H * W + block2_row(h, w, W) : row;
+    if (out) *reinterpret_cast<float4*>(out + orow * ldo + c) = o;
     if (outp) {
       uint2 h2, l2;
       split4(o, h2, l2);
-      unsigned short* q_ = outp + row * ldp + ilv(c);
+      unsigned short* q_ = outp + orow * ldp + ilv(c);
       *reinterpret_cast<uint2*>(q_) = h2;
       *reinterpret_cast<uint2*>(q_ + 32) = l2;
     }
@@ -368,13 +369,21 @@
 
 extern "C" int mmsa_ca_apply(const float* z, long ldz, const float* att, long lda, float* out, long ldo,
                              unsigned short* out_planes, long ldp, int B, int H, int W, int C, hipStream_t stream) {
+  return mmsa_ca_apply_rows(z, ldz, att, lda, out, ldo, out_planes, ldp, B, H, W, C, MMSA_ROWS_RASTER, stream);
+}
+
+extern "C" int mmsa_ca_apply_rows(const float* z, long ldz, const float* att, long lda, float* out, long ldo,
+                                  unsigned short* out_planes, long ldp, int B, int H, int W, int C, int out_rows, hipStream_t stream) {
+  MMSA_CHECK_ARG(out_rows == MMSA_ROWS_RASTER || (out_rows == MMSA_ROWS_BLOCK2 && H % 2 == 0 && W % 2 == 0),
+                 "ca_apply: row order %d of a %d x %d map (2 x 2-block-major rows need even sides)", out_rows, H, W);
   MMSA_CHECK_ARG(z && att && (out || out_planes) && (C & 3) == 0 && (ldz & 3) == 0 && (lda & 3) == 0 && (ldo & 3) == 0, "ca_apply: bad args");
   MMSA_CHECK_ARG(!out_planes || ((((uintptr_t)out_planes) & 127) == 0 && (ldp & 63) == 0 && ldp >= 2L * ((C + 31) / 32 * 32)), "ca_apply: bad output planes");
   const long total4 = (long)B * H * W * (C >> 2);
   MMSA_CHECK_ARG(total4 < (1L << 31), "ca_apply: too many elements for the 32-bit index arithmetic");
   int blocks = cdiv(total4, 256);
   if (blocks > 8192) blocks = 8192;
-  hipLaunchKernelGGL(ca_apply_kernel, dim3(blocks), dim3(256), 0, stream, z, ldz, att, lda, out, ldo, out_planes, ldp, H, W, C, total4);
+  hipLaunchKernelGGL(ca_apply_kernel, dim3(blocks), dim3(256), 0, stream, z, ldz, att, lda, out, ldo, out_planes, ldp, H, W, C, total4,
+                     out_rows == MMSA_ROWS_BLOCK2 ? 1 : 0);
   MMSA_CHECK_LAUNCH("ca_apply");
   return MMSA_OK;
 }
diff --git a/multimodal-sam-adapter_amd/csrc/tail.hip b/multimodal-sam-adapter_amd/csrc/tail.hip
--- a/multimodal-sam-adapter_amd/csrc/tail.hip
+++ b/multimodal-sam-adapter_amd/csrc/tail.hip
@@ -3,7 +3,7 @@
 __global__ __launch_bounds__(256) void tail_fuse_kernel(const float* __restrict__ cmap, long ldc, long cstrideB, const float* __restrict__ xtok, long ldx,
                                                         const float* __restrict__ bn_scale, const float* __restrict__ bn_shift,
                                                         float* __restrict__ out, unsigned short* __restrict__ outp, long ldp,
-                                                        int Hc, int Wc, int Hx, int Wx, int C, float rh, float rw) {
+                                                        int Hc, int Wc, int Hx, int Wx, int C, float rh, float rw, int block2) {
   __shared__ float tile[32][33];
   const int b = blockIdx.z;
   const int pix0 = blockIdx.x * 32;
@@ -18,7 +18,7 @@
     float v = 0.f;
     if (pix < npix && c < C) {
       const int h = pix / Wc, w = pix - h * Wc;
-      v = cmap[(long)b * cstrideB + (long)pix * ldc + c];
+      v = cmap[(long)b * cstrideB + (long)(block2 ? block2_row(h, w, Wc) : pix) * ldc + c];
       float sh = ((float)h + 0.5f) * rh - 0.5f;
       float sw = ((float)w + 0.5f) * rw - 0.5f;
       sh = sh < 0.f ? 0.f : sh;
@@ -30,10 +30,11 @@
         const float* xb = xtok + (long)b * Hx * Wx * ldx + c;
         const float v00 = xb[((long)h0 * Wx + w0) * ldx], v01 = xb[((long)h0 * Wx + w1) * ldx];
         const float v10 = xb[((long)h1 * Wx + w0) * ldx], v11 = xb[((long)h1 * Wx + w1) * ldx];
-        const float r = (1.f - lh) * ((1.f - lw) * v00 + lw * v01) + lh * ((1.f - lw) * v10 + lw * v11);
+        const float top = fmaf(v01, lw, (1.f - lw) * v00), bot = fmaf(v11, lw, (1.f - lw) * v10);
+        const float r = fmaf(1.f - lh, top, lh * bot);
         v = v + r;
       }
-      v = v * bn_scale[c] + bn_shift[c];
+      v = fmaf(v, bn_scale[c], bn_shift[c]);
       if (outp) {
         unsigned short hh, ll;
         split_bf16(v, hh, ll);
@@ -57,7 +58,7 @@
 __global__ __launch_bounds__(256) void tail_fuse64_kernel(const float* __restrict__ cmap, long ldc, long cstrideB, const float* __restrict__ xtok, long ldx,
                                                           const float* __restrict__ bn_scale, const float* __restrict__ bn_shift,
                                                           float* __restrict__ out, unsigned short* __restrict__ outp, long ldp,
-                                                          int Hc, int Wc, int Hx, int Wx, int C, float rh, float rw) {
+                                                          int Hc, int Wc, int Hx, int Wx, int C, float rh, float rw, int block2) {
   __shared__ float tile[64][65];
   const int b = blockIdx.z;
   const int pix0 = blockIdx.x * 64, c0 = blockIdx.y * 64;
@@ -77,7 +78,7 @@
     const bool ok = pix < npix && c_ok;
     if (ok) {
       const int h = pix / Wc, w = pix - h * Wc;
-      v = *reinterpret_cast<const float4*>(cmap + (long)b * cstrideB + (long)pix * ldc + c);
+      v = *reinterpret_cast<const float4*>(cmap + (long)b * cstrideB + (long)(block2 ? block2_row(h, w, Wc) : pix) * ldc + c);
       float sh = ((float)h + 0.5f) * rh - 0.5f;
       float sw = ((float)w + 0.5f) * rw - 0.5f;
       sh = sh < 0.f ? 0.f : sh;
@@ -88,11 +89,12 @@
       if (xtok) {
         const float4 v00 = *reinterpret_cast<const float4*>(xb + ((long)h0 * Wx + w0) * ldx), v01 = *reinterpret_cast<const float4*>(xb + ((long)h0 * Wx + w1) * ldx);
         const float4 v10 = *reinterpret_cast<const float4*>(xb + ((long)h1 * Wx + w0) * ldx), v11 = *reinterpret_cast<const float4*>(xb + ((long)h1 * Wx + w1) * ldx);
-#define TF_ONE(f_) { const float r_ = (1.f - lh) * ((1.f - lw) * v00.f_ + lw * v01.f_) + lh * ((1.f - lw) * v10.f_ + lw * v11.f_); v.f_ = (v.f_ + r_) * sc.f_ + sf.f_; }
+#define TF_ONE(f_) { const float top_ = fmaf(v01.f_, lw, (1.f - lw) * v00.f_), bot_ = fmaf(v10.f_, 1.f - lw, lw * v11.f_); \
+                     const float r_ = fmaf(1.f - lh, top_, lh * bot_); v.f_ = fmaf(v.f_ + r_, sc.f_, sf.f_); }
         TF_ONE(x) TF_ONE(y) TF_ONE(z) TF_ONE(w)
 #undef TF_ONE
       } else {
-        v.x = v.x * sc.x + sf.x; v.y = v.y * sc.y + sf.y; v.z = v.z * sc.z + sf.z; v.w = v.w * sc.w + sf.w;
+        v.x = fmaf(v.x, sc.x, sf.x); v.y = fmaf(v.y, sc.y, sf.y); v.z = fmaf(v.z, sc.z, sf.z); v.w = fmaf(v.w, sc.w, sf.w);
       }
     }
     if (outp) {
@@ -125,6 +127,15 @@
 extern "C" int mmsa_tail_fuse(const float* cmap, long ldc, long cstrideB, const float* xtok, long ldx, const float* bn_scale,
                               const float* bn_shift, float* out, unsigned short* out_planes, long ldp, int B, int Hc, int Wc,
                               int Hx, int Wx, int C, hipStream_t stream) {
+  return mmsa_tail_fuse_rows(cmap, ldc, cstrideB, xtok, ldx, bn_scale, bn_shift, out, out_planes, ldp, B, Hc, Wc, Hx, Wx, C, MMSA_ROWS_RASTER, stream);
+}
+
+extern "C" int mmsa_tail_fuse_rows(const float* cmap, long ldc, long cstrideB, const float* xtok, long ldx, const float* bn_scale,
+                                   const float* bn_shift, float* out, unsigned short* out_planes, long ldp, int B, int Hc, int Wc,
+                                   int Hx, int Wx, int C, int cmap_rows, hipStream_t stream) {
+  MMSA_CHECK_ARG(cmap_rows == MMSA_ROWS_RASTER || (cmap_rows == MMSA_ROWS_BLOCK2 && Hc % 2 == 0 && Wc % 2 == 0),
+                 "tail_fuse: row order %d of a %d x %d map (2 x 2-block-major rows need even sides)", cmap_rows, Hc, Wc);
+  const int b2 = cmap_rows == MMSA_ROWS_BLOCK2 ? 1 : 0;
   MMSA_CHECK_ARG(cmap && bn_scale && bn_shift && out, "tail_fuse: null pointer");
   MMSA_CHECK_ARG(B > 0 && Hc > 0 && Wc > 0 && Hx > 0 && Wx > 0 && C > 0, "tail_fuse: bad shape");
   MMSA_CHECK_ARG(!out_planes || ((C & 31) == 0 && ldp >= 2L * C), "tail_fuse: planes output needs C % 32 == 0 and ldp >= 2C");
@@ -135,12 +146,12 @@
                     (!out_planes || ((C & 7) == 0 && (ldp & 7) == 0 && (((uintptr_t)out_planes) & 15) == 0));
   if (wide) {
     dim3 grid64(cdiv((long)Hc * Wc, 64), cdiv(C, 64), B);
-    hipLaunchKernelGGL(tail_fuse64_kernel, grid64, dim3(256), 0, stream, cmap, ldc, cstrideB, xtok, ldx, bn_scale, bn_shift, out, out_planes, ldp, Hc, Wc, Hx, Wx, C, rh, rw);
+    hipLaunchKernelGGL(tail_fuse64_kernel, grid64, dim3(256), 0, stream, cmap, ldc, cstrideB, xtok, ldx, bn_scale, bn_shift, out, out_planes, ldp, Hc, Wc, Hx, Wx, C, rh, rw, b2);
     MMSA_CHECK_LAUNCH("tail_fuse");
     return MMSA_OK;
   }
   dim3 grid(cdiv((long)Hc * Wc, 32), cdiv(C, 32), B);
-  hipLaunchKernelGGL(tail_fuse_kernel, grid, dim3(256), 0, stream, cmap, ldc, cstrideB, xtok, ldx, bn_scale, bn_shift, out, out_planes, ldp, Hc, Wc, Hx, Wx, C, rh, rw);
+  hipLaunchKernelGGL(tail_fuse_kernel, grid, dim3(256), 0, stream, cmap, ldc, cstrideB, xtok, ldx, bn_scale, bn_shift, out, out_planes, ldp, Hc, Wc, Hx, Wx, C, rh, rw, b2);
   MMSA_CHECK_LAUNCH("tail_fuse");
   return MMSA_OK;
 }
diff --git a/multimodal-sam-adapter_amd/mmsa/backbone.py b/multimodal-sam-adapter_amd/mmsa/backbone.py
--- a/multimodal-sam-adapter_amd/mmsa/backbone.py
+++ b/multimodal-sam-adapter_amd/mmsa/backbone.py
@@ -186,6 +186,16 @@
 
     fuse_gfe_qkv = True
 
+    c1_block_major = True
+
+    def _c1_rows(self):
+        return ops.ROWS_BLOCK2 if self.c1_block_major else ops.ROWS_RASTER
+
+    @staticmethod
+    def _raster_rows(t, B, h, w):
+        perm = ops.block2_rows(h, w, t.device)
+        return t[(torch.arange(B, device=t.device)[:, None] * (h * w) + perm[None, :]).reshape(-1)]
+
     def _inter_pair_set(self):
         return set(getattr(self, "_inter_pairs", ()) or ())
 
@@ -409,14 +419,19 @@
 
         if c1_ready is not None:
             torch.cuda.current_stream().wait_event(c1_ready)
+        c1_rows = self._c1_rows()
         if taps is not None:
-            taps["c1_map"] = c1.clone()
+            taps["c1_map"] = self._raster_rows(c1, B, H // 4, W // 4) if c1_rows else c1.clone()
         outs = []
         c2p = ws.planes("up_a", B * n2, D, fmt=pk["up"].fmt)
         for bi in range(B):
             ops.split_planes(cbuf[bi * Nc:bi * Nc + n2], kpad=D, out=c2p.rows(bi * n2, (bi + 1) * n2))
-        ops.gemm(c2p, pk["up"], c1, bias=pk["up_b"], resid=c1, batch=B, m=n2, stride_a=c2p.batch_stride(n2),
-                 stride_r=(H // 4) * (W // 4) * D, stride_c=(H // 4) * (W // 4) * D, pixel_shuffle=(H // 8, W // 8, D))
+        if c1_rows:
+            c1v = c1.view(B * n2, 4 * D)
+            ops.gemm(c2p, pk["up"], c1v, bias=pk["up_b"], resid=c1v, batch=B, m=n2, stride_a=c2p.batch_stride(n2), stride_r=n2 * 4 * D, stride_c=n2 * 4 * D)
+        else:
+            ops.gemm(c2p, pk["up"], c1, bias=pk["up_b"], resid=c1, batch=B, m=n2, stride_a=c2p.batch_stride(n2),
+                     stride_r=(H // 4) * (W // 4) * D, stride_c=(H // 4) * (W // 4) * D, pixel_shuffle=(H // 8, W // 8, D))
         emit = bool(getattr(self, "emit_planes", False)) and D % 32 == 0
         ctag = getattr(self._ws, "tag", "")
         if not hasattr(self, "_planes_gens"):
@@ -428,7 +443,8 @@
                                                   (cbuf[n2:], Nc * D, (Hp, Wp)), (cbuf[n2 + n3:], Nc * D, (H // 32, W // 32)))):
             f = torch.empty(B, D, hh, wwd, device=dev)
             fpl = ws.planes(f"f{k + 1}_out", B * hh * wwd, D) if emit else None
-            ops.tail_fuse(src, cs, xs[k + 1] if self.cfg["add_vit_feature"] else None, *pk["bn"][k], f, B, hh, wwd, Hp, Wp, out_planes=fpl)
+            ops.tail_fuse(src, cs, xs[k + 1] if self.cfg["add_vit_feature"] else None, *pk["bn"][k], f, B, hh, wwd, Hp, Wp, out_planes=fpl,
+                          cmap_rows=c1_rows if k == 0 else ops.ROWS_RASTER)
             if emit:
                 f._mmsa_planes = fpl.stamp(pgen)
             outs.append(f)
@@ -891,16 +907,20 @@
                  stride_a=(h + w) * lv["mip_pad"], stride_c=(h + w) * C)
         ops.gemm(y1[h:], lv["caw"], att[h:], bias=lv["caw_b"], act="sigmoid", batch=B, m=w,
                  stride_a=(h + w) * lv["mip_pad"], stride_c=(h + w) * C)
+        zrows = self._c1_rows() if level == 0 else ops.ROWS_RASTER
+        if zrows:
+            assert h % 2 == 0 and w % 2 == 0, "the 1/4-resolution map has even sides (H / 8 and W / 8 are integral)"
         if pl_ok:
             zo = ws.planes("nk_zop", P, C)
-            ops.ca_apply(z, att, None, B, h, w, out_planes=zo)
+            ops.ca_apply(z, att, None, B, h, w, out_planes=zo, out_rows=zrows)
             sa = HW * 2 * C
         else:
             zo = ws.get("nk_g", P, C)
-            ops.ca_apply(z, att, zo, B, h, w)
+            ops.ca_apply(z, att, zo, B, h, w, out_rows=zrows)
             sa = HW * C
         if self._taps is not None:
-            self._taps[f"fuse{level}"] = ops.planes_to_float(zo, cols=C) if pl_ok else zo[:, :C].clone()
+            tap = ops.planes_to_float(zo, cols=C) if pl_ok else zo[:, :C].clone()
+            self._taps[f"fuse{level}"] = self._raster_rows(tap, B, h, w) if zrows else tap
         if out_stride_b == 0:
             ops.gemm(zo, lv["fc"], out, bias=lv["fc_b"])
         else:
diff --git a/multimodal-sam-adapter_amd/mmsa/lib.py b/multimodal-sam-adapter_amd/mmsa/lib.py
--- a/multimodal-sam-adapter_amd/mmsa/lib.py
+++ b/multimodal-sam-adapter_amd/mmsa/lib.py
@@ -58,6 +58,8 @@
     "mmsa_pool_hw": [P, L, P, L, I, I, I, I, P],
     "mmsa_ca_apply": [P, L, P, L, P, L, P, L, I, I, I, I, P],
     "mmsa_tail_fuse": [P, L, L, P, L, P, P, P, P, L, I, I, I, I, I, I, P],
+    "mmsa_ca_apply_rows": [P, L, P, L, P, L, P, L, I, I, I, I, I, P],
+    "mmsa_tail_fuse_rows": [P, L, L, P, L, P, P, P, P, L, I, I, I, I, I, I, I, P],
     "mmsa_global_attention_planes": [P, L, P, P, P, L, I, I, I, I, I, F, I, I, P, P],
     "mmsa_window_attention_planes": [P, L, P, P, P, P, L, I, I, I, I, I, I, F, I, I, P, P],
     "mmsa_nchw_to_planes": [P, L, P, L, I, I, L, P],
diff --git a/multimodal-sam-adapter_amd/mmsa/ops.py b/multimodal-sam-adapter_amd/mmsa/ops.py
--- a/multimodal-sam-adapter_amd/mmsa/ops.py
+++ b/multimodal-sam-adapter_amd/mmsa/ops.py
@@ -673,7 +673,18 @@
     return out
 
 
-def ca_apply(z, att, out, b, h, w, out_planes=None):
+ROWS_RASTER, ROWS_BLOCK2 = 0, 1
+
+
+def block2_rows(h, w, device=None):
+    if h % 2 or w % 2:
+        raise RuntimeError(f"mmsa.block2_rows: a {h} x {w} map has no 2 x 2-block-major row order")
+    y = torch.arange(h, device=device)[:, None]
+    x = torch.arange(w, device=device)[None, :]
+    return ((((y // 2) * (w // 2) + x // 2) * 4) + (y % 2) * 2 + x % 2).reshape(-1)
+
+
+def ca_apply(z, att, out, b, h, w, out_planes=None, out_rows=ROWS_RASTER):
     pz, _, c, ldz = _mat(z, "z")
     pa, _, _, lda = _mat(att, "att")
     po, ldo = (None, 0)
@@ -682,15 +693,15 @@
     pp, ldp = (None, 0)
     if out_planes is not None:
         pp, _, _, ldp = out_planes.mat("out planes")
-    lib.call("mmsa_ca_apply", pz, ldz, pa, lda, po, ldo, pp, ldp, b, h, w, c, _stream())
+    lib.call("mmsa_ca_apply_rows", pz, ldz, pa, lda, po, ldo, pp, ldp, b, h, w, c, out_rows, _stream())
     return out if out is not None else out_planes
 
 
-def tail_fuse(cmap, cstride_b, xtok, bn_scale, bn_shift, out, b, hc, wc, hx, wx, out_planes=None):
+def tail_fuse(cmap, cstride_b, xtok, bn_scale, bn_shift, out, b, hc, wc, hx, wx, out_planes=None, cmap_rows=ROWS_RASTER):
     pc, _, c, ldc = _mat(cmap, "cmap")
     px, ldx = None, 0
     if xtok is not None:
         px, _, _, ldx = _mat(xtok, "xtok")
     pp, ldp = (out_planes.p.data_ptr(), 2 * out_planes.kpad) if out_planes is not None else (None, 0)
-    lib.call("mmsa_tail_fuse", pc, ldc, cstride_b, px, ldx, _chk(bn_scale), _chk(bn_shift), _chk(out), pp, ldp, b, hc, wc, hx, wx, c, _stream())
-    return out
+    lib.call("mmsa_tail_fuse_rows", pc, ldc, cstride_b, px, ldx, _chk(bn_scale), _chk(bn_shift), _chk(out), pp, ldp, b, hc, wc, hx, wx, c, cmap_rows, _stream())
+    return out
```

After: 67.34 (median of 6 runs). No clear change (+0.5%).
